# lmb-freiburg/flownet2

Hardware: AMD Instinct MI355X
Metric: image-pairs/sec FlowNetC forward at 448x320 (higher is better)
Workload: dtype f32

## Files before the change

### flownet2_amd/_lib.py

```python
from __future__ import annotations

import ctypes as C
import os

_HERE = os.path.dirname(os.path.abspath(__file__))
SO_PATH = os.path.join(_HERE, "libflownet2_hip.so")

EXPORTS = [
    "fn2_version", "fn2_last_error_string",
    "fn2_correlation_out_shape", "fn2_correlation_workspace_bytes", "fn2_correlation_forward", "fn2_correlation_forward_fused", "fn2_correlation_backward",
    "fn2_correlation1d_out_shape", "fn2_correlation1d_forward", "fn2_correlation1d_backward",
    "fn2_flow_warp_forward", "fn2_flow_warp_forward_slices", "fn2_flow_warp_backward_workspace_bytes", "fn2_flow_warp_backward",
    "fn2_resample_forward", "fn2_resample_forward_slices",
    "fn2_l1loss_workspace_bytes", "fn2_l1loss_forward", "fn2_l1loss_backward",
    "fn2_l1loss_multi_workspace_bytes", "fn2_l1loss_multi_sync_bytes", "fn2_l1loss_forward_multi", "fn2_l1loss_backward_multi",
    "fn2_channel_norm_forward", "fn2_channel_norm_forward_slices", "fn2_channel_norm_backward",
    "fn2_downsample_forward",
    "fn2_downsample_forward_multi",
    "fn2_predict_flow_conv_workspace_bytes", "fn2_predict_flow_conv_forward", "fn2_upsample_flow_deconv_forward", "fn2_upsample_flow_deconv_forward_into",
    "fn2_predict_flow_conv_backward_supported", "fn2_predict_flow_conv_backward_workspace_bytes", "fn2_predict_flow_conv_backward", "fn2_upsample_flow_deconv_backward_workspace_bytes", "fn2_upsample_flow_deconv_backward",
    "fn2_bias_leaky_relu_forward", "fn2_scale_shift_forward", "fn2_bias_leaky_relu_backward_workspace_bytes", "fn2_bias_leaky_relu_backward", "fn2_bias_leaky_relu_backward_slices", "fn2_bias_leaky_relu_backward_slices2",
    "fn2_conv_k7s2_relu_supported", "fn2_conv_k7s2_relu_forward",
    "fn2_conv_k7s2_wgrad_supported", "fn2_conv_k7s2_wgrad_ksplit", "fn2_conv_k7s2_wgrad_workspace_bytes", "fn2_conv_k7s2_wgrad",
    "fn2_conv_mfma_supported", "fn2_conv_mfma_packed_floats", "fn2_conv_mfma_pack_weights", "fn2_conv_mfma_pack_weights_view", "fn2_conv_mfma_forward",
    "fn2_conv_mfma_num_variants", "fn2_debug_set_conv_variant",
    "fn2_caffemodel_index", "fn2_caffemodel_read_blob", "fn2_hdf5_index", "fn2_hdf5_read_float",
    "fn2_conv_wino_supported", "fn2_conv_wino_packed_floats", "fn2_conv_wino_pack_weights", "fn2_conv_wino_forward",
    "fn2_conv_wino_num_variants", "fn2_debug_set_wino_variant",
    "fn2_conv_plane_supported", "fn2_conv_plane_ksplit", "fn2_conv_plane_workspace_bytes", "fn2_conv_plane_forward",
    "fn2_conv_plane_k_supported", "fn2_conv_plane_k_ksplit", "fn2_conv_plane_k_workspace_bytes", "fn2_conv_plane_k_forward",
    "fn2_conv_plane_num_variants", "fn2_debug_set_plane_variant", "fn2_debug_set_plane_ksplit", "fn2_set_batch_invariant", "fn2_get_batch_invariant",
    "fn2_deconv_plane_supported", "fn2_deconv_plane_ksplit", "fn2_deconv_plane_workspace_bytes", "fn2_deconv_plane_packed_floats",
    "fn2_deconv_plane_pack_weights", "fn2_deconv_plane_pack_weights_k", "fn2_deconv_plane_forward",
    "fn2_tconv_supported", "fn2_tconv_forward", "fn2_tconv_num_variants", "fn2_debug_set_tconv_variant",
    "fn2_debug_set_wgrad_buffers", "fn2_debug_set_wgrad_chunk", "fn2_conv_wgrad_supported", "fn2_conv_wgrad_ksplit", "fn2_conv_wgrad_workspace_bytes", "fn2_conv_wgrad",
    "fn2_conv_route", "fn2_conv_packed_weight_floats", "fn2_conv_pack_weights", "fn2_conv_workspace_bytes", "fn2_conv_forward",
    "fn2_deconv_route", "fn2_deconv_packed_weight_floats", "fn2_deconv_pack_weights", "fn2_deconv_workspace_bytes", "fn2_deconv_forward",
    "fn2_conv_backward_data_route", "fn2_conv_backward_data_packed_weight_floats", "fn2_conv_backward_data_pack_workspace_bytes",
    "fn2_conv_backward_data_pack_weights", "fn2_conv_backward_data_workspace_bytes", "fn2_conv_backward_data_workspace_bytes_with_room", "fn2_conv_backward_data_computed_channels", "fn2_conv_backward_data",
    "fn2_conv_backward_data_masked_supported", "fn2_conv_backward_data_masked", "fn2_conv_backward_weights_bias_fused", "fn2_conv_backward_weights_bias",
    "fn2_conv_backward_weights_supported", "fn2_conv_backward_weights_workspace_bytes", "fn2_conv_backward_weights", "fn2_conv_backward_bias",
    "fn2_im2col_forward", "fn2_col2im_bias_relu_forward", "fn2_col2im_bias_relu_forward_into",
    "fn2_datum_parse", "fn2_datum_float_data", "fn2_datum_serialize",
    "fn2_custom_data_sample_bytes", "fn2_custom_data_encode_sample", "fn2_custom_data_stage_records", "fn2_custom_data_decode_forward",
    "fn2_augmentation_matrix", "fn2_flow_augmentation_forward",
    "fn2_data_augmentation_workspace_bytes", "fn2_data_augmentation_forward",
]


class Fn2Error(RuntimeError):

    def __init__(self, status: int, message: str):
        super().__init__(f"[fn2 status {status}] {message}")
        self.status = status


class CaffemodelEntry(C.Structure):
    _fields_ = [("name_off", C.c_size_t), ("name_len", C.c_size_t), ("type_off", C.c_size_t), ("type_len", C.c_size_t),
                ("v1_type", C.c_longlong), ("v1", C.c_int), ("blob_index", C.c_int), ("num_axes", C.c_int), ("dim", C.c_longlong * 8),
                ("count", C.c_size_t), ("is_double", C.c_int), ("blob_off", C.c_size_t), ("blob_len", C.c_size_t)]


class Hdf5Entry(C.Structure):
    _fields_ = [("path", C.c_char * 256), ("num_axes", C.c_int), ("dim", C.c_longlong * 8), ("count", C.c_size_t), ("type_class", C.c_int),
                ("type_size", C.c_int), ("type_signed", C.c_int), ("big_endian", C.c_int), ("layout", C.c_int), ("num_filters", C.c_int),
                ("header_off", C.c_size_t)]


class ConvDesc(C.Structure):
    _fields_ = [("N", C.c_int), ("Cin", C.c_int), ("Hin", C.c_int), ("Win", C.c_int), ("Cout", C.c_int), ("kernel", C.c_int), ("stride", C.c_int), ("pad", C.c_int)]


class CorrParams(C.Structure):
    _fields_ = [("pad", C.c_int), ("kernel_size", C.c_int), ("max_displacement", C.c_int),
                ("stride1", C.c_int), ("stride2", C.c_int), ("corr_type", C.c_int), ("do_abs", C.c_int),
                ("single_direction", C.c_int)]


class DatumView(C.Structure):
    _fields_ = [("channels", C.c_int), ("height", C.c_int), ("width", C.c_int), ("label", C.c_int), ("encoded", C.c_int),
                ("data", C.c_void_p), ("data_bytes", C.c_size_t), ("float_data_count", C.c_size_t)]


class DataAugParams(C.Structure):
    _fields_ = [("crop_width", C.c_int), ("crop_height", C.c_int), ("max_multiplier", C.c_float), ("has_chromatic_eigvec", C.c_int),
                ("chromatic_eigvec", C.c_float * 9), ("mean_mode", C.c_int), ("noise_seed", C.c_ulonglong), ("noise_stream", C.c_ulonglong)]


class L1LossParams(C.Structure):
    _fields_ = [("l2_per_location", C.c_int), ("l2_prescale_by_channels", C.c_int),
                ("normalize_by_num_entries", C.c_int), ("epsilon", C.c_float), ("plateau", C.c_float)]


class L1LossScale(C.Structure):
    _fields_ = [("bottom0", C.c_void_p), ("bottom1", C.c_void_p), ("bottom0_diff", C.c_void_p), ("bottom1_diff", C.c_void_p),
                ("N", C.c_int), ("C", C.c_int), ("H", C.c_int), ("W", C.c_int), ("loss_weight", C.c_float)]


_lib = None


def lib():
    global _lib
    if _lib is not None:
        return _lib
    if not os.path.exists(SO_PATH):
        raise RuntimeError(
            f"{SO_PATH} not found: the HIP extension is not built. Run `python -m flownet2_amd.build` "
            "(or __graft_entry__.build()). flownet2_amd has no CPU / PyTorch fallback.")
    L = C.CDLL(SO_PATH)
    vp, fp, i, sz = C.c_void_p, C.c_void_p, C.c_int, C.c_size_t
    L.fn2_version.restype = C.c_char_p
    L.fn2_last_error_string.restype = C.c_char_p
    L.fn2_correlation_out_shape.argtypes = [C.POINTER(CorrParams), i, i, i, C.POINTER(i), C.POINTER(i), C.POINTER(i)]
    L.fn2_correlation_workspace_bytes.argtypes = [C.POINTER(CorrParams), i, i, i, i]
    L.fn2_correlation_workspace_bytes.restype = sz
    L.fn2_correlation_forward.argtypes = [C.POINTER(CorrParams), fp, fp, fp, i, i, i, i, vp, sz, vp]
    L.fn2_correlation_forward_fused.argtypes = [C.POINTER(CorrParams), fp, fp, fp, i, i, i, i, i, i, i, C.c_float, vp, sz, vp]
    L.fn2_correlation_backward.argtypes = [C.POINTER(CorrParams), fp, fp, fp, fp, fp, i, i, i, i, vp, sz, vp]
    L.fn2_correlation1d_out_shape.argtypes = [C.POINTER(CorrParams), i, i, i, C.POINTER(i), C.POINTER(i), C.POINTER(i)]
    L.fn2_correlation1d_forward.argtypes = [C.POINTER(CorrParams), fp, fp, fp, i, i, i, i, vp]
    L.fn2_correlation1d_backward.argtypes = [C.POINTER(CorrParams), fp, fp, fp, fp, fp, i, i, i, i, vp]
    L.fn2_flow_warp_forward.argtypes = [fp, fp, fp, i, i, i, i, i, vp]
    L.fn2_flow_warp_forward_slices.argtypes = [fp, i, i, fp, i, i, fp, i, i, i, i, i, i, i, vp]
    L.fn2_flow_warp_backward_workspace_bytes.argtypes = [i, i, i, i]
    L.fn2_flow_warp_backward_workspace_bytes.restype = sz
    L.fn2_flow_warp_backward.argtypes = [fp, fp, fp, fp, fp, i, i, i, i, i, i, vp, sz, vp]
    L.fn2_resample_forward.argtypes = [fp, fp, i, i, i, i, i, i, i, i, vp]
    L.fn2_resample_forward_slices.argtypes = [fp, C.c_float, fp, i, i, fp, i, i, C.c_float, i, i, i, i, i, i, i, i, vp]
    L.fn2_l1loss_workspace_bytes.argtypes = [i, i, i, i]
    L.fn2_l1loss_workspace_bytes.restype = sz
    L.fn2_l1loss_forward.argtypes = [C.POINTER(L1LossParams), fp, fp, fp, i, i, i, i, vp, sz, vp]
    L.fn2_l1loss_backward.argtypes = [C.POINTER(L1LossParams), fp, fp, C.c_float, fp, fp, i, i, i, i, vp, sz, vp]
    L.fn2_l1loss_multi_workspace_bytes.argtypes = [i]
    L.fn2_l1loss_multi_workspace_bytes.restype = sz
    L.fn2_l1loss_multi_sync_bytes.argtypes = []
    L.fn2_l1loss_multi_sync_bytes.restype = sz
    L.fn2_l1loss_forward_multi.argtypes = [C.POINTER(L1LossParams), i, C.POINTER(L1LossScale), fp, fp, vp, sz, vp, vp]
    L.fn2_l1loss_backward_multi.argtypes = [C.POINTER(L1LossParams), i, C.POINTER(L1LossScale), fp, vp, sz, vp]
    L.fn2_channel_norm_forward.argtypes = [fp, fp, i, i, i, i, vp]
    L.fn2_channel_norm_forward_slices.argtypes = [fp, i, i, fp, i, i, fp, i, i, i, i, i, i, vp]
    L.fn2_channel_norm_backward.argtypes = [fp, fp, fp, fp, i, i, i, i, vp]
    L.fn2_downsample_forward.argtypes = [fp, fp, i, i, i, i, i, i, vp]
    L.fn2_downsample_forward_multi.argtypes = [fp, C.POINTER(fp), C.POINTER(i), C.POINTER(i), i, i, i, i, i, vp]
    L.fn2_predict_flow_conv_workspace_bytes.argtypes = [i, i, i, i]
    L.fn2_predict_flow_conv_workspace_bytes.restype = sz
    L.fn2_predict_flow_conv_forward.argtypes = [fp, fp, fp, fp, i, i, i, i, vp, sz, vp]
    L.fn2_predict_flow_conv_backward_supported.argtypes = [i, i, i, i]
    L.fn2_predict_flow_conv_backward_workspace_bytes.argtypes = [i, i, i, i]
    L.fn2_predict_flow_conv_backward_workspace_bytes.restype = sz
    L.fn2_predict_flow_conv_backward.argtypes = [fp, i, i, fp, fp, fp, fp, fp, i, i, i, i, i, vp, sz, vp]
    L.fn2_upsample_flow_deconv_backward_workspace_bytes.argtypes = [i, i, i]
    L.fn2_upsample_flow_deconv_backward_workspace_bytes.restype = sz
    L.fn2_upsample_flow_deconv_backward.argtypes = [fp, fp, fp, fp, fp, fp, i, i, i, i, vp, sz, vp]
    L.fn2_upsample_flow_deconv_forward.argtypes = [fp, fp, fp, fp, i, i, i, vp]
    L.fn2_upsample_flow_deconv_forward_into.argtypes = [fp, fp, fp, fp, i, i, i, i, i, vp]
    L.fn2_bias_leaky_relu_forward.argtypes = [fp, fp, i, i, i, i, C.c_float, vp]
    L.fn2_scale_shift_forward.argtypes = [fp, fp, fp, i, i, i, i, i, i, C.c_float, vp]
    L.fn2_bias_leaky_relu_backward_workspace_bytes.argtypes = [i, i, i, i]
    L.fn2_bias_leaky_relu_backward_workspace_bytes.restype = sz
    L.fn2_bias_leaky_relu_backward.argtypes = [fp, fp, fp, fp, i, i, i, i, C.c_float, vp, sz, vp]
    L.fn2_bias_leaky_relu_backward_slices.argtypes = [fp, fp, i, i, fp, fp, i, i, i, i, C.c_float, vp, sz, vp]
    L.fn2_bias_leaky_relu_backward_slices2.argtypes = [fp, i, i, fp, i, i, fp, fp, i, i, i, i, C.c_float, vp, sz, vp]
    L.fn2_conv_k7s2_relu_supported.argtypes = [i, i, i, i]
    L.fn2_im2col_forward.argtypes = [fp, fp, i, i, i, i, i, i, i, vp]
    L.fn2_col2im_bias_relu_forward.argtypes = [fp, fp, fp, i, i, i, i, i, i, i, i, C.c_float, vp]
    L.fn2_col2im_bias_relu_forward_into.argtypes = [fp, fp, fp, i, i, i, i, i, i, i, i, C.c_float, i, i, vp]
    L.fn2_conv_k7s2_relu_forward.argtypes = [fp, fp, fp, fp, i, i, i, i, i, C.c_float, vp]
    L.fn2_conv_mfma_supported.argtypes = [i] * 7
    L.fn2_conv_mfma_packed_floats.argtypes = [i, i, i]
    L.fn2_conv_mfma_packed_floats.restype = sz
    L.fn2_conv_mfma_pack_weights.argtypes = [fp, fp, i, i, i, vp]
    L.fn2_conv_mfma_pack_weights_view.argtypes = [fp, fp, i, i, i, i, i, C.c_longlong, C.c_longlong, i, vp]
    L.fn2_conv_mfma_forward.argtypes = [fp, fp, fp, fp] + [i] * 13 + [C.c_float, vp]
    L.fn2_debug_set_conv_variant.argtypes = [i]
    L.fn2_conv_wino_supported.argtypes = [i] * 5
    L.fn2_conv_wino_packed_floats.argtypes = [i, i]
    L.fn2_conv_wino_packed_floats.restype = sz
    L.fn2_conv_wino_pack_weights.argtypes = [fp, fp, i, i, vp]
    L.fn2_conv_wino_forward.argtypes = [fp, fp, fp, fp] + [i] * 11 + [C.c_float, vp]
    L.fn2_debug_set_wino_variant.argtypes = [i]
    L.fn2_conv_plane_supported.argtypes = [i] * 7
    L.fn2_conv_plane_ksplit.argtypes = [i] * 7
    L.fn2_conv_plane_workspace_bytes.argtypes = [i] * 7
    L.fn2_conv_plane_workspace_bytes.restype = sz
    L.fn2_conv_plane_forward.argtypes = [fp, fp, fp, fp] + [i] * 12 + [C.c_float, vp, sz, vp]
    L.fn2_conv_k7s2_wgrad_supported.argtypes = [i] * 5
    L.fn2_conv_k7s2_wgrad_ksplit.argtypes = [i] * 5
    L.fn2_conv_k7s2_wgrad_workspace_bytes.argtypes = [i] * 5
    L.fn2_conv_k7s2_wgrad_workspace_bytes.restype = sz
    L.fn2_conv_k7s2_wgrad.argtypes = [fp, fp, fp] + [i] * 6 + [vp, sz, vp]
    L.fn2_conv_plane_k_supported.argtypes = [i] * 8
    L.fn2_conv_plane_k_ksplit.argtypes = [i] * 8
    L.fn2_conv_plane_k_workspace_bytes.argtypes = [i] * 8
    L.fn2_conv_plane_k_workspace_bytes.restype = sz
    L.fn2_conv_plane_k_forward.argtypes = [fp, fp, fp, fp] + [i] * 13 + [C.c_float, vp, sz, vp]
    L.fn2_debug_set_plane_variant.argtypes = [i]
    L.fn2_debug_set_plane_ksplit.argtypes = [i]
    L.fn2_set_batch_invariant.argtypes = [i]
    L.fn2_get_batch_invariant.argtypes = []
    L.fn2_tconv_supported.argtypes = [i] * 8
    L.fn2_tconv_forward.argtypes = [fp, fp, fp, fp] + [i] * 14 + [C.c_float, vp]
    L.fn2_debug_set_tconv_variant.argtypes = [i]
    L.fn2_debug_set_wgrad_buffers.argtypes = [i]
    L.fn2_debug_set_wgrad_chunk.argtypes = [i]
    L.fn2_conv_wgrad_supported.argtypes = [i] * 10
    L.fn2_conv_wgrad_ksplit.argtypes = [i] * 10
    L.fn2_conv_wgrad_workspace_bytes.argtypes = [i] * 10
    L.fn2_conv_wgrad_workspace_bytes.restype = sz
    L.fn2_conv_wgrad.argtypes = [fp, fp, fp] + [i] * 15 + [vp, sz, vp]
    L.fn2_deconv_plane_supported.argtypes = [i] * 5
    L.fn2_deconv_plane_ksplit.argtypes = [i] * 5
    L.fn2_deconv_plane_workspace_bytes.argtypes = [i] * 5
    L.fn2_deconv_plane_workspace_bytes.restype = sz
    L.fn2_deconv_plane_packed_floats.argtypes = [i, i]
    L.fn2_deconv_plane_packed_floats.restype = sz
    L.fn2_deconv_plane_pack_weights.argtypes = [fp, fp, i, i, vp]
    L.fn2_deconv_plane_pack_weights_k.argtypes = [fp, fp, i, i, i, vp]
    L.fn2_deconv_plane_forward.argtypes = [fp, fp, fp, fp] + [i] * 10 + [C.c_float, vp, sz, vp]
    L.fn2_caffemodel_index.argtypes = [vp, sz, C.POINTER(CaffemodelEntry), i, C.POINTER(C.c_int)]
    L.fn2_caffemodel_read_blob.argtypes = [vp, sz, C.POINTER(CaffemodelEntry), fp, sz]
    L.fn2_hdf5_index.argtypes = [vp, sz, C.POINTER(Hdf5Entry), i, C.POINTER(C.c_int)]
    L.fn2_hdf5_read_float.argtypes = [vp, sz, C.POINTER(Hdf5Entry), fp, sz]
    ip = C.POINTER(C.c_int)
    L.fn2_datum_parse.argtypes = [vp, sz, C.POINTER(DatumView)]
    L.fn2_datum_float_data.argtypes = [vp, sz, fp, sz]
    L.fn2_datum_serialize.argtypes = [i, i, i, vp, sz, i, vp, sz]
    L.fn2_datum_serialize.restype = C.c_longlong
    L.fn2_custom_data_sample_bytes.argtypes = [i, i, i, ip, i, ip, i]
    L.fn2_custom_data_sample_bytes.restype = sz
    L.fn2_custom_data_encode_sample.argtypes = [vp, vp, vp, vp, i, i, vp, sz]
    L.fn2_custom_data_stage_records.argtypes = [C.POINTER(C.c_void_p), C.POINTER(sz), i, vp, sz, ip, ip, ip, C.POINTER(sz), ip]
    L.fn2_custom_data_decode_forward.argtypes = [vp, sz, i, i, i, i, ip, i, ip, i, i, fp, C.c_float, C.POINTER(C.c_void_p), vp]
    L.fn2_augmentation_matrix.argtypes = [fp, i, i, i, i, i, fp]
    L.fn2_flow_augmentation_forward.argtypes = [fp, fp, fp, fp, i, i, i, i, i, vp]
    L.fn2_data_augmentation_workspace_bytes.argtypes = [i]
    L.fn2_data_augmentation_workspace_bytes.restype = sz
    L.fn2_data_augmentation_forward.argtypes = [C.POINTER(DataAugParams), fp, fp, fp, fp, i, i, i, i, vp, sz, vp]
    dp = C.POINTER(ConvDesc)
    for pre in ("fn2_conv", "fn2_deconv"):
        getattr(L, pre + "_route").argtypes = [dp, i]
        getattr(L, pre + "_packed_weight_floats").argtypes = [dp, i]
        getattr(L, pre + "_packed_weight_floats").restype = sz
        getattr(L, pre + "_pack_weights").argtypes = [dp, i, fp, fp, vp]
        getattr(L, pre + "_workspace_bytes").argtypes = [dp, i]
        getattr(L, pre + "_workspace_bytes").restype = sz
        getattr(L, pre + "_forward").argtypes = [dp, i, fp, i, i, fp, fp, fp, i, i, i, C.c_float, vp, sz, vp]
    L.fn2_conv_backward_data_route.argtypes = [dp, i]
    L.fn2_conv_backward_data_packed_weight_floats.argtypes = [dp, i, i]
    L.fn2_conv_backward_data_packed_weight_floats.restype = sz
    L.fn2_conv_backward_data_pack_workspace_bytes.argtypes = [dp, i, i]
    L.fn2_conv_backward_data_pack_workspace_bytes.restype = sz
    L.fn2_conv_backward_data_pack_weights.argtypes = [dp, i, i, fp, fp, vp, sz, vp]
    L.fn2_conv_backward_data_workspace_bytes.argtypes = [dp, i, i]
    L.fn2_conv_backward_data_workspace_bytes.restype = sz
    L.fn2_conv_backward_data_computed_channels.argtypes = [dp, i, i]
    L.fn2_conv_backward_data.argtypes = [dp, i, i, fp, i, i, fp, fp, i, i, i, vp, sz, vp]
    L.fn2_conv_backward_weights_supported.argtypes = [dp, i]
    L.fn2_conv_backward_weights_workspace_bytes.argtypes = [dp, i]
    L.fn2_conv_backward_weights_workspace_bytes.restype = sz
    L.fn2_conv_backward_weights.argtypes = [dp, i, fp, i, i, fp, i, i, fp, i, vp, sz, vp]
    L.fn2_conv_backward_data_workspace_bytes_with_room.argtypes = [dp, i, i, i]
    L.fn2_conv_backward_data_workspace_bytes_with_room.restype = sz
    L.fn2_conv_backward_data_masked_supported.argtypes = [dp, i, i]
    L.fn2_conv_backward_data_masked.argtypes = [dp, i, i, fp, i, i, fp, fp, i, i, fp, i, i, C.c_float, vp]
    L.fn2_conv_backward_weights_bias_fused.argtypes = [dp, i]
    L.fn2_conv_backward_weights_bias.argtypes = [dp, i, fp, fp, fp, fp, i, vp, sz, vp]
    L.fn2_conv_backward_bias.argtypes = [fp, i, i, fp, i, i, i, i, i, vp, sz, vp]
    if hasattr(L, "fn2_debug_set_correlation_impl"):
        L.fn2_debug_set_correlation_impl.argtypes = [i]
    if hasattr(L, "fn2_debug_correlation_units_plan"):
        L.fn2_debug_correlation_units_plan.argtypes = [i, i, i, i, C.POINTER(C.c_uint), i]
    if hasattr(L, "fn2_debug_set_resample_generic"):
        L.fn2_debug_set_resample_generic.argtypes = [i]
    for name in EXPORTS:
        if not hasattr(L, name):
            raise RuntimeError(f"{SO_PATH} does not export {name}")
        fn = getattr(L, name)
        if fn.restype is C.c_int:
            pass
    _lib = L
    return L


def check(status: int):
    if status != 0:
        raise Fn2Error(status, lib().fn2_last_error_string().decode())


def version() -> str:
    return lib().fn2_version().decode()
```

### flownet2_amd/build.py

```python
from __future__ import annotations

import glob
import os
import shutil
import subprocess
import sys

HERE = os.path.dirname(os.path.abspath(__file__))
CSRC = os.path.join(HERE, "csrc")
SO = os.path.join(HERE, "libflownet2_hip.so")
ARCH = "gfx950"


def hipcc() -> str:
    for c in (os.environ.get("HIPCC"), "/opt/rocm/bin/hipcc", shutil.which("hipcc")):
        if c and os.path.exists(c):
            return c
    raise RuntimeError("hipcc not found (need ROCm >= 7.0 for gfx950)")


def sources():
    return sorted(glob.glob(os.path.join(CSRC, "*.hip")) + glob.glob(os.path.join(CSRC, "*.cpp")))


def is_stale() -> bool:
    if not os.path.exists(SO):
        return True
    t = os.path.getmtime(SO)
    deps = sources() + glob.glob(os.path.join(CSRC, "*.hpp")) + [os.path.join(HERE, "..", "include", "flownet2_hip.h")]
    return any(os.path.getmtime(d) > t for d in deps)


def build(force: bool = False, verbose: bool = False) -> str:
    if not force and not is_stale():
        return SO
    objs = []
    objdir = os.path.join(HERE, "build")
    os.makedirs(objdir, exist_ok=True)
    flags = ["--offload-arch=" + ARCH, "-O3", "-std=c++17", "-fPIC", "-fvisibility=hidden", "-munsafe-fp-atomics",
             "-Wall", "-Wno-unused-function"]
    if os.environ.get("FN2_ABLATION"):
        flags.append("-DFN2_ABLATION=1")
    per_file = {"conv_wino.hip": ["-fno-slp-vectorize"]}
    procs = []
    for src in sources():
        obj = os.path.join(objdir, os.path.basename(src) + ".o")
        objs.append(obj)
        hdrs = glob.glob(os.path.join(CSRC, "*.hpp")) + [os.path.join(HERE, "..", "include", "flownet2_hip.h")]
        if not force and os.path.exists(obj) and all(os.path.getmtime(obj) >= os.path.getmtime(d) for d in [src] + hdrs):
            continue
        cmd = [hipcc()] + flags + per_file.get(os.path.basename(src), []) + ["-x", "hip", "-c", src, "-o", obj]
        if verbose:
            print(" ".join(cmd), file=sys.stderr)
        procs.append((src, subprocess.Popen(cmd, stdout=subprocess.PIPE, stderr=subprocess.STDOUT)))
    for src, p in procs:
        out, _ = p.communicate()
        if p.returncode != 0:
            raise RuntimeError(f"hipcc failed on {src}:\n{out.decode()}")
        if verbose and out:
            print(out.decode(), file=sys.stderr)
    cmd = [hipcc(), "--offload-arch=" + ARCH, "-shared", "-fPIC", "-o", SO] + objs + ["-lz"]
    subprocess.check_call(cmd)
    return SO


if __name__ == "__main__":
    print(build(force="--force" in sys.argv, verbose=True))
```

### flownet2_amd/csrc/conv_stem.hip

```cpp
#include "fn2_common.hpp"
#include "mfma_tile.hpp"

#include <type_traits>

namespace fn2 {
using mfma::f32x4;
using mfma::kOOB;
using mfma::kRsrcWord3;
using mfma::lds_ptr_t;

struct StemArgs {
  int N, Hin, Win, Hout, Wout, Cout;
  int Ctot, c0;
  int ntx;
  int nyb;
  float slope;
};

template <int CIN, int RB, int XT, int PASS>
__global__ void __launch_bounds__(256, 2)
conv_k7s2_relu(const float* __restrict__ in, const float* __restrict__ weight, const float* __restrict__ bias,
               float* __restrict__ out, StemArgs a) {
  constexpr int ROWS = 2 * RB + 5;
  constexpr int RS = 32 * XT + 8;
  constexpr int CS = ROWS * RS;
  constexpr int SLOTS = CIN * ROWS * (RS / 4);
  constexpr int NRUN = (SLOTS + 63) / 64;
  extern __shared__ __attribute__((aligned(16))) float smem[];

  const int tid = threadIdx.x, lane = tid & 63;
  const int wave = __builtin_amdgcn_readfirstlane(tid >> 6);
  int b = blockIdx.x;
  const int bx = b % a.ntx; b /= a.ntx;
  const int by = b % a.nyb; b /= a.nyb;
  const int cog = b % (a.Cout / 64), n = b / (a.Cout / 64);
  const int x0 = bx * 16 * XT, y0 = by * RB;
  const int co0 = cog * 64 + wave * 16;

  const size_t plane = (size_t)a.Hin * a.Win;
  const __amdgpu_buffer_rsrc_t rs = __builtin_amdgcn_make_buffer_rsrc(
      const_cast<float*>(in + ((size_t)n * a.Ctot + a.c0) * plane), 0, (unsigned)(4u * CIN * plane), kRsrcWord3);
  const unsigned lds_base = (unsigned)(uintptr_t)(lds_ptr_t)smem;
#pragma unroll
  for (int i = 0; i < (NRUN + 3) / 4; ++i) {
    const int run = i * 4 + wave;
    if (run < NRUN) {
      const int s = run * 64 + lane;
      unsigned voff = kOOB;
      if (s < SLOTS) {
        const int c = s / (ROWS * (RS / 4)), rem = s % (ROWS * (RS / 4));
        const int row = rem / (RS / 4), gq = rem % (RS / 4);
        const int yi = 2 * y0 - 3 + row, xi = 2 * x0 - 4 + 4 * gq;
        if (yi >= 0 && yi < a.Hin && xi >= 0 && xi < a.Win) voff = 4u * (unsigned)(c * plane + (size_t)yi * a.Win + xi);
      }
      __builtin_amdgcn_raw_ptr_buffer_load_lds(rs, (lds_ptr_t)(uintptr_t)(lds_base + run * 1024u), 16, voff, 0, 0, 0);
    }
  }

  const int kk = lane >> 4, nn = lane & 15;
  float w[CIN][7][2];
  {
    const float* wp = weight + ((size_t)(co0 + nn) * a.Ctot + a.c0) * 49;
#pragma unroll
    for (int c = 0; c < CIN; ++c)
#pragma unroll
      for (int ky = 0; ky < 7; ++ky) {
        w[c][ky][0] = wp[(c * 7 + ky) * 7 + kk];
        w[c][ky][1] = kk < 3 ? wp[(c * 7 + ky) * 7 + 4 + kk] : 0.f;
      }
  }
  const float bv = bias ? bias[co0 + nn] : 0.f;
  asm volatile("s_waitcnt vmcnt(0)" ::: "memory");
  __syncthreads();

  const int abase = 2 * nn + kk + 1;
  const int xq = 4 * (lane >> 4);
  auto tiles = [&](auto ntag, int rb, int y, int t) {
    constexpr int NTL = decltype(ntag)::value;
    f32x4 acc[NTL];
#pragma unroll
    for (int u = 0; u < NTL; ++u) acc[u] = f32x4{0.f, 0.f, 0.f, 0.f};
    const float* r0 = smem + (2 * rb) * RS + 32 * t + abase;
#pragma unroll
    for (int c = 0; c < CIN; ++c)
#pragma unroll
      for (int ky = 0; ky < 7; ++ky)
#pragma unroll
        for (int h = 0; h < 2; ++h)
#pragma unroll
          for (int u = 0; u < NTL; ++u) {
            float av = r0[c * CS + ky * RS + 4 * h + 32 * u];
            if (h == 1) av = kk == 3 ? 0.f : av;
            acc[u] = __builtin_amdgcn_mfma_f32_16x16x4f32(av, w[c][ky][h], acc[u], 0, 0, 0);
          }
    float* orow = out + (((size_t)n * a.Cout + co0 + nn) * a.Hout + y) * a.Wout;
#pragma unroll
    for (int u = 0; u < NTL; ++u) {
      const int x = x0 + 16 * (t + u) + xq;
      if (x < a.Wout) {
        f32x4 v = acc[u];
        if constexpr (PASS == 2) v += *reinterpret_cast<const f32x4*>(orow + x);
        if constexpr (PASS != 1) {
#pragma unroll
          for (int j = 0; j < 4; ++j) { const float s = v[j] + bv; v[j] = s > 0.f ? s : s * a.slope; }
        }
        *reinterpret_cast<f32x4*>(orow + x) = v;
      }
    }
  };
  for (int rb = 0; rb < RB; ++rb) {
    const int y = y0 + rb;
    if (y >= a.Hout) break;
    int t = 0;
#pragma unroll 1
    for (; t + 1 < XT; t += 2) {
      if (x0 + 16 * t >= a.Wout) break;
      tiles(std::integral_constant<int, 2>{}, rb, y, t);
    }
    if ((XT & 1) && x0 + 16 * t < a.Wout) tiles(std::integral_constant<int, 1>{}, rb, y, t);
  }
}

template <int CIN, int PASS>
static int launch_stem(const float* in, const float* weight, const float* bias, float* out, int N, int Ctot, int c0, int Hin, int Win,
                       int Cout, float slope, hipStream_t st) {
  constexpr int RB = 2, XT = 7;
  StemArgs a;
  a.N = N; a.Hin = Hin; a.Win = Win; a.Cout = Cout; a.slope = slope; a.Ctot = Ctot; a.c0 = c0;
  a.Hout = (Hin + 6 - 7) / 2 + 1; a.Wout = (Win + 6 - 7) / 2 + 1;
  a.ntx = (a.Wout + 16 * XT - 1) / (16 * XT);
  a.nyb = (a.Hout + RB - 1) / RB;
  const long long grid = (long long)N * (Cout / 64) * a.nyb * a.ntx;
  if (grid > 0x7fffffffll) return fail(FN2_ERR_UNSUPPORTED, "conv_k7s2_relu: grid too large");
  constexpr size_t lds = sizeof(float) * CIN * (2 * RB + 5) * (32 * XT + 8) + 1024;
  static bool attr_set = false;
  if (!attr_set) {
    (void)hipFuncSetAttribute(reinterpret_cast<const void*>(&conv_k7s2_relu<CIN, RB, XT, PASS>), hipFuncAttributeMaxDynamicSharedMemorySize, (int)lds);
    attr_set = true;
  }
  hipLaunchKernelGGL((conv_k7s2_relu<CIN, RB, XT, PASS>), dim3((unsigned)grid), dim3(256), lds, st, in, weight, bias, out, a);
  return check_launch("conv_k7s2_relu_forward");
}

}

using namespace fn2;

FN2_API int fn2_conv_k7s2_relu_supported(int Cin, int Hin, int Win, int Cout) {
  return (Cin == 3 || Cin == 6 || Cin == 12) && Cout % 64 == 0 && Cout > 0 && Hin >= 1 && Win >= 8 && Win % 8 == 0 &&
         (long long)Cin * Hin * Win < (1ll << 28);
}

FN2_API int fn2_conv_k7s2_relu_forward(const float* in, const float* weight, const float* bias, float* out,
                                       int N, int Cin, int Hin, int Win, int Cout, float negative_slope, void* stream) {
  if (N < 0 || Cin <= 0 || Hin <= 0 || Win <= 0 || Cout <= 0) return fail(FN2_ERR_INVALID_ARG, "conv_k7s2_relu: bad shape");
  if (N == 0) return FN2_OK;
  if (!in || !weight || !out) return fail(FN2_ERR_INVALID_ARG, "conv_k7s2_relu: null blob");
  if (!fn2_conv_k7s2_relu_supported(Cin, Hin, Win, Cout))
    return fail(FN2_ERR_UNSUPPORTED, "conv_k7s2_relu: needs Cin in {3,6,12}, Cout %% 64 == 0, width %% 8 == 0 (got Cin %d, Cout %d, W %d)", Cin, Cout, Win);
  if (((reinterpret_cast<uintptr_t>(in) | reinterpret_cast<uintptr_t>(out)) & 15) != 0)
    return fail(FN2_ERR_UNSUPPORTED, "conv_k7s2_relu: blobs must be 16-byte aligned");
  hipStream_t st = reinterpret_cast<hipStream_t>(stream);
  if (Cin == 3) return launch_stem<3, 0>(in, weight, bias, out, N, 3, 0, Hin, Win, Cout, negative_slope, st);
  if (Cin == 6) return launch_stem<6, 0>(in, weight, bias, out, N, 6, 0, Hin, Win, Cout, negative_slope, st);
  const int rc = launch_stem<6, 1>(in, weight, bias, out, N, 12, 0, Hin, Win, Cout, negative_slope, st);
  if (rc) return rc;
  return launch_stem<6, 2>(in, weight, bias, out, N, 12, 6, Hin, Win, Cout, negative_slope, st);
}
```

### flownet2_amd/csrc/flow_head.hip

```cpp
#include "fn2_common.hpp"

namespace fn2 {

constexpr int kHeadPix = 64;

template <int G>
__global__ void __launch_bounds__(kHeadPix* G) conv3x3_c2_taps(const float* __restrict__ in, const float* __restrict__ w,
                                                                float* __restrict__ P, int N, int C, int H, int W, int nsplit) {
  __shared__ float red[G][18][kHeadPix];
  const int lane_pix = threadIdx.x % kHeadPix;
  const int grp = __builtin_amdgcn_readfirstlane(threadIdx.x / kHeadPix);
  const size_t plane = (size_t)H * W;
  const long long total = (long long)N * H * W;
  const long long p = (long long)blockIdx.x * kHeadPix + lane_pix;
  const bool live = p < total;
  const int n = live ? (int)(p / (long long)plane) : 0;
  const unsigned pix = live ? (unsigned)(p - (long long)n * plane) : 0u;
  const float* src = in + (size_t)n * C * plane + pix;
  float a[18];
#pragma unroll
  for (int k = 0; k < 18; ++k) a[k] = 0.f;
  const int ngroups = G * nsplit;
  const int c_per = (C + ngroups - 1) / ngroups;
  const int c_lo = min(C, ((int)blockIdx.y * G + grp) * c_per), c_hi = min(C, c_lo + c_per);
  for (int c = c_lo; c < c_hi; c += 8) {
    float v[8];
#pragma unroll
    for (int cc = 0; cc < 8; ++cc) v[cc] = (c + cc < c_hi) ? src[(size_t)(c + cc) * plane] : 0.f;
    __builtin_amdgcn_sched_barrier(0);
#pragma unroll
    for (int cc = 0; cc < 8; ++cc) {
      if (c + cc < c_hi) {
        const float* w0 = w + (size_t)(c + cc) * 9;
        const float* w1 = w + ((size_t)C + c + cc) * 9;
#pragma unroll
        for (int t = 0; t < 9; ++t) {
          a[t] = fmaf(w0[t], v[cc], a[t]);
          a[9 + t] = fmaf(w1[t], v[cc], a[9 + t]);
        }
      }
    }
  }
#pragma unroll
  for (int k = 0; k < 18; ++k) red[grp][k][lane_pix] = a[k];
  __syncthreads();
  if (live) {
    float* dst = P + ((size_t)blockIdx.y * N + n) * 18 * plane + pix;
    for (int k = grp; k < 18; k += G) {
      float sacc = 0.f;
#pragma unroll
      for (int g = 0; g < G; ++g) sacc += red[g][k][lane_pix];
      dst[(size_t)k * plane] = sacc;
    }
  }
}

template <int NSPLIT>
__global__ void __launch_bounds__(256) conv3x3_c2_gather(const float* __restrict__ P, const float* __restrict__ bias,
                                                          float* __restrict__ out, int N, int H, int W) {
  const unsigned plane = (unsigned)H * W;
  const unsigned pix = blockIdx.x * 256u + threadIdx.x;
  if (pix >= plane) return;
  const int y = pix / W, x = pix - y * W;
  const unsigned no = blockIdx.y;
  const unsigned n = no >> 1, o = no & 1;
  float v[NSPLIT][9];
#pragma unroll
  for (int sp = 0; sp < NSPLIT; ++sp) {
    const float* Pn = P + (((size_t)sp * N + n) * 18 + o * 9) * plane;
#pragma unroll
    for (int dy = 0; dy < 3; ++dy)
#pragma unroll
      for (int dx = 0; dx < 3; ++dx) {
        const int yy = y + dy - 1, xx = x + dx - 1;
        const bool ok = yy >= 0 && yy < H && xx >= 0 && xx < W;
        v[sp][dy * 3 + dx] = ok ? Pn[(size_t)(dy * 3 + dx) * plane + (unsigned)yy * W + xx] : 0.f;
      }
  }
  float sacc = bias ? bias[o] : 0.f;
#pragma unroll
  for (int sp = 0; sp < NSPLIT; ++sp)
#pragma unroll
    for (int t = 0; t < 9; ++t) sacc += v[sp][t];
  out[(size_t)no * plane + pix] = sacc;
}

__global__ void __launch_bounds__(256) deconv4x4s2_c2(const float* __restrict__ in, const float* __restrict__ w,
                                                       const float* __restrict__ bias, float* __restrict__ out,
                                                       int N, int H, int W, int out_ctot, int out_c0) {
  const int Ho = 2 * H, Wo = 2 * W;
  const long long total = (long long)N * Ho * Wo;
  for (long long idx = blockIdx.x * (long long)blockDim.x + threadIdx.x; idx < total; idx += (long long)gridDim.x * blockDim.x) {
    const int X = (int)(idx % Wo), Y = (int)((idx / Wo) % Ho), n = (int)(idx / ((long long)Wo * Ho));
    float a0 = bias ? bias[0] : 0.f, a1 = bias ? bias[1] : 0.f;
#pragma unroll
    for (int ty = 0; ty < 2; ++ty) {
      const int ky = ((Y + 1) & 1) + 2 * ty;
      const int iy = (Y + 1 - ky) / 2;
      if (Y + 1 - ky < 0 || iy >= H) continue;
#pragma unroll
      for (int tx = 0; tx < 2; ++tx) {
        const int kx = ((X + 1) & 1) + 2 * tx;
        const int ix = (X + 1 - kx) / 2;
        if (X + 1 - kx < 0 || ix >= W) continue;
#pragma unroll
        for (int c = 0; c < 2; ++c) {
          const float v = in[(((size_t)n * 2 + c) * H + iy) * W + ix];
          a0 = fmaf(w[((c * 2 + 0) * 4 + ky) * 4 + kx], v, a0);
          a1 = fmaf(w[((c * 2 + 1) * 4 + ky) * 4 + kx], v, a1);
        }
      }
    }
    out[(((size_t)n * out_ctot + out_c0 + 0) * Ho + Y) * Wo + X] = a0;
    out[(((size_t)n * out_ctot + out_c0 + 1) * Ho + Y) * Wo + X] = a1;
  }
}

}

using namespace fn2;

constexpr int kHeadG = 16;

static int head_splits(int N, int C, int H, int W) {
  const long long blocks = ((long long)order_batch(N) * H * W + kHeadPix - 1) / kHeadPix;
  int nsplit = 1;
  while (nsplit < 8 && blocks * kHeadG * nsplit < 4096 && C >= 8 * kHeadG * nsplit * 2) nsplit *= 2;
  return nsplit;
}

FN2_API size_t fn2_predict_flow_conv_workspace_bytes(int N, int C, int H, int W) {
  if (N < 1 || C < 1 || H < 1 || W < 1) return 0;
  return sizeof(float) * (size_t)head_splits(N, C, H, W) * N * 18 * H * W;
}

FN2_API int fn2_predict_flow_conv_forward(const float* in, const float* weight, const float* bias, float* out,
                                          int N, int C, int H, int W, void* workspace, size_t workspace_bytes, void* stream) {
  if (N < 0 || C < 1 || H < 1 || W < 1) return fail(FN2_ERR_INVALID_ARG, "predict_flow_conv: bad shape [%d,%d,%d,%d]", N, C, H, W);
  if (N == 0) return FN2_OK;
  if (!in || !weight || !out) return fail(FN2_ERR_INVALID_ARG, "predict_flow_conv: NULL blob pointer");
  if ((long long)H * W >= (1ll << 31) || 2ll * N > 65535) return fail(FN2_ERR_UNSUPPORTED, "predict_flow_conv: blob too large");
  const size_t need = fn2_predict_flow_conv_workspace_bytes(N, C, H, W);
  if (!workspace || workspace_bytes < need) return fail(FN2_ERR_WORKSPACE, "predict_flow_conv: workspace too small (%zu < %zu)", workspace_bytes, need);
  const long long total = (long long)N * H * W;
  const unsigned blocks = (unsigned)((total + kHeadPix - 1) / kHeadPix);
  const int nsplit = head_splits(N, C, H, W);
  hipStream_t st = as_stream(stream);
  float* P = reinterpret_cast<float*>(workspace);
  hipLaunchKernelGGL(conv3x3_c2_taps<kHeadG>, dim3(blocks, nsplit), dim3(kHeadPix * kHeadG), 0, st, in, weight, P, N, C, H, W, nsplit);
  const dim3 g2(((unsigned)H * W + 255) / 256, 2 * N);
  switch (nsplit) {
    case 1: hipLaunchKernelGGL(conv3x3_c2_gather<1>, g2, dim3(256), 0, st, P, bias, out, N, H, W); break;
    case 2: hipLaunchKernelGGL(conv3x3_c2_gather<2>, g2, dim3(256), 0, st, P, bias, out, N, H, W); break;
    case 4: hipLaunchKernelGGL(conv3x3_c2_gather<4>, g2, dim3(256), 0, st, P, bias, out, N, H, W); break;
    default: hipLaunchKernelGGL(conv3x3_c2_gather<8>, g2, dim3(256), 0, st, P, bias, out, N, H, W); break;
  }
  return check_launch("predict_flow_conv_forward");
}

FN2_API int fn2_upsample_flow_deconv_forward(const float* in, const float* weight, const float* bias, float* out,
                                             int N, int H, int W, void* stream) {
  if (N < 0 || H < 1 || W < 1) return fail(FN2_ERR_INVALID_ARG, "upsample_flow_deconv: bad shape");
  if (N == 0) return FN2_OK;
  if (!in || !weight || !out) return fail(FN2_ERR_INVALID_ARG, "upsample_flow_deconv: NULL blob pointer");
  const long long total = (long long)N * 4 * H * W;
  hipLaunchKernelGGL(deconv4x4s2_c2, dim3(blocks_for(total, 256, 4096)), dim3(256), 0, as_stream(stream), in, weight, bias, out, N, H, W, 2, 0);
  return check_launch("upsample_flow_deconv_forward");
}

FN2_API int fn2_upsample_flow_deconv_forward_into(const float* in, const float* weight, const float* bias, float* top,
                                                  int N, int H, int W, int top_channels, int top_c0, void* stream) {
  if (N < 0 || H < 1 || W < 1) return fail(FN2_ERR_INVALID_ARG, "upsample_flow_deconv: bad shape");
  if (top_c0 < 0 || top_c0 + 2 > top_channels) return fail(FN2_ERR_INVALID_ARG, "upsample_flow_deconv: channel slice outside the blob");
  if (N == 0) return FN2_OK;
  if (!in || !weight || !top) return fail(FN2_ERR_INVALID_ARG, "upsample_flow_deconv: NULL blob pointer");
  const long long total = (long long)N * 4 * H * W;
  hipLaunchKernelGGL(deconv4x4s2_c2, dim3(blocks_for(total, 256, 4096)), dim3(256), 0, as_stream(stream), in, weight, bias, top, N, H, W, top_channels, top_c0);
  return check_launch("upsample_flow_deconv_forward_into");
}
```

### flownet2_amd/functional.py

```python
from __future__ import annotations

import os

import torch

from . import ops


_BATCH_INVARIANT = [False]


def set_batch_invariant(on: bool = True):
    _BATCH_INVARIANT[0] = bool(on)
    ops.set_batch_invariant(bool(on))


def batch_invariant() -> bool:
    return _BATCH_INVARIANT[0]


LIBRARY_FALLBACKS = [0]


def _note_fallback(what, x, w):
    LIBRARY_FALLBACKS[0] += 1
    if os.environ.get("FN2_STRICT") == "1":
        raise RuntimeError("flownet2_amd: no own kernel for %s bottom %s weight %s (FN2_STRICT=1)" % (what, tuple(x.shape), tuple(w.shape)))
    if os.environ.get("FN2_TRACE_FALLBACK") == "1":
        print("library fallback: %s bottom %s weight %s" % (what, tuple(x.shape), tuple(w.shape)), flush=True)


def lib_conv2d(x, w, b, stride, pad):
    if x.is_cuda:
        _note_fallback("Convolution{stride %d, pad %d}" % (stride, pad), x, w)
    if not _BATCH_INVARIANT[0] or not x.is_cuda:
        return torch.nn.functional.conv2d(x, w, b, stride=stride, padding=pad)
    return torch.cat([torch.nn.functional.conv2d(x[n:n + 1], w, b, stride=stride, padding=pad) for n in range(x.shape[0])], 0)


def lib_conv_transpose2d(x, w, b, stride, pad):
    if x.is_cuda:
        _note_fallback("Deconvolution{stride %d, pad %d}" % (stride, pad), x, w)
    if not _BATCH_INVARIANT[0] or not x.is_cuda:
        return torch.nn.functional.conv_transpose2d(x, w, b, stride=stride, padding=pad)
    return torch.cat([torch.nn.functional.conv_transpose2d(x[n:n + 1], w, b, stride=stride, padding=pad) for n in range(x.shape[0])], 0)


def scale_shift(x, scale, shift=None, out=None, out_c0=0):
    with torch.no_grad():
        return ops.scale_shift_forward(x.detach().contiguous(), scale, shift, out=out, out_c0=out_c0)


class _Correlation(torch.autograd.Function):
    @staticmethod
    def forward(ctx, b0, b1, params):
        ctx.params = params
        ctx.save_for_backward(b0, b1)
        return ops.correlation_forward(params, b0, b1)

    @staticmethod
    def backward(ctx, g):
        b0, b1 = ctx.saved_tensors
        d0, d1 = ops.correlation_backward(ctx.params, b0, b1, g.contiguous(),
                                          need0=ctx.needs_input_grad[0], need1=ctx.needs_input_grad[1])
        return d0, d1, None


def correlation(b0, b1, pad=0, kernel_size=1, max_displacement=0, stride_1=1, stride_2=1, correlation_type=ops.MULTIPLY):
    p = ops.corr_params(pad, kernel_size, max_displacement, stride_1, stride_2, correlation_type)
    return _Correlation.apply(b0.contiguous(), b1.contiguous(), p)


class _CorrelationReluInto(torch.autograd.Function):

    @staticmethod
    def forward(ctx, b0, b1, params, blob, c0, slope):
        ops.correlation_forward(params, b0, b1, out=blob, out_c0=c0, relu=True, negative_slope=slope)
        tc = ops.correlation_out_shape(params, b0.shape[1], b0.shape[2], b0.shape[3])[0]
        ctx.cfg = (params, c0, tc, slope)
        ctx.save_for_backward(b0, b1, blob)
        return blob[:, c0:c0 + tc]

    @staticmethod
    def backward(ctx, g):
        b0, b1, blob = ctx.saved_tensors
        params, c0, tc, slope = ctx.cfg
        gb, g0 = _channel_slice(g)
        d, _ = ops.bias_leaky_relu_backward((blob, c0, tc), (gb, g0, tc), slope, False)
        d0, d1 = ops.correlation_backward(params, b0, b1, d, need0=ctx.needs_input_grad[0], need1=ctx.needs_input_grad[1])
        return d0, d1, None, None, None, None


def correlation_relu_into(b0, b1, out, out_c0, negative_slope, pad=0, kernel_size=1, max_displacement=0, stride_1=1, stride_2=1, training=False):
    p = ops.corr_params(pad, kernel_size, max_displacement, stride_1, stride_2, ops.MULTIPLY)
    if torch.is_grad_enabled() and (b0.requires_grad or b1.requires_grad):
        if not training:
            return None
        return _CorrelationReluInto.apply(b0.contiguous(), b1.contiguous(), p, out, out_c0, negative_slope)
    return ops.correlation_forward(p, b0.contiguous(), b1.contiguous(), out=out, out_c0=out_c0, relu=True, negative_slope=negative_slope)


class _FlowWarp(torch.autograd.Function):
    @staticmethod
    def forward(ctx, image, flow, fill_value):
        ctx.save_for_backward(image, flow)
        return ops.flow_warp_forward(image, flow, fill_value)

    @staticmethod
    def backward(ctx, g):
        image, flow = ctx.saved_tensors
        di, df = ops.flow_warp_backward(image, flow, g.contiguous(), ctx.needs_input_grad[0], ctx.needs_input_grad[1])
        return (di if ctx.needs_input_grad[0] else None), (df if ctx.needs_input_grad[1] else None), None


def flow_warp(image, flow, fill_value=ops.FILL_ZERO):
    return _FlowWarp.apply(image.contiguous(), flow.contiguous(), fill_value)


def resample(x, height, width, type=ops.LINEAR, antialias=True):
    with torch.no_grad():
        return ops.resample_forward(x.detach().contiguous(), height, width, type, antialias)


def resample_slices(x, height, width, type=ops.LINEAR, antialias=True, in_scale=1.0, out=None, out2=None, out2_scale=1.0):
    with torch.no_grad():
        return ops.resample_forward_slices(x.detach().contiguous(), height, width, type, antialias, in_scale, out, out2, out2_scale)


def flow_warp_slices(image, flow, out=None, fill_value=ops.FILL_ZERO):
    with torch.no_grad():
        return ops.flow_warp_forward_slices(image, flow, out, fill_value)


def channel_norm_slices(x, minus=None, out=None):
    with torch.no_grad():
        return ops.channel_norm_forward_slices(x, minus, out)


def downsample(x, top_height, top_width):
    with torch.no_grad():
        return ops.downsample_forward(x.detach().contiguous(), top_height, top_width)


def downsample_ahead(x, sizes):
    with torch.no_grad():
        x = x.detach().contiguous()
        many = (lambda: ops.downsample_forward_multi(x, sizes)) if ops.downsample_multi_supported(x.shape, sizes) and x.shape[0] > 0 else \
            (lambda: [ops.downsample_forward(x, h, w) for h, w in sizes])
        if not x.is_cuda:
            return [ops.downsample_forward(x, h, w) for h, w in sizes], None
        main = torch.cuda.current_stream(x.device)
        side = _WGRAD_SIDE["streams"].get(x.device)
        if side is None:
            side = _WGRAD_SIDE["streams"][x.device] = torch.cuda.Stream(device=x.device)
        side.wait_stream(main)
        with torch.cuda.stream(side):
            outs = many()
            ev = torch.cuda.Event()
            ev.record(side)
        x.record_stream(side)
        for t in outs:
            t.record_stream(main)
        return outs, ev


def wait_ahead(event):
    if event is not None:
        torch.cuda.current_stream().wait_event(event)


class _ChannelNorm(torch.autograd.Function):
    @staticmethod
    def forward(ctx, x):
        top = ops.channel_norm_forward(x)
        ctx.save_for_backward(x, top)
        return top

    @staticmethod
    def backward(ctx, g):
        x, top = ctx.saved_tensors
        return ops.channel_norm_backward(x, top, g.contiguous())


def channel_norm(x):
    return _ChannelNorm.apply(x.contiguous())


class _L1Loss(torch.autograd.Function):
    @staticmethod
    def forward(ctx, b0, b1, params):
        loss, ws = ops.l1loss_forward(params, b0, b1)
        ctx.params, ctx.ws = params, ws
        ctx.save_for_backward(b0, b1)
        return loss

    @staticmethod
    def backward(ctx, g):
        b0, b1 = ctx.saved_tensors
        d0, d1 = ops.l1loss_backward(ctx.params, b0, b1, float(g), ctx.ws)
        return (d0 if ctx.needs_input_grad[0] else None), (d1 if (b1 is not None and ctx.needs_input_grad[1]) else None), None


def l1_loss(b0, b1=None, l2_per_location=False, l2_prescale_by_channels=False, normalize_by_num_entries=False,
            epsilon=1e-2, plateau=0.0):
    p = ops.l1_params(l2_per_location, l2_prescale_by_channels, normalize_by_num_entries, epsilon, plateau)
    return _L1Loss.apply(b0.contiguous(), b1.contiguous() if b1 is not None else None, p)


class _L1LossMulti(torch.autograd.Function):

    @staticmethod
    def forward(ctx, params, weights, n, *blobs):
        b0, b1 = list(blobs[:n]), list(blobs[n:])
        total, losses, ws = ops.l1loss_forward_multi(params, b0, b1, weights)
        ctx.params, ctx.weights, ctx.n, ctx.ws = params, weights, n, ws
        ctx.save_for_backward(*blobs)
        ctx.mark_non_differentiable(losses)
        return total, losses

    @staticmethod
    def backward(ctx, g, _g_losses):
        n = ctx.n
        blobs = ctx.saved_tensors
        b0, b1 = list(blobs[:n]), list(blobs[n:])
        need1 = any(ctx.needs_input_grad[3 + n:])
        d0, d1 = ops.l1loss_backward_multi(ctx.params, b0, b1, ctx.weights, g.contiguous(), ctx.ws, need1=need1)
        grads = [d if ctx.needs_input_grad[3 + k] else None for k, d in enumerate(d0)]
        grads += [d if ctx.needs_input_grad[3 + n + k] else None for k, d in enumerate(d1)]
        return (None, None, None) + tuple(grads)


def l1_loss_multi(preds, targets, weights, l2_per_location=False, l2_prescale_by_channels=False, normalize_by_num_entries=False,
                  epsilon=1e-2, plateau=0.0):
    p = ops.l1_params(l2_per_location, l2_prescale_by_channels, normalize_by_num_entries, epsilon, plateau)
    blobs = [t.contiguous() for t in preds] + [t.contiguous() for t in targets]
    return _L1LossMulti.apply(p, tuple(float(w) for w in weights), len(preds), *blobs)


class _PredictFlow(torch.autograd.Function):

    @staticmethod
    def forward(ctx, x, weight, bias):
        ctx.save_for_backward(x, weight)
        ctx.has_bias = bias is not None
        return ops.predict_flow_conv_forward(x.contiguous(), weight.contiguous(), bias)

    @staticmethod
    def backward(ctx, g):
        x, w = ctx.saved_tensors
        blob, c0 = _channel_slice(x)
        g = g.contiguous()
        need_x, need_w, need_b = ctx.needs_input_grad[0], ctx.needs_input_grad[1], ctx.has_bias and ctx.needs_input_grad[2]
        side = _wgrad_side_stream(g, x, w) if (need_w or need_b) and need_x else None
        if side is None:
            return ops.predict_flow_conv_backward((blob, c0, x.shape[1]), w, g, need_x, need_w, need_b)
        dx, _, _ = ops.predict_flow_conv_backward((blob, c0, x.shape[1]), w, g, True, False, False)
        main = torch.cuda.current_stream(g.device)
        side.wait_stream(main)
        with torch.cuda.stream(side):
            _, dw, db = ops.predict_flow_conv_backward((blob, c0, x.shape[1]), w, g, False, need_w, need_b)
        for t in (g, blob):
            t.record_stream(side)
        for t in (dw, db):
            if t is not None:
                t.record_stream(main)
        if dw is not None:
            _SIDE_PENDING.append((w, dw.data_ptr()))
        return dx, dw, db


class _UpsampleFlow(torch.autograd.Function):

    @staticmethod
    def forward(ctx, x, weight, bias, into=None):
        ctx.save_for_backward(x, weight)
        ctx.has_bias = bias is not None
        if into is None:
            return ops.upsample_flow_deconv_forward(x.contiguous(), weight.contiguous(), bias)
        ops.upsample_flow_deconv_forward(x.contiguous(), weight.contiguous(), bias, out=into[0], out_c0=into[1])
        return into[0][:, into[1]:into[1] + 2]

    @staticmethod
    def backward(ctx, g):
        x, w = ctx.saved_tensors
        dx, dw, db = ops.upsample_flow_deconv_backward(x.contiguous(), w, g.contiguous(), ctx.needs_input_grad[0], ctx.needs_input_grad[1],
                                                       ctx.has_bias and ctx.needs_input_grad[2])
        return dx, dw, db, None


def predict_flow_conv(x, weight, bias=None):
    run = lambda xx, ww, bb: ops.predict_flow_conv_forward(xx.contiguous(), ww.contiguous(), bb)
    if _needs_grad(x, weight, bias):
        if ops.predict_flow_conv_backward_supported(x.shape[0], x.shape[1], x.shape[2], x.shape[3]):
            return _PredictFlow.apply(x, weight, bias)
        return _OwnForwardConv.apply(x, weight, bias, run, 1, 1, 0.0, False, False)
    return run(x, weight, bias)


def upsample_flow_deconv(x, weight, bias=None, out=None, out_c0=0):
    if out is not None and not _needs_grad(x, weight, bias):
        return ops.upsample_flow_deconv_forward(x.contiguous(), weight.contiguous(), bias, out=out, out_c0=out_c0)
    run = lambda xx, ww, bb: ops.upsample_flow_deconv_forward(xx.contiguous(), ww.contiguous(), bb)
    if _needs_grad(x, weight, bias):
        return _UpsampleFlow.apply(x, weight, bias, None if out is None else (out, out_c0))
    return run(x, weight, bias)


class _BiasLeakyReLU(torch.autograd.Function):

    @staticmethod
    def forward(ctx, y, bias, negative_slope):
        ctx.mark_dirty(y)
        ops.bias_leaky_relu_(y, bias, negative_slope)
        ctx.slope = negative_slope
        ctx.has_bias = bias is not None
        ctx.save_for_backward(y)
        return y

    @staticmethod
    def backward(ctx, g):
        (y,) = ctx.saved_tensors
        d, db = ops.bias_leaky_relu_backward(y, g.contiguous(), ctx.slope, ctx.has_bias and ctx.needs_input_grad[1])
        return d, db, None


def conv_bias_leaky_relu(y, bias, negative_slope=0.1):
    if not y.is_contiguous():
        if bias is not None:
            y = y + bias.view(1, -1, 1, 1)
        return torch.nn.functional.leaky_relu(y, negative_slope)
    if torch.is_grad_enabled() and (y.requires_grad or (bias is not None and bias.requires_grad)):
        return _BiasLeakyReLU.apply(y, bias, negative_slope)
    return ops.bias_leaky_relu_(y, bias, negative_slope)


def invalidate_weight_caches():
    _bump_weight_generation()
    _PACKED_T.clear()


_WEIGHT_GENERATION = [0]


def weight_generation() -> int:
    return _WEIGHT_GENERATION[0]


def _bump_weight_generation(*_a, **_k):
    _WEIGHT_GENERATION[0] += 1


try:
    from torch.optim.optimizer import register_optimizer_step_post_hook as _reg_step_hook
    _reg_step_hook(_bump_weight_generation)
    _HAVE_STEP_HOOK = True
except Exception:
    _HAVE_STEP_HOOK = False


def _cached(cache, key, w, make):
    import weakref
    if w.requires_grad and (not _HAVE_STEP_HOOK or (w.is_cuda and torch.cuda.is_current_stream_capturing())):
        cache.pop(key, None)
        return make()
    gen = _WEIGHT_GENERATION[0] if w.requires_grad else -1
    hit = cache.get(key)
    if hit is None or hit[0]() is not w or hit[1] != w._version or hit[3] != gen:
        hit = (weakref.ref(w, lambda _r, k=key: cache.pop(k, None)), w._version, make(), gen)
        cache[key] = hit
    return hit[2]


_ROUTE_FORCE = [False]


def set_route_force(on: bool = True):
    _ROUTE_FORCE[0] = bool(on)


def _channel_slice(x):
    if x.is_contiguous():
        return x, 0
    b = x._base
    if (b is not None and b.dim() == 4 and b.is_contiguous() and x.dim() == 4 and x.stride() == b.stride() and x.shape[0] == b.shape[0]
            and x.shape[2:] == b.shape[2:]):
        plane = b.shape[2] * b.shape[3]
        off = x.storage_offset() - b.storage_offset()
        if off % plane == 0 and 0 <= off // plane and off // plane + x.shape[1] <= b.shape[1]:
            return b, off // plane
    return x.contiguous(), 0


class _OwnForwardConv(torch.autograd.Function):

    @staticmethod
    def forward(ctx, x, weight, bias, runner, stride, pad, negative_slope, act, transposed, into=None, relu_chain=None):
        if into is None:
            y = runner(x, weight, bias)
        else:
            runner(x, weight, bias, into[0], into[1])
            co = weight.shape[1] if transposed else weight.shape[0]
            y = into[0][:, into[1]:into[1] + co]
        ctx.cfg = (stride, pad, negative_slope, act, bias is not None, transposed)
        ctx.into = into
        ctx.relu_chain, ctx.chain_cell = (int(relu_chain[0]), relu_chain[1]) if relu_chain else (0, None)
        if ctx.relu_chain & 1:
            ctx.chain_cell["armed"] = True
        elif ctx.relu_chain & 2 and not ctx.chain_cell.get("armed"):
            raise RuntimeError("relu_chain: the layer in front of this one is not a chain producer (it would undo its ReLU twice)")
        ctx.save_for_backward(x, weight, (into[0] if into is not None else y) if act else None)
        return y

    @staticmethod
    def backward(ctx, g):
        x, w, y = ctx.saved_tensors
        stride, pad, slope, act, has_bias, transposed = ctx.cfg
        if act and ctx.into is not None:
            y = (y, ctx.into[1], w.shape[1] if transposed else w.shape[0])
        premasked = False
        if ctx.relu_chain & 1:
            if not ctx.chain_cell.get("masked"):
                raise RuntimeError("relu_chain: the consumer of this layer did not fold the ReLU derivative into its data gradient")
            ctx.chain_cell["masked"] = False
            premasked = True
        gx, gw, db = conv_backward(x, w, y if act else None, g, stride, pad, slope, transposed, bool(ctx.needs_input_grad[0]),
                                   bool(ctx.needs_input_grad[1]), has_bias and ctx.needs_input_grad[2], premasked=premasked,
                                   mask_bottom=(ctx.chain_cell["slope"] if (ctx.relu_chain & 2) else None))
        if ctx.relu_chain & 2:
            ctx.chain_cell["masked"] = True
        return (gx, gw, db) + (None,) * (len(ctx.needs_input_grad) - 3)


_GRAD_SLOT = [None]


def set_grad_slots(fn=None):
    _GRAD_SLOT[0] = fn


def _grad_slot(w):
    fn = _GRAD_SLOT[0]
    if fn is None or w.grad is not None:
        return None
    return fn(w)


_WGRAD_SIDE = {"pixels": 0, "streams": {}}
_SIDE_TASK = [-1]
_SIDE_PENDING = []


def set_wgrad_side_stream(max_pixels: int = 0):
    _WGRAD_SIDE["pixels"] = int(max_pixels)


def side_stream_for_collective(device):
    if not _WGRAD_SIDE["pixels"]:
        return None
    st = _WGRAD_SIDE["streams"].get(device)
    if st is None:
        return None
    st.wait_stream(torch.cuda.current_stream(device))
    return st


def _wgrad_side_stream(d, x, w):
    if not _WGRAD_SIDE["pixels"] or not d.is_cuda or w.grad is not None or max(d.shape[2] * d.shape[3], x.shape[2] * x.shape[3]) > _WGRAD_SIDE["pixels"]:
        return None
    task = torch._C._current_graph_task_id()
    if task < 0:
        return None
    if task != _SIDE_TASK[0]:
        if _SIDE_PENDING:
            _SIDE_PENDING.clear()
            for dev, st in _WGRAD_SIDE["streams"].items():
                torch.cuda.current_stream(dev).wait_stream(st)
        torch.autograd.Variable._execution_engine.queue_callback(join_side_streams)
        _SIDE_TASK[0] = task
    st = _WGRAD_SIDE["streams"].get(d.device)
    if st is None:
        st = _WGRAD_SIDE["streams"][d.device] = torch.cuda.Stream(device=d.device)
    return st


def join_side_streams():
    _SIDE_TASK[0] = -1
    if not _SIDE_PENDING:
        return
    for dev, st in _WGRAD_SIDE["streams"].items():
        torch.cuda.current_stream(dev).wait_stream(st)
    pending = list(_SIDE_PENDING)
    _SIDE_PENDING.clear()
    if _GRAD_SLOT[0] is not None:
        return
    for w, ptr in pending:
        if ptr and w.grad is not None and w.grad.data_ptr() != ptr:
            raise RuntimeError("functional.set_wgrad_side_stream: autograd did not move a weight gradient computed on the second stream into "
                               ".grad as it was (shared weight? retained graph?): the result may have been read early.  Switch it off "
                               "(set_wgrad_side_stream(0)) for this graph.")


def relu_chain_supported(x_shape, w, stride, pad) -> bool:
    desc = _layer_desc(w, stride, pad, False, x_shape=x_shape)
    if desc is None or not w.is_cuda:
        return False
    route = ops.conv_backward_data_route(desc, False)
    return route != 0 and ops.conv_backward_data_masked_supported(desc, False, route)


def conv_backward(x, w, y, g, stride, pad, slope, transposed, need_x, need_w, need_b, premasked=False, mask_bottom=None):
    if y is not None and premasked:
        d = g.contiguous()
        db = None
        if need_w and need_b and not transposed and d.is_cuda:
            desc = _layer_desc(w, stride, pad, False, x_shape=x.shape)
            if desc is not None and ops.conv_backward_weights_bias_fused(desc, False) and x.is_contiguous():
                gw, db = ops.conv_backward_weights_bias(x, d, desc, False, out=_grad_slot(w))
                gx = _own_bwd_data(d, w, stride, pad, transposed, x.shape) if need_x else None
                if not need_x or gx is not None:
                    return gx, gw, db
        if need_b:
            db = ops.conv_backward_bias(d, d.shape[1])
    elif y is not None:
        gb, g0 = _channel_slice(g)
        if not isinstance(y, tuple):
            yb, y0 = _channel_slice(y)
            y = (yb, y0, y.shape[1])
        d, db = ops.bias_leaky_relu_backward(y, (gb, g0, g.shape[1]), slope, need_b)
    else:
        g = g.contiguous()
        d, db = g, (g.sum((0, 2, 3)) if need_b else None)
    gx = None
    if need_x and mask_bottom is not None:
        gx = _own_bwd_data_masked(d, w, stride, pad, x, mask_bottom)
    if need_x and gx is None:
        if mask_bottom is not None:
            raise RuntimeError("relu_chain: the data gradient of this layer has no masked form (relu_chain_supported was not asked?)")
        gx = _own_bwd_data(d, w, stride, pad, transposed, x.shape)
    gw = None
    if need_w:
        side = _wgrad_side_stream(d, x, w)
        if side is None:
            gw = _own_bwd_weight(d, x, w, stride, pad, transposed)
        else:
            main = torch.cuda.current_stream(d.device)
            side.wait_stream(main)
            with torch.cuda.stream(side):
                gw = _own_bwd_weight(d, x, w, stride, pad, transposed)
            if gw is None:
                main.wait_stream(side)
            else:
                for t in (d, x):
                    t.record_stream(side)
                gw.record_stream(main)
                _SIDE_PENDING.append((w, gw.data_ptr()))
    lib_x, lib_w = need_x and gx is None, need_w and gw is None
    if (lib_x or lib_w) and os.environ.get("FN2_TRACE_BWD") == "1":
        print("bwd on the library: x %s w %s stride %d pad %d transposed %s -> %s%s" % (tuple(x.shape), tuple(w.shape), stride, pad, transposed,
                                                                                      "data " if lib_x else "", "weight" if lib_w else ""), flush=True)
    if lib_x or lib_w:
        if x.is_cuda:
            _note_fallback("%s backward{stride %d, pad %d}%s%s" % ("Deconvolution" if transposed else "Convolution", stride, pad,
                                                                   " data" if lib_x else "", " weight" if lib_w else ""), x, w)
        cd, was = torch.backends.cudnn, torch.backends.cudnn.deterministic
        cd.deterministic = True
        try:
            gxl, gwl, _ = torch.ops.aten.convolution_backward(d, x, w, None, [stride, stride], [pad, pad], [1, 1], transposed, [0, 0], 1,
                                                              [lib_x, lib_w, False])
        finally:
            cd.deterministic = was
        gx, gw = (gxl if lib_x else gx), (gwl if lib_w else gw)
    return gx, gw, db


def _layer_desc(w, stride, pad, transposed, x_shape=None, d_shape=None):
    k = int(w.shape[2])
    if w.shape[3] != k:
        return None
    Cin, Cout = (int(w.shape[0]), int(w.shape[1])) if transposed else (int(w.shape[1]), int(w.shape[0]))
    if x_shape is not None:
        N, H, W = int(x_shape[0]), int(x_shape[2]), int(x_shape[3])
    elif transposed and d_shape[2] % 2 == 0 and d_shape[3] % 2 == 0:
        N, H, W = int(d_shape[0]), int(d_shape[2]) // 2, int(d_shape[3]) // 2
    elif not transposed and stride == 1:
        N, H, W = int(d_shape[0]), int(d_shape[2]) - 1 + k - 2 * pad, int(d_shape[3]) - 1 + k - 2 * pad
    else:
        return None
    if H < 1 or W < 1:
        return None
    return ops.conv_desc(N, Cin, H, W, Cout, k, stride, pad)


def _own_bwd_weight(d, x, w, stride, pad, transposed):
    if not d.is_cuda:
        return None
    desc = _layer_desc(w, stride, pad, transposed, x_shape=x.shape)
    if desc is None or not ops.conv_backward_weights_supported(desc, transposed):
        return None
    if (not transposed and desc.kernel == 7) and not (d.is_contiguous() and x.is_contiguous()):
        d, x = d.contiguous(), x.contiguous()
    xb, x0 = _channel_slice(x)
    db, d0 = _channel_slice(d)
    return ops.conv_backward_weights(xb, db, desc, transposed, out=_grad_slot(w), bottom_c0=x0, top_c0=d0)


_PACKED_T = {}


def _cached_pack(cache, w, tag, make):
    return _cached(cache, (id(w), tag), w, make)


def _own_bwd_data(d, w, stride, pad, transposed, x_shape=None):
    if not d.is_cuda:
        return None
    desc = _layer_desc(w, stride, pad, transposed, x_shape=x_shape, d_shape=d.shape)
    if desc is None:
        return None
    route = ops.conv_backward_data_route(desc, transposed)
    if route == 0:
        return None
    key = (desc.N, desc.Hin, desc.Win)
    packed = _cached_pack(_PACKED_T, w, ("dgrad", route, bool(transposed), stride, pad) + key,
                          lambda: ops.conv_backward_data_pack_weights(w.detach().contiguous(), desc, transposed, route))
    db, d0 = _channel_slice(d)
    return ops.conv_backward_data(db, packed, desc, transposed, route, top_c0=d0)


def _own_bwd_data_masked(d, w, stride, pad, x, slope):
    desc = _layer_desc(w, stride, pad, False, x_shape=x.shape)
    if desc is None or not d.is_cuda:
        return None
    route = ops.conv_backward_data_route(desc, False)
    if route == 0 or not ops.conv_backward_data_masked_supported(desc, False, route):
        return None
    key = (desc.N, desc.Hin, desc.Win)
    packed = _cached_pack(_PACKED_T, w, ("dgrad", route, False, stride, pad) + key,
                          lambda: ops.conv_backward_data_pack_weights(w.detach().contiguous(), desc, False, route))
    db, d0 = _channel_slice(d)
    xb, x0 = _channel_slice(x)
    return ops.conv_backward_data_masked(db, packed, desc, False, route, xb, slope, top_c0=d0, data_c0=x0)


def _needs_grad(*ts):
    return torch.is_grad_enabled() and any(t is not None and t.requires_grad for t in ts)


def conv_forward_route(desc, act=True, whole_blobs=True) -> int:
    route = ops.conv_forward_route(desc, force=_ROUTE_FORCE[0])
    stem = route == ops.CONV_ROUTE_STEM
    if route == ops.CONV_ROUTE_HEAD:
        return ops.CONV_ROUTE_NONE
    if stem and not (act and whole_blobs):
        return ops.CONV_ROUTE_NONE
    if desc.kernel not in (1, 3, 5, 7) or (desc.kernel == 7 and not stem and desc.Cin % 4 != 0):
        return ops.CONV_ROUTE_NONE
    return route


def deconv_forward_route(desc, act=True) -> int:
    if not act or desc.Cin < 64:
        return ops.DECONV_ROUTE_NONE
    route = ops.deconv_forward_route(desc)
    return ops.DECONV_ROUTE_NONE if route == ops.DECONV_ROUTE_HEAD else route


def conv_route_name(x_shape, w, stride, pad, act=True, whole_blobs=True):
    desc = _layer_desc(w, stride, pad, False, x_shape=x_shape)
    return ops.CONV_FWD_ROUTES[conv_forward_route(desc, act, whole_blobs)] if desc is not None else None


def conv_mfma_relu(x, weight, bias, stride, pad, negative_slope=0.1, act=True, out=None, out_c0=0, relu_chain=None):
    desc = _layer_desc(weight, stride, pad, False, x_shape=x.shape) if x.is_cuda else None
    route = conv_forward_route(desc, act, out is None) if desc is not None else ops.CONV_ROUTE_NONE
    if route == ops.CONV_ROUTE_NONE:
        return None
    if relu_chain is not None and int(relu_chain[0]) & 1 and route != ops.CONV_ROUTE_STEM:
        raise RuntimeError("relu_chain: only the stem layer is a chain producer")

    def run(xx, ww, bb, o=None, o0=0):
        if route == ops.CONV_ROUTE_STEM:
            blob, c0, packed = xx.contiguous(), 0, ww.detach().contiguous()
        else:
            blob, c0 = _channel_slice(xx)
            packed = _cached_pack(_PACKED_T, ww, ("fwd", route, False), lambda: ops.conv_pack_weights(ww.detach(), desc, route))
        return ops.conv_forward(blob, packed, bb, desc, route, False, act, negative_slope, out=o, out_c0=o0, in_c0=c0)

    if _needs_grad(x, weight, bias):
        return _OwnForwardConv.apply(x, weight, bias, run, stride, pad, negative_slope, act, False, None if out is None else (out, out_c0), relu_chain)
    return run(x, weight, bias, out, out_c0)


def deconv_relu(x, weight, bias, negative_slope=0.1, act=True, out=None, out_c0=0):
    desc = _layer_desc(weight, 2, 1, True, x_shape=x.shape) if x.is_cuda else None
    route = deconv_forward_route(desc, act) if desc is not None else ops.DECONV_ROUTE_NONE
    if route == ops.DECONV_ROUTE_NONE:
        return None

    def run(xx, ww, bb, o=None, o0=0):
        blob, c0 = _channel_slice(xx)
        packed = _cached_pack(_PACKED_T, ww, ("fwd", route, True), lambda: ops.conv_pack_weights(ww.detach(), desc, route, True))
        return ops.conv_forward(blob, packed, bb, desc, route, True, True, negative_slope, out=o, out_c0=o0, in_c0=c0)

    if _needs_grad(x, weight, bias):
        return _OwnForwardConv.apply(x, weight, bias, run, 2, 1, negative_slope, True, True, None if out is None else (out, out_c0))
    return run(x, weight, bias, out, out_c0)
```

### flownet2_amd/nets.py

```python
from __future__ import annotations

import math
import weakref
from typing import Dict, Optional


import torch
import torch.nn.functional as F

NEG_SLOPE = 0.1
FLOW_SCALE = 20.0
SD_FLOW_SCALE = 0.05
LOSS_WEIGHTS = {6: 0.32, 5: 0.08, 4: 0.02, 3: 0.01, 2: 0.005}

_ENC_TAIL = [("conv4", 256, 512, 3, 2, 1), ("conv4_1", 512, 512, 3, 1, 1), ("conv5", 512, 512, 3, 2, 1),
             ("conv5_1", 512, 512, 3, 1, 1), ("conv6", 512, 1024, 3, 2, 1), ("conv6_1", 1024, 1024, 3, 1, 1)]
_DEC = [("Convolution1", "conv", 1024, 2), ("deconv5", "deconv", 1024, 512), ("upsample_flow6to5", "deconv", 2, 2),
        ("Convolution2", "conv", 1026, 2), ("deconv4", "deconv", 1026, 256), ("upsample_flow5to4", "deconv", 2, 2),
        ("Convolution3", "conv", 770, 2), ("deconv3", "deconv", 770, 128), ("upsample_flow4to3", "deconv", 2, 2),
        ("Convolution4", "conv", 386, 2), ("deconv2", "deconv", 386, 64), ("upsample_flow3to2", "deconv", 2, 2),
        ("Convolution5", "conv", 194, 2)]


def layer_table(kind: str = "C", in_channels: int = 6):
    t = []
    if kind == "C":
        t += [("conv1", "conv", 3, 64, 7, 2, 3), ("conv2", "conv", 64, 128, 5, 2, 2), ("conv3", "conv", 128, 256, 5, 2, 2),
              ("conv_redir", "conv", 256, 32, 1, 1, 0), ("conv3_1", "conv", 473, 256, 3, 1, 1)]
    else:
        t += [("conv1", "conv", in_channels, 64, 7, 2, 3), ("conv2", "conv", 64, 128, 5, 2, 2), ("conv3", "conv", 128, 256, 5, 2, 2),
              ("conv3_1", "conv", 256, 256, 3, 1, 1)]
    t += [(n, "conv", ci, co, k, s, p) for (n, ci, co, k, s, p) in _ENC_TAIL]
    for (n, k, ci, co) in _DEC:
        t.append((n, k, ci, co, 3, 1, 1) if k == "conv" else (n, k, ci, co, 4, 2, 1))
    return t


def init_params(kind: str = "C", seed: int = 0, device="cpu", in_channels: int = 6) -> Dict[str, torch.Tensor]:
    g = torch.Generator().manual_seed(seed)
    params = {}
    for (name, k, ci, co, ks, s, p) in layer_table(kind, in_channels):
        shape = (co, ci, ks, ks) if k == "conv" else (ci, co, ks, ks)
        fan_in = ci * ks * ks if k == "conv" else ci * ks * ks / (s * s)
        std = math.sqrt(2.0 / ((1 + NEG_SLOPE ** 2) * fan_in))
        if name.startswith("Convolution"):
            std *= 0.5
        if name.startswith("upsample_flow"):
            std = 0.25
        params[name + ".w"] = (torch.randn(shape, generator=g) * std).to(device)
        params[name + ".b"] = torch.zeros(co).to(device)
    return params


def num_params(params) -> int:
    return sum(int(v.numel()) for v in params.values())


def _conv(x, P, name, stride, pad, act=True, backend=None, relu_chain=None):
    w = P[name + ".w"]
    if relu_chain is not None:
        y = conv_forward(x, w, P[name + ".b"], stride, pad, act, backend, relu_chain=relu_chain)
    else:
        y = _conv_routed(x, P, name, stride, pad, act, backend)
    if _TRACE_CONV:
        print("conv route %-16s in %-22s k%d s%d act=%d -> %s" % (name, tuple(x.shape), w.shape[2], stride, act, _LAST_ROUTE[0]))
    return y


_TRACE_CONV = __import__("os").environ.get("FN2_TRACE_CONV") == "1"
_LAST_ROUTE = [""]


def _conv_routed(x, P, name, stride, pad, act, backend):
    return conv_forward(x, P[name + ".w"], P[name + ".b"], stride, pad, act, backend)


def conv_forward(x, w, b, stride, pad, act, backend, slope=None, relu_chain=None):
    slope = NEG_SLOPE if slope is None else slope
    y = None
    if backend is not None and hasattr(backend, "conv_mfma_relu"):
        y = backend.conv_mfma_relu(x, w, b, stride, pad, slope, act, relu_chain=relu_chain)
    if y is not None:
        _LAST_ROUTE[0] = "fn2 %s" % backend.conv_route_name(x.shape, w, stride, pad, act) if _TRACE_CONV and hasattr(backend, "conv_route_name") else "own kernel"
        return y
    if relu_chain is not None:
        raise RuntimeError("relu_chain: no own kernel takes this layer (its consumer was told the stem kernel would)")
    _LAST_ROUTE[0] = "library conv2d"
    conv2d = getattr(backend, "lib_conv2d", None) or (lambda xx, ww, bb, s, p: F.conv2d(xx, ww, bb, stride=s, padding=p))
    if act and backend is not None and hasattr(backend, "conv_bias_leaky_relu"):
        return backend.conv_bias_leaky_relu(conv2d(x, w, None, stride, pad), b, slope)
    y = conv2d(x, w, b, stride, pad)
    return F.leaky_relu(y, slope) if act else y


_CONSTS: Dict[tuple, torch.Tensor] = {}


def _const(device, values):
    key = (str(device), tuple(float(v) for v in values))
    if key not in _CONSTS:
        _CONSTS[key] = torch.tensor(key[1], device=device, dtype=torch.float32)
    return _CONSTS[key]


def _deconv(x, P, name, act=True, backend=None):
    return deconv_forward(x, P[name + ".w"], P[name + ".b"], act, backend)


def deconv_forward(x, w, b, act=True, backend=None, slope=None):
    slope = NEG_SLOPE if slope is None else slope
    if backend is not None and hasattr(backend, "deconv_relu"):
        y = backend.deconv_relu(x, w, b, slope, act)
        if y is not None:
            return y
    deconv2d = getattr(backend, "lib_conv_transpose2d", None) or (lambda xx, ww, bb, s, p: F.conv_transpose2d(xx, ww, bb, stride=s, padding=p))
    if act and backend is not None and hasattr(backend, "conv_bias_leaky_relu"):
        return backend.conv_bias_leaky_relu(deconv2d(x, w, None, 2, 1), b, slope)
    y = deconv2d(x, w, b, 2, 1)
    return F.leaky_relu(y, slope) if act else y


def _conv_into_concat(x, P, name, stride, pad, extra_channels, backend, relu_chain=None):
    w = P[name + ".w"]
    training = torch.is_grad_enabled() and (x.requires_grad or _any_requires_grad(P))
    if (backend is not None and hasattr(backend, "conv_mfma_relu") and x.is_cuda and w.shape[2] in (3, 5)
            and (not training or (CONCAT_IN_PLACE_TRAINING[0] and hasattr(backend, "conv_backward")))):
        k = w.shape[2]
        ho, wo = (x.shape[2] + 2 * pad - k) // stride + 1, (x.shape[3] + 2 * pad - k) // stride + 1
        blob = torch.empty((x.shape[0], w.shape[0] + extra_channels, ho, wo), device=x.device, dtype=x.dtype)
        y = backend.conv_mfma_relu(x, w, P[name + ".b"], stride, pad, NEG_SLOPE, True, out=blob, out_c0=0, relu_chain=relu_chain)
        if y is not None:
            return blob, (y if (training and y.requires_grad) else blob[:, :w.shape[0]])
    if relu_chain is not None:
        raise RuntimeError("relu_chain: conv '%s' left the own-kernel route after its producer was told it would fold the ReLU derivative" % name)
    return None, _conv(x, P, name, stride, pad, backend=backend)


def _conv_into(x, P, name, stride, pad, blob, c0, backend):
    return backend.conv_mfma_relu(x, P[name + ".w"], P[name + ".b"], stride, pad, NEG_SLOPE, True, out=blob, out_c0=c0)


def _any_requires_grad(P) -> bool:
    vals = P.P.values() if isinstance(P, _Prefixed) else P.values()
    return any(v.requires_grad for v in vals)


def _stage_deconv(P, x, dname, blob, cs, cd, backend, allow_copy=True):
    d = backend.deconv_relu(x, P[dname + ".w"], P[dname + ".b"], NEG_SLOPE, True, out=blob, out_c0=cs) if hasattr(backend, "deconv_relu") else None
    if d is None and allow_copy:
        blob[:, cs:cs + cd].copy_(_deconv(x, P, dname, backend=backend))
    return d


def _refine_stage(P, skip, x, dname, flow, uname, backend):
    def up(t, name, out=None, out_c0=0):
        if backend is not None and hasattr(backend, "upsample_flow_deconv"):
            if out is not None:
                return backend.upsample_flow_deconv(t, P[name + ".w"], P[name + ".b"], out=out, out_c0=out_c0)
            return backend.upsample_flow_deconv(t, P[name + ".w"], P[name + ".b"])
        return _deconv(t, P, name, act=False)

    blob, s = skip if isinstance(skip, tuple) else (None, skip)
    if blob is None:
        return torch.cat([s, _deconv(x, P, dname, backend=backend), up(flow, uname)], 1)
    cs, cd = s.shape[1], P[dname + ".w"].shape[1]
    assert blob.shape[1] == cs + cd + 2
    stage_params = [P[n] for n in (dname + ".w", dname + ".b", uname + ".w", uname + ".b")]
    if torch.is_grad_enabled() and (s.requires_grad or x.requires_grad or flow.requires_grad or any(p.requires_grad for p in stage_params)):
        d = _stage_deconv(P, x, dname, blob, cs, cd, backend, allow_copy=False)
        u = up(flow, uname, out=blob, out_c0=cs + cd) if (d is not None and hasattr(backend, "upsample_flow_deconv")) else None
        if d is None or u is None:
            return torch.cat([s, _deconv(x, P, dname, backend=backend), up(flow, uname)], 1)
        part = lambda t, c0, c: t if t.requires_grad else blob[:, c0:c0 + c]
        return _ConcatInPlace.apply(blob, s, part(d, cs, cd), part(u, cs + cd, 2))
    _stage_deconv(P, x, dname, blob, cs, cd, backend)
    if hasattr(backend, "upsample_flow_deconv"):
        up(flow, uname, out=blob, out_c0=cs + cd)
    else:
        blob[:, cs + cd:].copy_(up(flow, uname))
    return blob


def _decoder(P, conv6_1, conv5_1, conv4_1, conv3_1, conv2, backend=None):
    def pf(x, name):
        if backend is not None and hasattr(backend, "predict_flow_conv"):
            return backend.predict_flow_conv(x, P[name + ".w"], P[name + ".b"])
        return _conv(x, P, name, 1, 1, act=False, backend=backend)

    def stage(skip, x, dname, flow, uname):
        return _refine_stage(P, skip, x, dname, flow, uname, backend)


    flow6 = pf(conv6_1, "Convolution1")
    c5 = stage(conv5_1, conv6_1, "deconv5", flow6, "upsample_flow6to5")
    flow5 = pf(c5, "Convolution2")
    c4 = stage(conv4_1, c5, "deconv4", flow5, "upsample_flow5to4")
    flow4 = pf(c4, "Convolution3")
    c3 = stage(conv3_1, c4, "deconv3", flow4, "upsample_flow4to3")
    flow3 = pf(c3, "Convolution4")
    c2 = stage(conv2, c3, "deconv2", flow3, "upsample_flow3to2")
    flow2 = pf(c2, "Convolution5")
    return {2: flow2, 3: flow3, 4: flow4, 5: flow5, 6: flow6}


def _skip_conv(x, P, name, stride, pad, dname, backend, relu_chain=None):
    return _conv_into_concat(x, P, name, stride, pad, P[dname + ".w"].shape[1] + 2, backend, relu_chain=relu_chain)


RELU_CHAIN = [True]


def _stem_chain(P, x, backend):
    if not (RELU_CHAIN[0] and CONCAT_IN_PLACE_TRAINING[0] and torch.is_grad_enabled() and x.is_cuda and hasattr(backend, "relu_chain_supported")
            and hasattr(backend, "conv_route_name")):
        return None, None
    w1, w2 = P["conv1.w"], P["conv2.w"]
    if not (w1.requires_grad and w2.requires_grad and P["conv1.b"].requires_grad) or x.requires_grad:
        return None, None
    if backend.conv_route_name(x.shape, w1, 2, 3) != "stem":
        return None, None
    c1_shape = (x.shape[0], w1.shape[0], (x.shape[2] - 1) // 2 + 1, (x.shape[3] - 1) // 2 + 1)
    if not backend.relu_chain_supported(c1_shape, w2, 2, 2):
        return None, None
    cell = {"masked": False, "slope": NEG_SLOPE}
    return (1, cell), (2, cell)


CONCAT_IN_PLACE_TRAINING = [True]


class _ConcatInPlace(torch.autograd.Function):

    @staticmethod
    def forward(ctx, blob, *parts):
        ctx.cuts = [p.shape[1] for p in parts]
        assert sum(ctx.cuts) == blob.shape[1] and all(p.data_ptr() >= blob.data_ptr() for p in parts)
        return blob.view_as(blob)

    @staticmethod
    def backward(ctx, g):
        out, c0 = [None], 0
        for c in ctx.cuts:
            out.append(g[:, c0:c0 + c])
            c0 += c
        return tuple(out)


TOWER_SPLIT_OPS = [True]


class _SplitTowers(torch.autograd.Function):

    @staticmethod
    def forward(ctx, x):
        n = x.shape[0] // 2
        return x[:n], x[n:]

    @staticmethod
    def backward(ctx, ga, gb):
        return torch.cat([ga, gb], 0)


class _StackedAndFirstTower(torch.autograd.Function):

    @staticmethod
    def forward(ctx, x):
        return x.view_as(x), x[:x.shape[0] // 2]

    @staticmethod
    def backward(ctx, g_all, g_first):
        if g_all._base is not None or not g_all.is_contiguous():
            g_all = g_all.clone(memory_format=torch.contiguous_format)
        g_all[:g_first.shape[0]].add_(g_first)
        return g_all


def flownet_c_core(P, img0, img1, backend, towers=None):
    x = towers if towers is not None else torch.cat([img0, img1], 0)
    n = x.shape[0] // 2
    chain1, chain2 = _stem_chain(P, x, backend)
    c1 = _conv(x, P, "conv1", 2, 3, backend=backend, relu_chain=chain1)
    blob2, c2 = _skip_conv(c1, P, "conv2", 2, 2, "deconv2", backend, relu_chain=chain2)
    training = TOWER_SPLIT_OPS[0] and torch.is_grad_enabled() and c2.requires_grad
    c2_first = None
    if training:
        c2, c2_first = _StackedAndFirstTower.apply(c2)
    c3 = _conv(c2, P, "conv3", 2, 2, backend=backend)
    c3a, c3b = _SplitTowers.apply(c3) if (training and c3.requires_grad) else (c3[:n], c3[n:])
    cat = redir = None
    cr = P["conv_redir.w"].shape[0]
    if hasattr(backend, "correlation_relu_into") and c3a.is_cuda:
        cat = torch.empty((n, cr + 441, c3a.shape[2], c3a.shape[3]), device=c3a.device, dtype=c3a.dtype)
        in_graph = (CONCAT_IN_PLACE_TRAINING[0] and torch.is_grad_enabled() and (c3a.requires_grad or c3b.requires_grad)
                    and hasattr(backend, "conv_backward"))
        if in_graph:
            redir = _conv_into(c3a, P, "conv_redir", 1, 0, cat, 0, backend)
            corr = backend.correlation_relu_into(c3a, c3b, cat, cr, NEG_SLOPE, pad=20, kernel_size=1, max_displacement=20, stride_1=1, stride_2=2,
                                                 training=True)
            if redir is not None and redir.requires_grad:
                cat = _ConcatInPlace.apply(cat, redir, corr)
            else:
                cat = torch.cat([_conv(c3a, P, "conv_redir", 1, 0, backend=backend), corr], 1)
        elif backend.correlation_relu_into(c3a, c3b, cat, cr, NEG_SLOPE, pad=20, kernel_size=1, max_displacement=20,
                                           stride_1=1, stride_2=2) is None:
            cat = None
        else:
            into = None
            if hasattr(backend, "conv_mfma_relu") and not (torch.is_grad_enabled() and _any_requires_grad(P)):
                into = backend.conv_mfma_relu(c3a, P["conv_redir.w"], P["conv_redir.b"], 1, 0, NEG_SLOPE, True, out=cat, out_c0=0)
            if into is None:
                cat[:, :cr].copy_(_conv(c3a, P, "conv_redir", 1, 0, backend=backend))
    if cat is None:
        redir = _conv(c3a, P, "conv_redir", 1, 0, backend=backend)
        corr = backend.correlation(c3a, c3b, pad=20, kernel_size=1, max_displacement=20, stride_1=1, stride_2=2)
        cat = torch.cat([redir, F.leaky_relu(corr, NEG_SLOPE)], 1)
    blob3, c31 = _skip_conv(cat, P, "conv3_1", 1, 1, "deconv3", backend)
    c4 = _conv(c31, P, "conv4", 2, 1, backend=backend)
    blob4, c41 = _skip_conv(c4, P, "conv4_1", 1, 1, "deconv4", backend)
    c5 = _conv(c41, P, "conv5", 2, 1, backend=backend)
    blob5, c51 = _skip_conv(c5, P, "conv5_1", 1, 1, "deconv5", backend)
    c6 = _conv(c51, P, "conv6", 2, 1, backend=backend)
    c61 = _conv(c6, P, "conv6_1", 1, 1, backend=backend)
    c2s = c2_first if c2_first is not None else c2[:n]
    skip2 = (blob2[:n], c2s) if blob2 is not None else c2s
    return _decoder(P, c61, (blob5, c51), (blob4, c41), (blob3, c31), skip2, backend)


def flownet_s_core(P, x, backend=None):
    c1 = _conv(x, P, "conv1", 2, 3, backend=backend)
    blob2, c2 = _skip_conv(c1, P, "conv2", 2, 2, "deconv2", backend)
    c3 = _conv(c2, P, "conv3", 2, 2, backend=backend)
    blob3, c31 = _skip_conv(c3, P, "conv3_1", 1, 1, "deconv3", backend)
    c4 = _conv(c31, P, "conv4", 2, 1, backend=backend)
    blob4, c41 = _skip_conv(c4, P, "conv4_1", 1, 1, "deconv4", backend)
    c5 = _conv(c41, P, "conv5", 2, 1, backend=backend)
    blob5, c51 = _skip_conv(c5, P, "conv5_1", 1, 1, "deconv5", backend)
    c6 = _conv(c51, P, "conv6", 2, 1, backend=backend)
    c61 = _conv(c6, P, "conv6_1", 1, 1, backend=backend)
    return _decoder(P, c61, (blob5, c51), (blob4, c41), (blob3, c31), (blob2, c2), backend)


def adapted_size(h: int, w: int, divisor: int = 64):
    return int(math.ceil(h / divisor) * divisor), int(math.ceil(w / divisor) * divisor)


def deploy_forward(kind: str, P, img0, img1, backend, mean: Optional[torch.Tensor] = None):
    N, _, H, W = img0.shape
    ah, aw = adapted_size(H, W)
    neg_default = mean is None
    if mean is None:
        mean = _const(img0.device, (0.411, 0.433, 0.45))
    if (ah, aw) == (H, W) and img0.is_cuda and not torch.is_grad_enabled() and hasattr(backend, "scale_shift"):
        neg_mean = _const(img0.device, (-0.411, -0.433, -0.45)) if neg_default else (-mean).contiguous()
        if kind == "C":
            x = torch.empty((2 * N, 3, H, W), device=img0.device, dtype=torch.float32)
            backend.scale_shift(img0, 1.0 / 255.0, neg_mean, out=x[:N])
            backend.scale_shift(img1, 1.0 / 255.0, neg_mean, out=x[N:])
            flows = flownet_c_core(P, None, None, backend, towers=x)
        else:
            x = torch.empty((N, 6, H, W), device=img0.device, dtype=torch.float32)
            backend.scale_shift(img0, 1.0 / 255.0, neg_mean, out=x, out_c0=0)
            backend.scale_shift(img1, 1.0 / 255.0, neg_mean, out=x, out_c0=3)
            flows = flownet_s_core(P, x, backend)
    else:
        pre = []
        for im in (img0, img1):
            x = im * (1.0 / 255.0)
            if (ah, aw) != (H, W):
                x = backend.resample(x, ah, aw)
            pre.append(x - mean.view(1, 3, 1, 1))
        if kind == "C":
            flows = flownet_c_core(P, pre[0], pre[1], backend)
        else:
            flows = flownet_s_core(P, torch.cat(pre, 1), backend)
    if img0.is_cuda and not torch.is_grad_enabled() and hasattr(backend, "resample_slices"):
        flow = backend.resample_slices(flows[2], H, W, in_scale=FLOW_SCALE)
        if (ah, aw) == (H, W):
            return flow
    else:
        flow = flows[2] * FLOW_SCALE
        flow = backend.resample(flow, H, W)
    scale = _const(flow.device, (W / float(aw), H / float(ah)))
    return flow * scale.view(1, 2, 1, 1)


def loss_targets_ahead(gt_flow, backend, divisors=None):
    if not (hasattr(backend, "downsample_ahead") and gt_flow.is_cuda):
        return None
    H, W = gt_flow.shape[2], gt_flow.shape[3]
    divisors = divisors or {s: 2 ** s for s in LOSS_WEIGHTS}
    gt = gt_flow * (1.0 / FLOW_SCALE)
    sizes = [(H // divisors[s], W // divisors[s]) for s in LOSS_WEIGHTS]
    tgts, ev = backend.downsample_ahead(gt, sizes)
    return {"targets": dict(zip(LOSS_WEIGHTS, tgts)), "event": ev, "sizes": dict(zip(LOSS_WEIGHTS, sizes))}


FINAL_FLOW_GT_SCALE = {"SD": 1.0 / SD_FLOW_SCALE, "fusion": 1.0}


def final_flow_loss(flow, gt_flow, backend, scale):
    tgt = backend.downsample(gt_flow * scale, flow.shape[2], flow.shape[3])
    return backend.l1_loss(flow, tgt, l2_per_location=True, normalize_by_num_entries=True)


def multiscale_loss(flows, gt_flow, backend, targets=None):
    if hasattr(backend, "l1_loss_multi") and gt_flow.is_cuda:
        scales = list(LOSS_WEIGHTS.items())
        preds = [flows[s] for s, _ in scales]
        if targets is not None and all(tuple(targets["sizes"][s]) == tuple(flows[s].shape[2:]) for s, _ in scales):
            backend.wait_ahead(targets["event"])
            tgts = [targets["targets"][s] for s, _ in scales]
        else:
            gt = gt_flow * (1.0 / FLOW_SCALE)
            tgts = [backend.downsample(gt, p.shape[2], p.shape[3]) for p in preds]
        return backend.l1_loss_multi(preds, tgts, [w for _, w in scales], l2_per_location=True, normalize_by_num_entries=True)[0]
    gt = gt_flow * (1.0 / FLOW_SCALE)
    total = 0.0
    for s, w in LOSS_WEIGHTS.items():
        pred = flows[s]
        tgt = backend.downsample(gt, pred.shape[2], pred.shape[3])
        total = total + w * backend.l1_loss(pred, tgt, l2_per_location=True, normalize_by_num_entries=True)
    return total


def conv_flops(kind: str, h: int, w: int, in_channels: int = 6) -> float:
    fl = 0.0
    size = {}
    hh, ww = h, w
    res = {"conv1": 2, "conv2": 4, "conv3": 8, "conv_redir": 8, "conv3_1": 8, "conv4": 16, "conv4_1": 16, "conv5": 32, "conv5_1": 32,
           "conv6": 64, "conv6_1": 64, "Convolution1": 64, "deconv5": 32, "upsample_flow6to5": 32, "Convolution2": 32,
           "deconv4": 16, "upsample_flow5to4": 16, "Convolution3": 16, "deconv3": 8, "upsample_flow4to3": 8, "Convolution4": 8,
           "deconv2": 4, "upsample_flow3to2": 4, "Convolution5": 4}
    for (name, k, ci, co, ks, s, p) in layer_table(kind, in_channels):
        oh, ow = hh // res[name], ww // res[name]
        macs = oh * ow * co * ci * ks * ks if k == "conv" else (oh // 2) * (ow // 2) * ci * co * ks * ks
        mult = 2 if (kind == "C" and name in ("conv1", "conv2", "conv3")) else 1
        fl += 2.0 * macs * mult
    return fl


_SD_TABLE = [("conv0", "conv", 6, 64, 3, 1, 1), ("conv1", "conv", 64, 64, 3, 2, 1), ("conv1_1", "conv", 64, 128, 3, 1, 1),
             ("conv2", "conv", 128, 128, 3, 2, 1), ("conv2_1", "conv", 128, 128, 3, 1, 1), ("conv3", "conv", 128, 256, 3, 2, 1),
             ("conv3_1", "conv", 256, 256, 3, 1, 1), ("conv4", "conv", 256, 512, 3, 2, 1), ("conv4_1", "conv", 512, 512, 3, 1, 1),
             ("conv5", "conv", 512, 512, 3, 2, 1), ("conv5_1", "conv", 512, 512, 3, 1, 1), ("conv6", "conv", 512, 1024, 3, 2, 1),
             ("conv6_1", "conv", 1024, 1024, 3, 1, 1),
             ("Convolution1", "conv", 1024, 2, 3, 1, 1), ("deconv5", "deconv", 1024, 512, 4, 2, 1), ("upsample_flow6to5", "deconv", 2, 2, 4, 2, 1),
             ("interconv5", "conv", 1026, 512, 3, 1, 1), ("Convolution2", "conv", 512, 2, 3, 1, 1),
             ("deconv4", "deconv", 1026, 256, 4, 2, 1), ("upsample_flow5to4", "deconv", 2, 2, 4, 2, 1),
             ("interconv4", "conv", 770, 256, 3, 1, 1), ("Convolution3", "conv", 256, 2, 3, 1, 1),
             ("deconv3", "deconv", 770, 128, 4, 2, 1), ("upsample_flow4to3", "deconv", 2, 2, 4, 2, 1),
             ("interconv3", "conv", 386, 128, 3, 1, 1), ("Convolution4", "conv", 128, 2, 3, 1, 1),
             ("deconv2", "deconv", 386, 64, 4, 2, 1), ("upsample_flow3to2", "deconv", 2, 2, 4, 2, 1),
             ("interconv2", "conv", 194, 64, 3, 1, 1), ("Convolution5", "conv", 64, 2, 3, 1, 1)]
_FUSE_TABLE = [("conv0", "conv", 11, 64, 3, 1, 1), ("conv1", "conv", 64, 64, 3, 2, 1), ("conv1_1", "conv", 64, 128, 3, 1, 1),
               ("conv2", "conv", 128, 128, 3, 2, 1), ("conv2_1", "conv", 128, 128, 3, 1, 1),
               ("Convolution5", "conv", 128, 2, 3, 1, 1), ("deconv1", "deconv", 128, 32, 4, 2, 1), ("upsample_flow2to1", "deconv", 2, 2, 4, 2, 1),
               ("interconv1", "conv", 162, 32, 3, 1, 1), ("Convolution6", "conv", 32, 2, 3, 1, 1),
               ("deconv0", "deconv", 162, 16, 4, 2, 1), ("upsample_flow1to0", "deconv", 2, 2, 4, 2, 1),
               ("interconv0", "conv", 82, 16, 3, 1, 1), ("Convolution7", "conv", 16, 2, 3, 1, 1)]


_SD_RES = {"conv0": 1, "conv1": 2, "conv1_1": 2, "conv2": 4, "conv2_1": 4, "conv3": 8, "conv3_1": 8, "conv4": 16, "conv4_1": 16, "conv5": 32,
           "conv5_1": 32, "conv6": 64, "conv6_1": 64, "Convolution1": 64, "deconv5": 32, "upsample_flow6to5": 32, "interconv5": 32,
           "Convolution2": 32, "deconv4": 16, "upsample_flow5to4": 16, "interconv4": 16, "Convolution3": 16, "deconv3": 8,
           "upsample_flow4to3": 8, "interconv3": 8, "Convolution4": 8, "deconv2": 4, "upsample_flow3to2": 4, "interconv2": 4, "Convolution5": 4}
_FUSE_RES = {"conv0": 1, "conv1": 2, "conv1_1": 2, "conv2": 4, "conv2_1": 4, "Convolution5": 4, "deconv1": 2, "upsample_flow2to1": 2,
             "interconv1": 2, "Convolution6": 2, "deconv0": 1, "upsample_flow1to0": 1, "interconv0": 1, "Convolution7": 1}


def _table_flops(table, res, h, w):
    fl = 0.0
    for (name, k, ci, co, ks, s, p) in table:
        oh, ow = h // res[name], w // res[name]
        fl += 2.0 * (oh * ow * co * ci * ks * ks if k == "conv" else (oh // 2) * (ow // 2) * ci * co * ks * ks)
    return fl


def flownet2_conv_flops(h: int, w: int) -> float:
    return conv_flops("C", h, w) + 2 * conv_flops("S", h, w, 12) + _table_flops(_SD_TABLE, _SD_RES, h, w) + _table_flops(_FUSE_TABLE, _FUSE_RES, h, w)


def _init_table(table, prefix, g, params, device):
    for (name, k, ci, co, ks, s, p) in table:
        shape = (co, ci, ks, ks) if k == "conv" else (ci, co, ks, ks)
        fan_in = ci * ks * ks if k == "conv" else ci * ks * ks / (s * s)
        std = math.sqrt(2.0 / ((1 + NEG_SLOPE ** 2) * fan_in))
        if name.startswith("Convolution"):
            std *= 0.5
        if name.startswith("upsample_flow"):
            std = 0.25
        params[prefix + name + ".w"] = (torch.randn(shape, generator=g) * std).to(device)
        params[prefix + name + ".b"] = torch.zeros(co).to(device)


def init_params_flownet2(seed: int = 0, device="cpu") -> Dict[str, torch.Tensor]:
    g = torch.Generator().manual_seed(seed)
    P: Dict[str, torch.Tensor] = {}
    _init_table(layer_table("C"), "", g, P, device)
    _init_table(layer_table("S", 12), "net2_", g, P, device)
    _init_table(layer_table("S", 12), "net3_", g, P, device)
    _init_table(_SD_TABLE, "netsd_", g, P, device)
    _init_table(_FUSE_TABLE, "fuse_", g, P, device)
    return P


class _Prefixed(dict):

    def __init__(self, P, prefix):
        super().__init__()
        self.P, self.prefix = P, prefix

    def __getitem__(self, k):
        return self.P[self.prefix + k]


def _pf(P, x, name, backend):
    if backend is not None and hasattr(backend, "predict_flow_conv"):
        return backend.predict_flow_conv(x, P[name + ".w"], P[name + ".b"])
    return _conv(x, P, name, 1, 1, act=False, backend=backend)


def flownet_sd_core(P, x, backend):
    c0 = _conv(x, P, "conv0", 1, 1, backend=backend)
    c1 = _conv(_conv(c0, P, "conv1", 2, 1, backend=backend), P, "conv1_1", 1, 1, backend=backend)
    blob2, c2 = _conv_into_concat(_conv(c1, P, "conv2", 2, 1, backend=backend), P, "conv2_1", 1, 1, 64 + 2, backend)
    blob3, c3 = _conv_into_concat(_conv(c2, P, "conv3", 2, 1, backend=backend), P, "conv3_1", 1, 1, 128 + 2, backend)
    blob4, c4 = _skip_conv(_conv(c3, P, "conv4", 2, 1, backend=backend), P, "conv4_1", 1, 1, "deconv4", backend)
    blob5, c5 = _skip_conv(_conv(c4, P, "conv5", 2, 1, backend=backend), P, "conv5_1", 1, 1, "deconv5", backend)
    c6 = _conv(_conv(c5, P, "conv6", 2, 1, backend=backend), P, "conv6_1", 1, 1, backend=backend)
    flow6 = _pf(P, c6, "Convolution1", backend)
    cat5 = _refine_stage(P, (blob5, c5), c6, "deconv5", flow6, "upsample_flow6to5", backend)
    flow5 = _pf(P, _conv(cat5, P, "interconv5", 1, 1, act=False, backend=backend), "Convolution2", backend)
    cat4 = _refine_stage(P, (blob4, c4), cat5, "deconv4", flow5, "upsample_flow5to4", backend)
    flow4 = _pf(P, _conv(cat4, P, "interconv4", 1, 1, act=False, backend=backend), "Convolution3", backend)
    cat3 = _refine_stage(P, (blob3, c3), cat4, "deconv3", flow4, "upsample_flow4to3", backend)
    flow3 = _pf(P, _conv(cat3, P, "interconv3", 1, 1, act=False, backend=backend), "Convolution4", backend)
    cat2 = _refine_stage(P, (blob2, c2), cat3, "deconv2", flow3, "upsample_flow3to2", backend)
    return _pf(P, _conv(cat2, P, "interconv2", 1, 1, act=False, backend=backend), "Convolution5", backend)


def fusion_core(P, x, backend):
    blob0, c0 = _conv_into_concat(x, P, "conv0", 1, 1, 16 + 2, backend)
    blob1, c1 = _conv_into_concat(_conv(c0, P, "conv1", 2, 1, backend=backend), P, "conv1_1", 1, 1, 32 + 2, backend)
    c2 = _conv(_conv(c1, P, "conv2", 2, 1, backend=backend), P, "conv2_1", 1, 1, backend=backend)
    flow2 = _pf(P, c2, "Convolution5", backend)
    cat1 = _refine_stage(P, (blob1, c1), c2, "deconv1", flow2, "upsample_flow2to1", backend)
    flow1 = _pf(P, _conv(cat1, P, "interconv1", 1, 1, act=False, backend=backend), "Convolution6", backend)
    cat0 = _refine_stage(P, (blob0, c0), cat1, "deconv0", flow1, "upsample_flow1to0", backend)
    return _pf(P, _conv(cat0, P, "interconv0", 1, 1, act=False, backend=backend), "Convolution7", backend)


def flownet2_deploy_forward(P, img0, img1, backend, mean: Optional[torch.Tensor] = None):
    N, _, H, W = img0.shape
    ah, aw = adapted_size(H, W)
    neg_mean = _const(img0.device, (-0.411, -0.433, -0.45)) if mean is None else (-mean).contiguous()
    if mean is None:
        mean = _const(img0.device, (0.411, 0.433, 0.45))
    if img0.is_cuda and not torch.is_grad_enabled() and hasattr(backend, "resample_slices"):
        return _flownet2_pick_streams(P, img0, img1, backend, neg_mean)
    if (ah, aw) == (H, W) and img0.is_cuda and not torch.is_grad_enabled() and hasattr(backend, "scale_shift"):
        a = backend.scale_shift(img0, 1.0 / 255.0, neg_mean)
        b = backend.scale_shift(img1, 1.0 / 255.0, neg_mean)
    else:
        a = backend.resample(img0 * (1.0 / 255.0), ah, aw) - mean.view(1, 3, 1, 1)
        b = backend.resample(img1 * (1.0 / 255.0), ah, aw) - mean.view(1, 3, 1, 1)

    def refine_input(flow_q):
        flow = backend.resample(flow_q * FLOW_SCALE, ah, aw)
        warped = backend.flow_warp(b, flow)
        err = backend.channel_norm(a - warped)
        return flow, warped, err

    flow1_q = flownet_c_core(P, a, b, backend)[2]
    f1, w1, e1 = refine_input(flow1_q)
    flow2_q = flownet_s_core(_Prefixed(P, "net2_"), torch.cat([a, b, w1, f1 * (1.0 / FLOW_SCALE), e1], 1), backend)[2]
    f2, w2, e2 = refine_input(flow2_q)
    flow3_q = flownet_s_core(_Prefixed(P, "net3_"), torch.cat([a, b, w2, f2 * (1.0 / FLOW_SCALE), e2], 1), backend)[2]
    flow_css = backend.resample(flow3_q * FLOW_SCALE, ah, aw, type=1)
    flow_sd = backend.resample(flownet_sd_core(_Prefixed(P, "netsd_"), torch.cat([a, b], 1), backend) * SD_FLOW_SCALE, ah, aw, type=1)
    err_css = backend.channel_norm(a - backend.flow_warp(b, flow_css))
    err_sd = backend.channel_norm(a - backend.flow_warp(b, flow_sd))
    fuse_in = torch.cat([a, flow_sd, flow_css, backend.channel_norm(flow_sd), backend.channel_norm(flow_css), err_sd, err_css], 1)
    flow = fusion_core(_Prefixed(P, "fuse_"), fuse_in, backend)
    flow = backend.resample(flow, H, W)
    scale = _const(flow.device, (W / float(aw), H / float(ah)))
    return flow * scale.view(1, 2, 1, 1)


_SD_STREAM = {"mode": "auto", "streams": {}, "picked": {}}


def set_sd_side_stream(mode="auto"):
    _SD_STREAM["mode"] = {True: "on", False: "off"}.get(mode, mode)
    _SD_STREAM["picked"] = {}


def _flownet2_pick_streams(P, img0, img1, backend, neg_mean):
    import time
    mode = _SD_STREAM["mode"]
    run = lambda side: _flownet2_deploy_forward_slices(P, img0, img1, backend, neg_mean, side)
    if mode != "auto":
        return run(mode == "on")
    key = (img0.device, tuple(img0.shape))
    st = _SD_STREAM["picked"].get(key)
    if isinstance(st, bool):
        return run(st)
    if torch.cuda.is_current_stream_capturing():
        return run(True)
    if st is None:
        st = _SD_STREAM["picked"][key] = {"n": 0, True: [], False: []}
    n = st["n"]
    st["n"] += 1
    if n == 0:
        return run(True)
    side = n % 2 == 1
    torch.cuda.synchronize(img0.device)
    t0 = time.perf_counter()
    out = run(side)
    torch.cuda.synchronize(img0.device)
    st[side].append(time.perf_counter() - t0)
    if n >= 4:
        _SD_STREAM["picked"][key] = min(st[True]) <= 1.01 * min(st[False])
        _SD_STREAM.setdefault("timings_ms", {})[key] = {"second_stream": round(min(st[True]) * 1e3, 4), "one_stream": round(min(st[False]) * 1e3, 4)}
    return out


def sd_side_stream_timings():
    return dict(_SD_STREAM.get("timings_ms", {}))


def sd_side_stream_picks():
    return {k: v for k, v in _SD_STREAM["picked"].items() if isinstance(v, bool)}


def _sd_side_stream(dev, on):
    if not on:
        return None
    st = _SD_STREAM["streams"].get(dev)
    if st is None:
        st = _SD_STREAM["streams"][dev] = torch.cuda.Stream(device=dev)
    return st


def _flownet2_deploy_forward_slices(P, img0, img1, backend, neg_mean, sd_beside=True):
    N, _, H, W = img0.shape
    ah, aw = adapted_size(H, W)
    dev = img0.device
    new = lambda c: torch.empty((N, c, ah, aw), device=dev, dtype=torch.float32)
    towers = torch.empty((2 * N, 3, ah, aw), device=dev, dtype=torch.float32)
    blob = new(12)
    pair = new(6)
    fuse = new(11)
    for k, img in enumerate((img0, img1)):
        if (ah, aw) == (H, W):
            src, s = img, 1.0 / 255.0
        else:
            src, s = backend.resample_slices(img, ah, aw, in_scale=1.0 / 255.0), 1.0
        backend.scale_shift(src, s, neg_mean, out=towers[k * N:(k + 1) * N])
        backend.scale_shift(src, s, neg_mean, out=blob, out_c0=3 * k)
        backend.scale_shift(src, s, neg_mean, out=pair, out_c0=3 * k)
        if k == 0:
            backend.scale_shift(src, s, neg_mean, out=fuse, out_c0=0)
    A, B, WARPED = (blob, 0, 3), (blob, 3, 3), (blob, 6, 3)

    def refine_input(flow_q):
        flow = backend.resample_slices(flow_q, ah, aw, in_scale=FLOW_SCALE, out2=(blob, 9, 2), out2_scale=1.0 / FLOW_SCALE)
        backend.flow_warp_slices(B, flow, out=WARPED)
        backend.channel_norm_slices(A, minus=WARPED, out=(blob, 11, 1))

    side = _sd_side_stream(dev, sd_beside)
    sd_q = None
    if side is not None:
        main = torch.cuda.current_stream(dev)
        side.wait_stream(main)
        with torch.cuda.stream(side):
            sd_q = flownet_sd_core(_Prefixed(P, "netsd_"), pair, backend)
    flow1_q = flownet_c_core(P, None, None, backend, towers=towers)[2]
    refine_input(flow1_q)
    flow2_q = flownet_s_core(_Prefixed(P, "net2_"), blob, backend)[2]
    refine_input(flow2_q)
    flow3_q = flownet_s_core(_Prefixed(P, "net3_"), blob, backend)[2]
    if side is not None:
        main.wait_stream(side)
        sd_q.record_stream(main)
    else:
        sd_q = flownet_sd_core(_Prefixed(P, "netsd_"), pair, backend)
    backend.resample_slices(sd_q, ah, aw, type=1, in_scale=SD_FLOW_SCALE, out=(fuse, 3, 2))
    backend.resample_slices(flow3_q, ah, aw, type=1, in_scale=FLOW_SCALE, out=(fuse, 5, 2))
    backend.channel_norm_slices((fuse, 3, 2), out=(fuse, 7, 1))
    backend.channel_norm_slices((fuse, 5, 2), out=(fuse, 8, 1))
    backend.flow_warp_slices(B, (fuse, 3, 2), out=WARPED)
    backend.channel_norm_slices(A, minus=WARPED, out=(fuse, 9, 1))
    backend.flow_warp_slices(B, (fuse, 5, 2), out=WARPED)
    backend.channel_norm_slices(A, minus=WARPED, out=(fuse, 10, 1))
    flow = fusion_core(_Prefixed(P, "fuse_"), fuse, backend)
    if (ah, aw) == (H, W):
        return flow
    flow = backend.resample(flow, H, W)
    scale = _const(flow.device, (W / float(aw), H / float(ah)))
    return flow * scale.view(1, 2, 1, 1)
```

### flownet2_amd/ops.py

```python
from __future__ import annotations

import ctypes as C

import torch

from . import _lib
from ._lib import CorrParams, L1LossParams, check

MULTIPLY, SUBTRACT = 0, 1
FILL_ZERO, FILL_NAN = 1, 2
NEAREST, LINEAR, CUBIC, AREA = 1, 2, 3, 4


def _stream():
    return C.c_void_p(torch.cuda.current_stream().cuda_stream)


def _chk(t: torch.Tensor, name: str, ndim: int = 4):
    if not isinstance(t, torch.Tensor) or not t.is_cuda:
        raise ValueError(f"{name}: expected a CUDA (HIP) tensor; flownet2_amd has no CPU path")
    if t.dtype != torch.float32:
        raise ValueError(f"{name}: expected float32 (Dtype=float), got {t.dtype}")
    if ndim is not None and t.dim() != ndim:
        raise ValueError(f"{name}: expected {ndim} axes (NCHW), got shape {tuple(t.shape)}")
    return t.contiguous()


def _ptr(t):
    return C.c_void_p(t.data_ptr()) if t is not None else C.c_void_p(0)


def corr_params(pad=0, kernel_size=1, max_displacement=0, stride_1=1, stride_2=1, correlation_type=MULTIPLY, do_abs=False,
                single_direction=0):
    return CorrParams(int(pad), int(kernel_size), int(max_displacement), int(stride_1), int(stride_2),
                      int(correlation_type), int(bool(do_abs)), int(single_direction))


def correlation_out_shape(p: CorrParams, Cc: int, H: int, W: int):
    tc, th, tw = C.c_int(), C.c_int(), C.c_int()
    check(_lib.lib().fn2_correlation_out_shape(C.byref(p), Cc, H, W, C.byref(tc), C.byref(th), C.byref(tw)))
    return tc.value, th.value, tw.value


def correlation_forward(p: CorrParams, bottom0: torch.Tensor, bottom1: torch.Tensor, out: torch.Tensor | None = None,
                        out_c0: int = 0, relu: bool = False, negative_slope: float = 0.0):
    b0, b1 = _chk(bottom0, "bottom[0]"), _chk(bottom1, "bottom[1]")
    if b0.shape != b1.shape:
        raise ValueError("Both bottom blobs must have same shape")
    N, Cc, H, W = b0.shape
    tc, th, tw = correlation_out_shape(p, Cc, H, W)
    top = out if out is not None else torch.empty((N, tc, th, tw), device=b0.device, dtype=torch.float32)
    assert top.is_contiguous() and top.shape[0] == N and tuple(top.shape[2:]) == (th, tw) and out_c0 + tc <= top.shape[1]
    if not relu and out_c0 == 0 and top.shape[1] == tc:
        check(_lib.lib().fn2_correlation_forward(C.byref(p), _ptr(b0), _ptr(b1), _ptr(top), N, Cc, H, W, None, 0, _stream()))
    else:
        check(_lib.lib().fn2_correlation_forward_fused(C.byref(p), _ptr(b0), _ptr(b1), _ptr(top), N, Cc, H, W, int(top.shape[1]), int(out_c0),
                                                       int(bool(relu)), C.c_float(float(negative_slope)), None, 0, _stream()))
    return top


def correlation_backward(p: CorrParams, bottom0, bottom1, top_diff, need0=True, need1=True):
    b0, b1, td = _chk(bottom0, "bottom[0]"), _chk(bottom1, "bottom[1]"), _chk(top_diff, "top.diff")
    N, Cc, H, W = b0.shape
    d0 = torch.empty_like(b0) if need0 else None
    d1 = torch.empty_like(b1) if need1 else None
    check(_lib.lib().fn2_correlation_backward(C.byref(p), _ptr(b0), _ptr(b1), _ptr(td), _ptr(d0), _ptr(d1),
                                              N, Cc, H, W, None, 0, _stream()))
    return d0, d1


def correlation1d_out_shape(p: CorrParams, Cc: int, H: int, W: int):
    tc, th, tw = C.c_int(), C.c_int(), C.c_int()
    check(_lib.lib().fn2_correlation1d_out_shape(C.byref(p), Cc, H, W, C.byref(tc), C.byref(th), C.byref(tw)))
    return tc.value, th.value, tw.value


def correlation1d_forward(p: CorrParams, bottom0: torch.Tensor, bottom1: torch.Tensor):
    b0, b1 = _chk(bottom0, "bottom[0]"), _chk(bottom1, "bottom[1]")
    if b0.shape != b1.shape:
        raise ValueError("Both bottom blobs must have same shape")
    N, Cc, H, W = b0.shape
    tc, th, tw = correlation1d_out_shape(p, Cc, H, W)
    top = torch.empty((N, tc, th, tw), device=b0.device, dtype=torch.float32)
    check(_lib.lib().fn2_correlation1d_forward(C.byref(p), _ptr(b0), _ptr(b1), _ptr(top), N, Cc, H, W, _stream()))
    return top


def correlation1d_backward(p: CorrParams, bottom0, bottom1, top_diff, need0=True, need1=True):
    b0, b1, td = _chk(bottom0, "bottom[0]"), _chk(bottom1, "bottom[1]"), _chk(top_diff, "top.diff")
    N, Cc, H, W = b0.shape
    d0 = torch.empty_like(b0) if need0 else None
    d1 = torch.empty_like(b1) if need1 else None
    check(_lib.lib().fn2_correlation1d_backward(C.byref(p), _ptr(b0), _ptr(b1), _ptr(td), _ptr(d0), _ptr(d1), N, Cc, H, W, _stream()))
    return d0, d1


def set_correlation_impl(impl):
    check(_lib.lib().fn2_debug_set_correlation_impl(int(impl)))


def set_resample_generic(on):
    check(_lib.lib().fn2_debug_set_resample_generic(int(bool(on))))


def flow_warp_forward(image, flow, fill_value=FILL_ZERO):
    im, fl = _chk(image, "bottom[0] (image)"), _chk(flow, "bottom[1] (flow)")
    N, Cc, H, W = im.shape
    if fl.shape[0] != N:
        raise ValueError("Num of the inputs should be the same")
    if fl.shape[1] != 2:
        raise ValueError("Flow should have 2 channels: x-flow and y-flow")
    if fl.shape[3] != W or fl.shape[2] != H:
        raise ValueError("Width/Height of the inputs should be the same")
    out = torch.empty_like(im)
    check(_lib.lib().fn2_flow_warp_forward(_ptr(im), _ptr(fl), _ptr(out), N, Cc, H, W, int(fill_value), _stream()))
    return out


def _as_slice(arg, what):
    if isinstance(arg, tuple):
        blob, c0, Cc = arg
        if isinstance(blob, torch.Tensor) and not blob.is_contiguous():
            raise ValueError(what + ": a sliced blob must be contiguous")
        blob = _chk(blob, what)
        if c0 < 0 or Cc < 1 or c0 + Cc > blob.shape[1]:
            raise ValueError("%s: channel slice [%d, %d) outside a blob of %d channels" % (what, c0, c0 + Cc, blob.shape[1]))
        return blob, int(blob.shape[1]), int(c0), int(Cc)
    t = _chk(arg, what)
    return t, int(t.shape[1]), 0, int(t.shape[1])


def flow_warp_forward_slices(image, flow, out=None, fill_value=FILL_ZERO):
    im, ictot, ic0, Cc = _as_slice(image, "bottom[0] (image)")
    fl, fctot, fc0, Cf = _as_slice(flow, "bottom[1] (flow)")
    N, _, H, W = im.shape
    if fl.shape[0] != N or Cf != 2 or tuple(fl.shape[2:]) != (H, W):
        raise ValueError("flow_warp: flow must be [N,2,H,W] of the image's size")
    if out is None:
        out = torch.empty((N, Cc, H, W), device=im.device, dtype=torch.float32)
    top, octot, oc0, Co = _as_slice(out, "top[0]")
    if Co != Cc or top.shape[0] != N or tuple(top.shape[2:]) != (H, W):
        raise ValueError("flow_warp: top slice does not match the image")
    check(_lib.lib().fn2_flow_warp_forward_slices(_ptr(im), ictot, ic0, _ptr(fl), fctot, fc0, _ptr(top), octot, oc0, N, Cc, H, W, int(fill_value), _stream()))
    return top


def flow_warp_backward(image, flow, warped_diff, propagate_image=True, propagate_flow=True):
    im, fl, wd = _chk(image, "image"), _chk(flow, "flow"), _chk(warped_diff, "top.diff")
    N, Cc, H, W = im.shape
    di, df = torch.empty_like(im), torch.empty_like(fl)
    nbytes = _lib.lib().fn2_flow_warp_backward_workspace_bytes(N, Cc, H, W)
    ws = torch.empty(nbytes, dtype=torch.uint8, device=im.device)
    check(_lib.lib().fn2_flow_warp_backward(_ptr(im), _ptr(fl), _ptr(wd), _ptr(di), _ptr(df), N, Cc, H, W,
                                            int(propagate_image), int(propagate_flow), _ptr(ws), nbytes, _stream()))
    return di, df


def resample_forward(x, height, width, type=LINEAR, antialias=True):
    x = _chk(x, "bottom[0]")
    N, Cc, H, W = x.shape
    if height < 1 or width < 1:
        raise ValueError("ResampleLayer must have top_height > 0 and top_width > 0")
    out = torch.empty((N, Cc, int(height), int(width)), device=x.device, dtype=torch.float32)
    check(_lib.lib().fn2_resample_forward(_ptr(x), _ptr(out), N, Cc, H, W, int(height), int(width), int(type), int(bool(antialias)), _stream()))
    return out


def resample_forward_slices(x, height, width, type=LINEAR, antialias=True, in_scale=1.0, out=None, out2=None, out2_scale=1.0):
    x = _chk(x, "bottom[0]")
    N, Cc, H, W = x.shape
    if height < 1 or width < 1:
        raise ValueError("ResampleLayer must have top_height > 0 and top_width > 0")
    if out is None:
        out = torch.empty((N, Cc, int(height), int(width)), device=x.device, dtype=torch.float32)
    top, octot, oc0, Co = _as_slice(out, "top[0]")
    if Co != Cc or top.shape[0] != N or tuple(top.shape[2:]) != (int(height), int(width)):
        raise ValueError("resample: top slice does not match")
    t2, o2ctot, o2c0 = None, 0, 0
    if out2 is not None:
        t2, o2ctot, o2c0, C2 = _as_slice(out2, "top[1]")
        if C2 != Cc or t2.shape[0] != N or tuple(t2.shape[2:]) != (int(height), int(width)):
            raise ValueError("resample: second top slice does not match")
    check(_lib.lib().fn2_resample_forward_slices(_ptr(x), C.c_float(float(in_scale)), _ptr(top), octot, oc0, _ptr(t2), o2ctot, o2c0,
                                                 C.c_float(float(out2_scale)), N, Cc, H, W, int(height), int(width), int(type),
                                                 int(bool(antialias)), _stream()))
    return top


def l1_params(l2_per_location=False, l2_prescale_by_channels=False, normalize_by_num_entries=False, epsilon=1e-2, plateau=0.0):
    return L1LossParams(int(bool(l2_per_location)), int(bool(l2_prescale_by_channels)), int(bool(normalize_by_num_entries)),
                        float(epsilon), float(plateau))


def l1loss_workspace(x: torch.Tensor) -> torch.Tensor:
    N, Cc, H, W = x.shape
    nbytes = _lib.lib().fn2_l1loss_workspace_bytes(N, Cc, H, W)
    return torch.empty(nbytes, dtype=torch.uint8, device=x.device)


def l1loss_forward(p: L1LossParams, bottom0, bottom1=None, workspace=None):
    b0 = _chk(bottom0, "bottom[0]")
    b1 = _chk(bottom1, "bottom[1]") if bottom1 is not None else None
    if b1 is not None and b1.shape != b0.shape:
        raise ValueError("L1Loss: bottom blobs must have the same shape")
    N, Cc, H, W = b0.shape
    ws = workspace if workspace is not None else l1loss_workspace(b0)
    loss = torch.empty((), device=b0.device, dtype=torch.float32)
    check(_lib.lib().fn2_l1loss_forward(C.byref(p), _ptr(b0), _ptr(b1), _ptr(loss), N, Cc, H, W, _ptr(ws), ws.numel(), _stream()))
    return loss, ws


def l1loss_backward(p: L1LossParams, bottom0, bottom1, top_diff: float, workspace):
    b0 = _chk(bottom0, "bottom[0]")
    b1 = _chk(bottom1, "bottom[1]") if bottom1 is not None else None
    N, Cc, H, W = b0.shape
    d0 = torch.empty_like(b0)
    d1 = torch.empty_like(b0) if b1 is not None else None
    check(_lib.lib().fn2_l1loss_backward(C.byref(p), _ptr(b0), _ptr(b1), C.c_float(float(top_diff)), _ptr(d0), _ptr(d1),
                                         N, Cc, H, W, _ptr(workspace), workspace.numel(), _stream()))
    return d0, d1


_L1_SYNC = {}


def _l1_scales(bottoms0, bottoms1, weights, diffs0=None, diffs1=None):
    n = len(bottoms0)
    arr = (_lib.L1LossScale * n)()
    for k in range(n):
        b0 = _chk(bottoms0[k], "bottom[0]")
        b1 = _chk(bottoms1[k], "bottom[1]") if bottoms1 is not None and bottoms1[k] is not None else None
        if b1 is not None and b1.shape != b0.shape:
            raise ValueError("L1Loss: bottom blobs must have the same shape")
        N, Cc, H, W = b0.shape
        arr[k].bottom0, arr[k].bottom1 = b0.data_ptr(), (b1.data_ptr() if b1 is not None else None)
        arr[k].bottom0_diff = diffs0[k].data_ptr() if diffs0 is not None else None
        arr[k].bottom1_diff = diffs1[k].data_ptr() if diffs1 is not None and diffs1[k] is not None else None
        arr[k].N, arr[k].C, arr[k].H, arr[k].W = N, Cc, H, W
        arr[k].loss_weight = float(weights[k])
    return arr


def l1loss_forward_multi(p: L1LossParams, bottoms0, bottoms1, weights):
    n = len(bottoms0)
    dev = bottoms0[0].device
    ws = torch.empty(int(_lib.lib().fn2_l1loss_multi_workspace_bytes(n)), dtype=torch.uint8, device=dev)
    key = (dev.index, int(torch.cuda.current_stream().cuda_stream))
    sync = _L1_SYNC.get(key)
    if sync is None:
        sync = _L1_SYNC[key] = torch.zeros(int(_lib.lib().fn2_l1loss_multi_sync_bytes()), dtype=torch.uint8, device=dev)
    losses = torch.empty((n,), device=dev, dtype=torch.float32)
    total = torch.empty((), device=dev, dtype=torch.float32)
    arr = _l1_scales(bottoms0, bottoms1, weights)
    check(_lib.lib().fn2_l1loss_forward_multi(C.byref(p), n, arr, _ptr(losses), _ptr(total), _ptr(ws), ws.numel(), _ptr(sync), _stream()))
    return total, losses, ws


def l1loss_backward_multi(p: L1LossParams, bottoms0, bottoms1, weights, total_diff, workspace, need1=False):
    n = len(bottoms0)
    d0 = [torch.empty_like(b) for b in bottoms0]
    d1 = [torch.empty_like(b) if (need1 and bottoms1 is not None and bottoms1[k] is not None) else None for k, b in enumerate(bottoms0)]
    arr = _l1_scales(bottoms0, bottoms1, weights, d0, d1)
    td = _chk(total_diff.reshape(1), "total_diff", ndim=1) if total_diff is not None else None
    check(_lib.lib().fn2_l1loss_backward_multi(C.byref(p), n, arr, _ptr(td), _ptr(workspace), workspace.numel(), _stream()))
    return d0, d1


def channel_norm_forward(x):
    x = _chk(x, "bottom[0]")
    N, Cc, H, W = x.shape
    out = torch.empty((N, 1, H, W), device=x.device, dtype=torch.float32)
    check(_lib.lib().fn2_channel_norm_forward(_ptr(x), _ptr(out), N, Cc, H, W, _stream()))
    return out


def channel_norm_forward_slices(x, minus=None, out=None):
    b, bctot, bc0, Cc = _as_slice(x, "bottom[0]")
    N, _, H, W = b.shape
    m, mctot, mc0 = None, 0, 0
    if minus is not None:
        m, mctot, mc0, Cm = _as_slice(minus, "bottom[1]")
        if Cm != Cc or tuple(m.shape[2:]) != (H, W) or m.shape[0] != N:
            raise ValueError("channel_norm: the subtrahend does not match the bottom")
    if out is None:
        out = torch.empty((N, 1, H, W), device=b.device, dtype=torch.float32)
    top, tctot, tc0, Ct = _as_slice(out, "top[0]")
    if Ct != 1 or top.shape[0] != N or tuple(top.shape[2:]) != (H, W):
        raise ValueError("channel_norm: top slice must be one channel of the bottom's size")
    check(_lib.lib().fn2_channel_norm_forward_slices(_ptr(b), bctot, bc0, _ptr(m), mctot, mc0, _ptr(top), tctot, tc0, N, Cc, H, W, _stream()))
    return top


def channel_norm_backward(x, top, top_diff):
    x, top, td = _chk(x, "bottom[0]"), _chk(top, "top"), _chk(top_diff, "top.diff")
    N, Cc, H, W = x.shape
    d = torch.empty_like(x)
    check(_lib.lib().fn2_channel_norm_backward(_ptr(x), _ptr(top), _ptr(td), _ptr(d), N, Cc, H, W, _stream()))
    return d


def downsample_forward(x, top_height, top_width):
    x = _chk(x, "bottom[0]")
    N, Cc, H, W = x.shape
    if top_height < 1 or top_width < 1:
        raise ValueError("DownsampleLayer must have top_height > 0 and top_width > 0")
    out = torch.empty((N, Cc, int(top_height), int(top_width)), device=x.device, dtype=torch.float32)
    check(_lib.lib().fn2_downsample_forward(_ptr(x), _ptr(out), N, Cc, H, W, int(top_height), int(top_width), _stream()))
    return out


def downsample_forward_multi(x, sizes):
    x = _chk(x, "bottom[0]")
    N, Cc, H, W = x.shape
    sizes = [(int(h), int(w)) for h, w in sizes]
    outs = [torch.empty((N, Cc, h, w), device=x.device, dtype=torch.float32) for h, w in sizes]
    n = len(sizes)
    ptrs = (C.c_void_p * n)(*[_ptr(o) for o in outs])
    hs, ws = (C.c_int * n)(*[h for h, _ in sizes]), (C.c_int * n)(*[w for _, w in sizes])
    check(_lib.lib().fn2_downsample_forward_multi(_ptr(x), ptrs, hs, ws, n, N, Cc, H, W, _stream()))
    return outs


def downsample_multi_supported(x_shape, sizes) -> bool:
    H, W = int(x_shape[2]), int(x_shape[3])
    return 1 <= len(sizes) <= 8 and all(int(h) >= 2 and int(w) >= 2 and (int(h), int(w)) != (H, W) for h, w in sizes)


def predict_flow_conv_forward(x, weight, bias=None):
    x, w = _chk(x, "bottom[0]"), _chk(weight, "weight")
    N, Cc, H, W = x.shape
    if tuple(w.shape) != (2, Cc, 3, 3):
        raise ValueError(f"predict_flow weight must be [2,{Cc},3,3], got {tuple(w.shape)}")
    b = _chk(bias, "bias", ndim=1) if bias is not None else None
    out = torch.empty((N, 2, H, W), device=x.device, dtype=torch.float32)
    nbytes = _lib.lib().fn2_predict_flow_conv_workspace_bytes(N, Cc, H, W)
    ws = torch.empty(nbytes, dtype=torch.uint8, device=x.device) if nbytes else None
    check(_lib.lib().fn2_predict_flow_conv_forward(_ptr(x), _ptr(w), _ptr(b), _ptr(out), N, Cc, H, W, _ptr(ws), nbytes, _stream()))
    return out


def upsample_flow_deconv_forward(x, weight, bias=None, out=None, out_c0=0):
    x, w = _chk(x, "bottom[0]"), _chk(weight, "weight")
    N, Cc, H, W = x.shape
    if Cc != 2 or tuple(w.shape) != (2, 2, 4, 4):
        raise ValueError("upsample_flow expects a 2-channel flow and a [2,2,4,4] weight")
    b = _chk(bias, "bias", ndim=1) if bias is not None else None
    if out is not None:
        _chk(out, "top[0]")
        if out.shape[0] != N or tuple(out.shape[2:]) != (2 * H, 2 * W):
            raise ValueError(f"upsample_flow: top blob {tuple(out.shape)} does not match [{N},*,{2 * H},{2 * W}]")
        check(_lib.lib().fn2_upsample_flow_deconv_forward_into(_ptr(x), _ptr(w), _ptr(b), _ptr(out), N, H, W, out.shape[1], int(out_c0), _stream()))
        return out[:, out_c0:out_c0 + 2]
    out = torch.empty((N, 2, 2 * H, 2 * W), device=x.device, dtype=torch.float32)
    check(_lib.lib().fn2_upsample_flow_deconv_forward(_ptr(x), _ptr(w), _ptr(b), _ptr(out), N, H, W, _stream()))
    return out


def bias_leaky_relu_(x, bias=None, negative_slope=0.1):
    if not (isinstance(x, torch.Tensor) and x.is_cuda and x.dtype == torch.float32 and x.dim() == 4 and x.is_contiguous()):
        raise ValueError("bias_leaky_relu_: expected a contiguous float32 CUDA (HIP) NCHW tensor")
    N, Cc, H, W = x.shape
    b = _chk(bias, "bias", ndim=1) if bias is not None else None
    if b is not None and b.numel() != Cc:
        raise ValueError(f"bias must have {Cc} entries, got {b.numel()}")
    check(_lib.lib().fn2_bias_leaky_relu_forward(_ptr(x), _ptr(b), N, Cc, H, W, C.c_float(float(negative_slope)), _stream()))
    return x


def scale_shift_forward(x, scale, shift=None, out=None, out_c0=0):
    x = _chk(x, "bottom[0]")
    N, Cc, H, W = x.shape
    if out is None:
        out = torch.empty_like(x)
    else:
        _chk(out, "top[0]")
        if out.shape[0] != N or tuple(out.shape[2:]) != (H, W):
            raise ValueError("scale_shift: top blob does not match the bottom")
    s = _chk(shift, "shift", ndim=1) if shift is not None else None
    check(_lib.lib().fn2_scale_shift_forward(_ptr(x), _ptr(out), _ptr(s), N, Cc, H, W, out.shape[1], out_c0, C.c_float(float(scale)), _stream()))
    return out


def predict_flow_conv_backward_supported(N, C, H, W) -> bool:
    return bool(_lib.lib().fn2_predict_flow_conv_backward_supported(int(N), int(C), int(H), int(W)))


def predict_flow_conv_backward(x, weight, top_diff, need_x=True, need_w=True, need_b=True):
    xb, xctot, xc0, Cc = _as_slice(x, "bottom[0]")
    w, g = _chk(weight, "weight"), _chk(top_diff, "top.diff")
    N, _, H, W = xb.shape
    if tuple(w.shape) != (2, Cc, 3, 3) or tuple(g.shape) != (N, 2, H, W):
        raise ValueError("predict_flow_conv_backward: weight must be [2,C,3,3] and top_diff [N,2,H,W]")
    dx = torch.empty((N, Cc, H, W), device=g.device, dtype=torch.float32) if need_x else None
    dw = torch.empty_like(w) if need_w else None
    db = torch.empty(2, device=g.device, dtype=torch.float32) if need_b else None
    nbytes = _lib.lib().fn2_predict_flow_conv_backward_workspace_bytes(N, Cc, H, W) if (need_w or need_b) else 0
    ws = torch.empty(max(nbytes, 4), dtype=torch.uint8, device=g.device)
    check(_lib.lib().fn2_predict_flow_conv_backward(_ptr(xb), xctot, xc0, _ptr(w), _ptr(g), _ptr(dx), _ptr(dw), _ptr(db), N, Cc, H, W, 0,
                                                    _ptr(ws), nbytes, _stream()))
    return dx, dw, db


def upsample_flow_deconv_backward(x, weight, top_diff, need_x=True, need_w=True, need_b=True):
    x, w, g = _chk(x, "bottom[0]"), _chk(weight, "weight"), _chk(top_diff, "top.diff")
    N, Cc, H, W = x.shape
    if Cc != 2 or tuple(w.shape) != (2, 2, 4, 4) or tuple(g.shape) != (N, 2, 2 * H, 2 * W):
        raise ValueError("upsample_flow_deconv_backward: bottom [N,2,H,W], weight [2,2,4,4], top_diff [N,2,2H,2W]")
    dx = torch.empty_like(x) if need_x else None
    dw = torch.empty_like(w) if need_w else None
    db = torch.empty(2, device=g.device, dtype=torch.float32) if need_b else None
    nbytes = _lib.lib().fn2_upsample_flow_deconv_backward_workspace_bytes(N, H, W) if (need_w or need_b) else 0
    ws = torch.empty(max(nbytes, 4), dtype=torch.uint8, device=g.device)
    check(_lib.lib().fn2_upsample_flow_deconv_backward(_ptr(x), _ptr(w), _ptr(g), _ptr(dx), _ptr(dw), _ptr(db), N, H, W, 0, _ptr(ws), nbytes, _stream()))
    return dx, dw, db


def conv_k7s2_relu_supported(Cin, Hin, Win, Cout) -> bool:
    return bool(_lib.lib().fn2_conv_k7s2_relu_supported(int(Cin), int(Hin), int(Win), int(Cout)))


def conv_k7s2_wgrad_supported(N, Cin, Hin, Win, Cout) -> bool:
    return bool(_lib.lib().fn2_conv_k7s2_wgrad_supported(int(N), int(Cin), int(Hin), int(Win), int(Cout)))


def conv_k7s2_wgrad_ksplit(N, Cin, Hin, Win, Cout) -> int:
    return int(_lib.lib().fn2_conv_k7s2_wgrad_ksplit(int(N), int(Cin), int(Hin), int(Win), int(Cout)))


def conv_k7s2_wgrad(top_diff, bottom):
    d, x = _chk(top_diff, "top.diff"), _chk(bottom, "bottom[0]")
    N, Cin, H, W = x.shape
    Cout = d.shape[1]
    if tuple(d.shape) != (N, Cout, (H - 1) // 2 + 1, (W - 1) // 2 + 1):
        raise ValueError(f"conv_k7s2_wgrad: top_diff {tuple(d.shape)} does not belong to a bottom of {tuple(x.shape)}")
    dw = torch.empty((Cout, Cin, 7, 7), device=x.device, dtype=torch.float32)
    need = int(_lib.lib().fn2_conv_k7s2_wgrad_workspace_bytes(N, Cin, H, W, Cout))
    ws = _plane_workspace(x.device, need) if need else None
    check(_lib.lib().fn2_conv_k7s2_wgrad(_ptr(d), _ptr(x), _ptr(dw), N, Cin, H, W, Cout, 0, _ptr(ws), need, _stream()))
    return dw


def conv_k7s2_relu_forward(x, weight, bias=None, negative_slope=0.1):
    x, w = _chk(x, "bottom[0]"), _chk(weight, "weight")
    N, Cin, H, W = x.shape
    Cout = w.shape[0]
    if tuple(w.shape) != (Cout, Cin, 7, 7):
        raise ValueError(f"stem weight must be [Cout,{Cin},7,7], got {tuple(w.shape)}")
    b = _chk(bias, "bias", ndim=1) if bias is not None else None
    out = torch.empty((N, Cout, (H - 1) // 2 + 1, (W - 1) // 2 + 1), device=x.device, dtype=torch.float32)
    check(_lib.lib().fn2_conv_k7s2_relu_forward(_ptr(x), _ptr(w), _ptr(b), _ptr(out), N, Cin, H, W, Cout,
                                                C.c_float(float(negative_slope)), _stream()))
    return out


CONV_ROUTE_NONE, CONV_ROUTE_DIRECT, CONV_ROUTE_WINOGRAD, CONV_ROUTE_PLANE, CONV_ROUTE_STEM, CONV_ROUTE_HEAD = range(6)
DECONV_ROUTE_NONE, DECONV_ROUTE_GEMM, DECONV_ROUTE_PLANE, DECONV_ROUTE_HEAD = range(4)
CONV_FWD_ROUTES = {0: None, 1: "direct", 2: "wino", 3: "plane", 4: "stem", 5: "head"}
DECONV_FWD_ROUTES = {0: None, 1: "gemm", 2: "plane", 3: "head"}
CONV_ROUTES = {0: None, 1: "direct", 2: "wino", 3: "plane", 4: None, 5: None}
DECONV_ROUTES = {0: None, 1: "gemm", 2: "plane", 3: None}


def conv_route(N, Cin, Hin, Win, Cout, kernel, stride, pad, force=False):
    return CONV_ROUTES[conv_forward_route(conv_desc(N, Cin, Hin, Win, Cout, kernel, stride, pad), force)]


def deconv_route(N, Cin, Hin, Win, Cout, kernel=4, stride=2, pad=1):
    return DECONV_ROUTES[deconv_forward_route(conv_desc(N, Cin, Hin, Win, Cout, kernel, stride, pad))]


BWD_ROUTES = {0: None, 1: "wino", 2: "tconv", 3: "plane", 4: "direct", 5: "deconv_plane"}


def conv_desc(N, Cin, Hin, Win, Cout, kernel, stride, pad):
    return _lib.ConvDesc(int(N), int(Cin), int(Hin), int(Win), int(Cout), int(kernel), int(stride), int(pad))


def conv_forward_route(desc, force=False) -> int:
    return int(_lib.lib().fn2_conv_route(C.byref(desc), 1 if force else 0))


def deconv_forward_route(desc) -> int:
    return int(_lib.lib().fn2_deconv_route(C.byref(desc), 0))


def conv_pack_weights(weight, desc, route, transposed=False):
    w = _chk(weight, "weight")
    L = _lib.lib()
    floats, pack = (L.fn2_deconv_packed_weight_floats, L.fn2_deconv_pack_weights) if transposed else (L.fn2_conv_packed_weight_floats, L.fn2_conv_pack_weights)
    n = int(floats(C.byref(desc), int(route)))
    k = desc.kernel
    if n == 0 or tuple(w.shape) != ((desc.Cin, desc.Cout, k, k) if transposed else (desc.Cout, desc.Cin, k, k)):
        raise ValueError("conv_pack_weights: route %d has no operand for a weight of shape %s" % (route, tuple(w.shape)))
    packed = torch.empty(n, device=w.device, dtype=torch.float32)
    check(pack(C.byref(desc), int(route), _ptr(w), _ptr(packed), _stream()))
    return packed


def conv_forward(x, packed, bias, desc, route, transposed=False, relu=True, negative_slope=0.1, out=None, out_c0=0, in_c0=0):
    x = _chk(x, "bottom[0]")
    N, Ctot, H, W = x.shape
    k, s, p = desc.kernel, desc.stride, desc.pad
    if (N, H, W) != (desc.N, desc.Hin, desc.Win) or in_c0 < 0 or in_c0 + desc.Cin > Ctot:
        raise ValueError(f"conv_forward: bottom blob {tuple(x.shape)} does not hold the layer's [{desc.N},{desc.Cin},{desc.Hin},{desc.Win}] at channel {in_c0}")
    Ho, Wo = (2 * H, 2 * W) if transposed else ((H + 2 * p - k) // s + 1, (W + 2 * p - k) // s + 1)
    if out is None:
        out = torch.empty((N, desc.Cout, Ho, Wo), device=x.device, dtype=torch.float32)
    else:
        _chk(out, "top[0]")
        if not out.is_contiguous() or out.shape[0] != N or tuple(out.shape[2:]) != (Ho, Wo) or out_c0 < 0 or out_c0 + desc.Cout > out.shape[1]:
            raise ValueError(f"conv_forward: top blob {tuple(out.shape)} does not match [{N},>={out_c0 + desc.Cout},{Ho},{Wo}]")
    b = _chk(bias, "bias", ndim=1) if bias is not None else None
    pw = _chk(packed, "packed weight", ndim=None)
    L = _lib.lib()
    if pw.numel() != int((L.fn2_deconv_packed_weight_floats if transposed else L.fn2_conv_packed_weight_floats)(C.byref(desc), int(route))):
        raise ValueError("conv_forward: the operand has %d floats, not what route %d reads for this layer" % (pw.numel(), route))
    need = int((L.fn2_deconv_workspace_bytes if transposed else L.fn2_conv_workspace_bytes)(C.byref(desc), int(route)))
    if transposed and route == DECONV_ROUTE_GEMM:
        ws = torch.empty((need + 3) // 4, device=x.device, dtype=torch.float32)
    else:
        ws = _plane_workspace(x.device, need) if need else None
    check((L.fn2_deconv_forward if transposed else L.fn2_conv_forward)(
        C.byref(desc), int(route), _ptr(x), Ctot, int(in_c0), _ptr(pw), _ptr(b), _ptr(out), out.shape[1], int(out_c0),
        int(bool(relu)), C.c_float(float(negative_slope)), _ptr(ws), need, _stream()))
    return out


def conv_backward_data_route(desc, transposed=False) -> int:
    return int(_lib.lib().fn2_conv_backward_data_route(C.byref(desc), int(bool(transposed))))


def conv_backward_data_pack_weights(weight, desc, transposed, route):
    w = _chk(weight, "weight")
    L, tr = _lib.lib(), int(bool(transposed))
    n = int(L.fn2_conv_backward_data_packed_weight_floats(C.byref(desc), tr, int(route)))
    if n == 0:
        raise ValueError("conv_backward_data_pack_weights: route %d is not this layer's" % route)
    packed = torch.empty(n, device=w.device, dtype=torch.float32)
    need = int(L.fn2_conv_backward_data_pack_workspace_bytes(C.byref(desc), tr, int(route)))
    ws = torch.empty(need // 4, device=w.device, dtype=torch.float32) if need else None
    check(L.fn2_conv_backward_data_pack_weights(C.byref(desc), tr, int(route), _ptr(w), _ptr(packed), _ptr(ws), need, _stream()))
    return packed


def conv_backward_data(top_diff, packed_weight, desc, transposed, route, top_c0=0):
    d = _chk(top_diff, "top_diff")
    L, tr = _lib.lib(), int(bool(transposed))
    Cp = int(L.fn2_conv_backward_data_computed_channels(C.byref(desc), tr, int(route)))
    if Cp == 0:
        raise ValueError("conv_backward_data: route %d is not this layer's" % route)
    out = torch.empty((desc.N, Cp, desc.Hin, desc.Win), device=d.device, dtype=torch.float32)
    need = int(L.fn2_conv_backward_data_workspace_bytes_with_room(C.byref(desc), tr, int(route), Cp))
    ws = _plane_workspace(d.device, need) if need else None
    check(L.fn2_conv_backward_data(C.byref(desc), tr, int(route), _ptr(d), d.shape[1], int(top_c0), _ptr(packed_weight), _ptr(out), Cp, 0, Cp,
                                   _ptr(ws), need, _stream()))
    return out[:, :desc.Cin] if Cp != desc.Cin else out


def conv_backward_weights_supported(desc, transposed=False) -> bool:
    return bool(_lib.lib().fn2_conv_backward_weights_supported(C.byref(desc), int(bool(transposed))))


def conv_backward_weights(bottom, top_diff, desc, transposed=False, out=None, accumulate=False, bottom_c0=0, top_c0=0):
    x, d = _chk(bottom, "bottom"), _chk(top_diff, "top_diff")
    L, tr = _lib.lib(), int(bool(transposed))
    k = desc.kernel
    shape = (desc.Cin, desc.Cout, k, k) if transposed else (desc.Cout, desc.Cin, k, k)
    if out is None:
        out = torch.empty(shape, device=x.device, dtype=torch.float32)
        accumulate = False
    else:
        out = _chk(out, "weight diff")
        if tuple(out.shape) != shape:
            raise ValueError("conv_backward_weights: weight diff has the wrong shape")
    need = int(L.fn2_conv_backward_weights_workspace_bytes(C.byref(desc), tr))
    ws = _plane_workspace(x.device, need) if need else None
    check(L.fn2_conv_backward_weights(C.byref(desc), tr, _ptr(x), x.shape[1], int(bottom_c0), _ptr(d), d.shape[1], int(top_c0), _ptr(out),
                                      int(bool(accumulate)), _ptr(ws), need, _stream()))
    return out


def conv_backward_data_masked_supported(desc, transposed, route) -> bool:
    return bool(_lib.lib().fn2_conv_backward_data_masked_supported(C.byref(desc), int(bool(transposed)), int(route)))


def conv_backward_data_masked(top_diff, packed, desc, transposed, route, bottom_data, negative_slope, top_c0=0, data_c0=0):
    d, y = _chk(top_diff, "top_diff"), _chk(bottom_data, "bottom data")
    out = torch.empty((desc.N, desc.Cin, desc.Hin, desc.Win), device=d.device, dtype=torch.float32)
    check(_lib.lib().fn2_conv_backward_data_masked(C.byref(desc), int(bool(transposed)), int(route), _ptr(d), d.shape[1], int(top_c0), _ptr(packed),
                                                   _ptr(out), desc.Cin, 0, _ptr(y), y.shape[1], int(data_c0), C.c_float(float(negative_slope)), _stream()))
    return out


def conv_backward_weights_bias_fused(desc, transposed=False) -> bool:
    return bool(_lib.lib().fn2_conv_backward_weights_bias_fused(C.byref(desc), int(bool(transposed))))


def conv_backward_weights_bias(bottom, top_diff, desc, transposed=False, out=None):
    x, d = _chk(bottom, "bottom"), _chk(top_diff, "top_diff")
    L, tr = _lib.lib(), int(bool(transposed))
    k = desc.kernel
    dw = out if out is not None else torch.empty((desc.Cout, desc.Cin, k, k), device=x.device, dtype=torch.float32)
    db = torch.empty(desc.Cout, device=x.device, dtype=torch.float32)
    need = int(L.fn2_conv_backward_weights_workspace_bytes(C.byref(desc), tr))
    ws = _plane_workspace(x.device, need) if need else None
    check(L.fn2_conv_backward_weights_bias(C.byref(desc), tr, _ptr(x), _ptr(d), _ptr(dw), _ptr(db), 0, _ptr(ws), need, _stream()))
    return dw, db


def conv_backward_bias(top_diff, C_, top_c0=0, out=None, accumulate=False):
    d = _chk(top_diff, "top_diff")
    N, Ctot, H, W = d.shape
    if out is None:
        out = torch.empty(C_, device=d.device, dtype=torch.float32)
        accumulate = False
    need = int(_lib.lib().fn2_bias_leaky_relu_backward_workspace_bytes(N, C_, H, W))
    ws = _plane_workspace(d.device, need)
    check(_lib.lib().fn2_conv_backward_bias(_ptr(d), Ctot, int(top_c0), _ptr(out), N, int(C_), H, W, int(bool(accumulate)), _ptr(ws), need, _stream()))
    return out


def conv_mfma_supported(Cin, Hin, Win, Cout, kernel, stride, pad) -> bool:
    return bool(_lib.lib().fn2_conv_mfma_supported(int(Cin), int(Hin), int(Win), int(Cout), int(kernel), int(stride), int(pad)))


def conv_mfma_pack_weights(weight):
    w = _chk(weight, "weight")
    Cout, Cin, k, k2 = w.shape
    n = _lib.lib().fn2_conv_mfma_packed_floats(Cout, Cin, k)
    if k != k2 or n == 0:
        raise ValueError(f"conv_mfma: unsupported weight shape {tuple(w.shape)}")
    packed = torch.empty(n, device=w.device, dtype=torch.float32)
    check(_lib.lib().fn2_conv_mfma_pack_weights(_ptr(w), _ptr(packed), Cout, Cin, k, _stream()))
    return packed


def conv_mfma_pack_weights_view(blob, Cout, Cin, kernel, src_cout, src_cin, stride_cout, stride_cin, flip=False):
    w = _chk(blob, "weight", ndim=blob.dim())
    if not w.is_contiguous():
        raise ValueError("conv_mfma_pack_weights_view: the blob itself must be contiguous (the view is described by the strides)")
    n = _lib.lib().fn2_conv_mfma_packed_floats(int(Cout), int(Cin), int(kernel))
    if n == 0:
        raise ValueError(f"conv_mfma: unsupported operand [{Cout},{Cin},{kernel},{kernel}]")
    last = (src_cout - 1) * stride_cout + (src_cin - 1) * stride_cin + kernel * kernel - 1
    if last >= w.numel():
        raise ValueError("conv_mfma_pack_weights_view: the view reaches beyond the blob")
    packed = torch.empty(n, device=w.device, dtype=torch.float32)
    check(_lib.lib().fn2_conv_mfma_pack_weights_view(_ptr(w), _ptr(packed), int(Cout), int(Cin), int(kernel), int(src_cout), int(src_cin),
                                                     int(stride_cout), int(stride_cin), int(bool(flip)), _stream()))
    return packed


def conv_mfma_forward(x, packed_weight, bias, Cout, kernel, stride, pad, relu=True, negative_slope=0.1, out=None, out_c0=0,
                      in_c0=0, Cin=None):
    x = _chk(x, "bottom[0]")
    N, Ctot, H, W = x.shape
    Cin = Ctot - in_c0 if Cin is None else Cin
    Ho, Wo = (H + 2 * pad - kernel) // stride + 1, (W + 2 * pad - kernel) // stride + 1
    if out is None:
        out = torch.empty((N, Cout, Ho, Wo), device=x.device, dtype=torch.float32)
    else:
        _chk(out, "top[0]")
        if out.shape[0] != N or tuple(out.shape[2:]) != (Ho, Wo):
            raise ValueError(f"conv_mfma: top blob {tuple(out.shape)} does not match [{N},*,{Ho},{Wo}]")
    b = _chk(bias, "bias", ndim=1) if bias is not None else None
    pw = _chk(packed_weight, "packed weight", ndim=1)
    check(_lib.lib().fn2_conv_mfma_forward(_ptr(x), _ptr(pw), _ptr(b), _ptr(out), N, Cin, H, W, Ctot, in_c0, Cout, out.shape[1], out_c0,
                                           kernel, stride, pad, int(bool(relu)), C.c_float(float(negative_slope)), _stream()))
    return out


def set_conv_variant(v: int):
    check(_lib.lib().fn2_debug_set_conv_variant(int(v)))


def conv_num_variants() -> int:
    return int(_lib.lib().fn2_conv_mfma_num_variants())


def conv_wino_supported(Cin, Hin, Win, Cout, pad) -> bool:
    return bool(_lib.lib().fn2_conv_wino_supported(int(Cin), int(Hin), int(Win), int(Cout), int(pad)))


def conv_wino_pack_weights(weight):
    w = _chk(weight, "weight")
    Cout, Cin, k, k2 = w.shape
    n = _lib.lib().fn2_conv_wino_packed_floats(Cout, Cin)
    if k != 3 or k2 != 3 or n == 0:
        raise ValueError(f"conv_wino: unsupported weight shape {tuple(w.shape)}")
    packed = torch.empty(n, device=w.device, dtype=torch.float32)
    check(_lib.lib().fn2_conv_wino_pack_weights(_ptr(w), _ptr(packed), Cout, Cin, _stream()))
    return packed


def conv_wino_forward(x, packed_weight, bias, Cout, pad=1, relu=True, negative_slope=0.1, out=None, out_c0=0, in_c0=0, Cin=None):
    x = _chk(x, "bottom[0]")
    N, Ctot, H, W = x.shape
    Cin = Ctot - in_c0 if Cin is None else Cin
    Ho, Wo = H + 2 * pad - 2, W + 2 * pad - 2
    if out is None:
        out = torch.empty((N, Cout, Ho, Wo), device=x.device, dtype=torch.float32)
    else:
        _chk(out, "top[0]")
        if out.shape[0] != N or tuple(out.shape[2:]) != (Ho, Wo):
            raise ValueError(f"conv_wino: top blob {tuple(out.shape)} does not match [{N},*,{Ho},{Wo}]")
    b = _chk(bias, "bias", ndim=1) if bias is not None else None
    pw = _chk(packed_weight, "packed weight", ndim=1)
    check(_lib.lib().fn2_conv_wino_forward(_ptr(x), _ptr(pw), _ptr(b), _ptr(out), N, Cin, H, W, Ctot, in_c0, Cout, out.shape[1], out_c0,
                                           pad, int(bool(relu)), C.c_float(float(negative_slope)), _stream()))
    return out


def conv_plane_supported(N, Cin, Hin, Win, Cout, stride, pad) -> bool:
    return bool(_lib.lib().fn2_conv_plane_supported(int(N), int(Cin), int(Hin), int(Win), int(Cout), int(stride), int(pad)))


def conv_plane_ksplit(N, Cin, Hin, Win, Cout, stride, pad) -> int:
    return int(_lib.lib().fn2_conv_plane_ksplit(int(N), int(Cin), int(Hin), int(Win), int(Cout), int(stride), int(pad)))


_PLANE_WS = {}
_PLANE_WS_RETIRED = []


def _plane_workspace(device, need):
    key = (device, int(torch.cuda.current_stream(device).cuda_stream))
    ws = _PLANE_WS.get(key)
    if ws is None or ws.numel() * 4 < need:
        if ws is not None:
            _PLANE_WS_RETIRED.append(ws)
        ws = _PLANE_WS[key] = torch.empty((need + 3) // 4, device=device, dtype=torch.float32)
    return ws


def conv_plane_k_supported(N, Cin, Hin, Win, Cout, kernel, stride, pad) -> bool:
    return bool(_lib.lib().fn2_conv_plane_k_supported(int(N), int(Cin), int(Hin), int(Win), int(Cout), int(kernel), int(stride), int(pad)))


def conv_plane_k_ksplit(N, Cin, Hin, Win, Cout, kernel, stride, pad) -> int:
    return int(_lib.lib().fn2_conv_plane_k_ksplit(int(N), int(Cin), int(Hin), int(Win), int(Cout), int(kernel), int(stride), int(pad)))


def conv_plane_forward(x, packed_weight, bias, Cout, stride, pad, relu=True, negative_slope=0.1, out=None, out_c0=0, in_c0=0, Cin=None, kernel=3):
    x = _chk(x, "bottom[0]")
    N, Ctot, H, W = x.shape
    Cin = Ctot - in_c0 if Cin is None else Cin
    Ho, Wo = (H + 2 * pad - kernel) // stride + 1, (W + 2 * pad - kernel) // stride + 1
    if out is None:
        out = torch.empty((N, Cout, Ho, Wo), device=x.device, dtype=torch.float32)
    else:
        _chk(out, "top[0]")
        if out.shape[0] != N or tuple(out.shape[2:]) != (Ho, Wo):
            raise ValueError(f"conv_plane: top blob {tuple(out.shape)} does not match [{N},*,{Ho},{Wo}]")
    b = _chk(bias, "bias", ndim=1) if bias is not None else None
    pw = _chk(packed_weight, "packed weight", ndim=1)
    need = int(_lib.lib().fn2_conv_plane_k_workspace_bytes(N, Cin, H, W, Cout, kernel, stride, pad))
    ws = _plane_workspace(x.device, need) if need else None
    check(_lib.lib().fn2_conv_plane_k_forward(_ptr(x), _ptr(pw), _ptr(b), _ptr(out), N, Cin, H, W, Ctot, in_c0, Cout, out.shape[1], out_c0,
                                              kernel, stride, pad, int(bool(relu)), C.c_float(float(negative_slope)),
                                              _ptr(ws if need else None), need, _stream()))
    return out


def tconv_supported(Cin, Hin, Win, Cout, Hout, Wout, kernel, pad) -> bool:
    return bool(_lib.lib().fn2_tconv_supported(int(Cin), int(Hin), int(Win), int(Cout), int(Hout), int(Wout), int(kernel), int(pad)))


def tconv_pack_weights(weight):
    w = weight.detach().contiguous()
    A, B, k, _ = w.shape
    return conv_mfma_pack_weights_view(w, B, A, k, B, A, k * k, B * k * k)


def tconv_forward(x, packed_weight, bias, Cout, kernel, pad, out_hw=None, relu=False, negative_slope=0.1, out=None, out_c0=0, in_c0=0, Cin=None):
    x = _chk(x, "bottom[0]")
    N, Ctot, H, W = x.shape
    Cin = Ctot - in_c0 if Cin is None else Cin
    Ho, Wo = out_hw if out_hw is not None else (2 * (H - 1) + kernel - 2 * pad, 2 * (W - 1) + kernel - 2 * pad)
    if out is None:
        out = torch.empty((N, Cout, Ho, Wo), device=x.device, dtype=torch.float32)
    else:
        _chk(out, "top[0]")
        if out.shape[0] != N or tuple(out.shape[2:]) != (Ho, Wo):
            raise ValueError(f"tconv: top blob {tuple(out.shape)} does not match [{N},*,{Ho},{Wo}]")
    b = _chk(bias, "bias", ndim=1) if bias is not None else None
    pw = _chk(packed_weight, "packed weight", ndim=1)
    check(_lib.lib().fn2_tconv_forward(_ptr(x), _ptr(pw), _ptr(b), _ptr(out), N, Cin, H, W, Ctot, in_c0, Cout, Ho, Wo, out.shape[1], out_c0,
                                       int(kernel), int(pad), int(bool(relu)), C.c_float(float(negative_slope)), _stream()))
    return out


def set_tconv_variant(v: int):
    check(_lib.lib().fn2_debug_set_tconv_variant(int(v)))


def tconv_num_variants() -> int:
    return int(_lib.lib().fn2_tconv_num_variants())


def conv_wgrad_supported(N, Ca, Ha, Wa, Cb, Hb, Wb, kernel, stride, pad) -> bool:
    return bool(_lib.lib().fn2_conv_wgrad_supported(int(N), int(Ca), int(Ha), int(Wa), int(Cb), int(Hb), int(Wb), int(kernel), int(stride), int(pad)))


def conv_wgrad_ksplit(N, Ca, Ha, Wa, Cb, Hb, Wb, kernel, stride, pad) -> int:
    return int(_lib.lib().fn2_conv_wgrad_ksplit(int(N), int(Ca), int(Ha), int(Wa), int(Cb), int(Hb), int(Wb), int(kernel), int(stride), int(pad)))


def conv_wgrad(a, b, kernel, stride, pad, out=None, accumulate=False, a_c0=0, Ca=None, b_c0=0, Cb=None):
    a, b = _chk(a, "a"), _chk(b, "b")
    N, Atot, Ha, Wa = a.shape
    Nb, Btot, Hb, Wb = b.shape
    if N != Nb:
        raise ValueError("conv_wgrad: batch sizes differ")
    Ca = Atot - a_c0 if Ca is None else Ca
    Cb = Btot - b_c0 if Cb is None else Cb
    if out is None:
        out = torch.empty((Ca, Cb, kernel, kernel), device=a.device, dtype=torch.float32)
        accumulate = False
    else:
        out = _chk(out, "weight diff")
        if tuple(out.shape) != (Ca, Cb, kernel, kernel):
            raise ValueError("conv_wgrad: weight diff has the wrong shape")
    need = int(_lib.lib().fn2_conv_wgrad_workspace_bytes(N, Ca, Ha, Wa, Cb, Hb, Wb, kernel, stride, pad))
    ws = _plane_workspace(a.device, need) if need else None
    check(_lib.lib().fn2_conv_wgrad(_ptr(a), _ptr(b), _ptr(out), N, Ca, Ha, Wa, Atot, a_c0, Cb, Hb, Wb, Btot, b_c0, int(kernel), int(stride), int(pad),
                                    int(bool(accumulate)), _ptr(ws), need, _stream()))
    return out


def deconv_plane_supported(N, Cin, Hin, Win, Cout) -> bool:
    return bool(_lib.lib().fn2_deconv_plane_supported(int(N), int(Cin), int(Hin), int(Win), int(Cout)))


def deconv_plane_ksplit(N, Cin, Hin, Win, Cout) -> int:
    return int(_lib.lib().fn2_deconv_plane_ksplit(int(N), int(Cin), int(Hin), int(Win), int(Cout)))


def deconv_plane_pack_weights(weight):
    w = _chk(weight, "weight")
    Cin, Cout, k, k2 = w.shape
    n = _lib.lib().fn2_deconv_plane_packed_floats(Cin, Cout)
    if k not in (3, 4) or k2 != k or n == 0:
        raise ValueError(f"deconv_plane: unsupported weight shape {tuple(w.shape)}")
    packed = torch.empty(n, device=w.device, dtype=torch.float32)
    check(_lib.lib().fn2_deconv_plane_pack_weights_k(_ptr(w), _ptr(packed), Cin, Cout, k, _stream()))
    return packed


def deconv_plane_forward(x, packed_weight, bias, Cout, relu=True, negative_slope=0.1, out=None, out_c0=0, in_c0=0, Cin=None):
    x = _chk(x, "bottom[0]")
    N, Ctot, H, W = x.shape
    Cin = Ctot - in_c0 if Cin is None else Cin
    if out is None:
        out = torch.empty((N, Cout, 2 * H, 2 * W), device=x.device, dtype=torch.float32)
    else:
        _chk(out, "top[0]")
        if out.shape[0] != N or tuple(out.shape[2:]) != (2 * H, 2 * W):
            raise ValueError(f"deconv_plane: top blob {tuple(out.shape)} does not match [{N},*,{2 * H},{2 * W}]")
    b = _chk(bias, "bias", ndim=1) if bias is not None else None
    pw = _chk(packed_weight, "packed weight", ndim=1)
    need = int(_lib.lib().fn2_deconv_plane_workspace_bytes(N, Cin, H, W, Cout))
    ws = _plane_workspace(x.device, need) if need else None
    check(_lib.lib().fn2_deconv_plane_forward(_ptr(x), _ptr(pw), _ptr(b), _ptr(out), N, Cin, H, W, Ctot, in_c0, Cout, out.shape[1], out_c0,
                                              int(bool(relu)), C.c_float(float(negative_slope)), _ptr(ws if need else None), need, _stream()))
    return out


def set_plane_variant(v: int):
    check(_lib.lib().fn2_debug_set_plane_variant(int(v)))


def set_plane_ksplit(k: int):
    check(_lib.lib().fn2_debug_set_plane_ksplit(int(k)))


def set_batch_invariant(on: bool):
    check(_lib.lib().fn2_set_batch_invariant(1 if on else 0))


def get_batch_invariant() -> bool:
    return bool(_lib.lib().fn2_get_batch_invariant())


def plane_num_variants() -> int:
    return int(_lib.lib().fn2_conv_plane_num_variants())


def set_wino_variant(v: int):
    check(_lib.lib().fn2_debug_set_wino_variant(int(v)))


def wino_num_variants() -> int:
    return int(_lib.lib().fn2_conv_wino_num_variants())


def im2col_forward(x, kernel, pad, stride):
    x = _chk(x, "bottom[0]")
    N, Cc, H, W = x.shape
    Hc, Wc = (H + 2 * pad - kernel) // stride + 1, (W + 2 * pad - kernel) // stride + 1
    col = torch.empty((N, Cc * kernel * kernel, Hc * Wc), device=x.device, dtype=torch.float32)
    check(_lib.lib().fn2_im2col_forward(_ptr(x), _ptr(col), N, Cc, H, W, int(kernel), int(pad), int(stride), _stream()))
    return col


def col2im_bias_relu_forward(col, bias, N, Cc, H, W, kernel, pad, stride, relu=True, negative_slope=0.1, out=None, out_c0=0):
    if not (col.is_cuda and col.dtype == torch.float32 and col.is_contiguous()):
        raise ValueError("col2im: expected a contiguous float32 CUDA (HIP) column blob")
    Hc, Wc = (H + 2 * pad - kernel) // stride + 1, (W + 2 * pad - kernel) // stride + 1
    if col.numel() != N * Cc * kernel * kernel * Hc * Wc:
        raise ValueError(f"col2im: column blob has {col.numel()} entries, expected {N * Cc * kernel * kernel * Hc * Wc}")
    b = _chk(bias, "bias", ndim=1) if bias is not None else None
    if out is not None:
        _chk(out, "top[0]")
        if out.shape[0] != N or tuple(out.shape[2:]) != (H, W):
            raise ValueError(f"col2im: top blob {tuple(out.shape)} does not match [{N},*,{H},{W}]")
        check(_lib.lib().fn2_col2im_bias_relu_forward_into(_ptr(col), _ptr(b), _ptr(out), N, Cc, H, W, int(kernel), int(pad), int(stride),
                                                           int(bool(relu)), C.c_float(float(negative_slope)), out.shape[1], int(out_c0), _stream()))
        return out[:, out_c0:out_c0 + Cc]
    out = torch.empty((N, Cc, H, W), device=col.device, dtype=torch.float32)
    check(_lib.lib().fn2_col2im_bias_relu_forward(_ptr(col), _ptr(b), _ptr(out), N, Cc, H, W, int(kernel), int(pad), int(stride),
                                                  int(bool(relu)), C.c_float(float(negative_slope)), _stream()))
    return out


def bias_leaky_relu_backward(top_data, top_diff, negative_slope=0.1, need_bias_diff=True):
    y, yctot, yc0, Cc = _as_slice(top_data, "top.data")
    g, gctot, gc0, gC = _as_slice(top_diff, "top.diff")
    N, _, H, W = y.shape
    if gC != Cc or g.shape[0] != N or tuple(g.shape[2:]) != (H, W):
        raise ValueError("top.data and top.diff must have the same shape")
    d = torch.empty((N, Cc, H, W), device=y.device, dtype=torch.float32)
    db = torch.empty(Cc, device=y.device, dtype=torch.float32) if need_bias_diff else None
    nbytes = _lib.lib().fn2_bias_leaky_relu_backward_workspace_bytes(N, Cc, H, W)
    ws = torch.empty(nbytes, dtype=torch.uint8, device=y.device)
    check(_lib.lib().fn2_bias_leaky_relu_backward_slices2(_ptr(y), yctot, yc0, _ptr(g), gctot, gc0, _ptr(d), _ptr(db), N, Cc, H, W,
                                                          C.c_float(float(negative_slope)), _ptr(ws), nbytes, _stream()))
    return d, db


AUG_NUM_PARAMS = 42


def augmentation_matrix(coeffs, crop_width, crop_height, bottom_width, bottom_height, invert=False):
    import numpy as np
    c = np.ascontiguousarray(coeffs, np.float32)
    if c.shape != (AUG_NUM_PARAMS,):
        raise ValueError(f"coefficient array must have {AUG_NUM_PARAMS} entries")
    out = np.empty(6, np.float32)
    check(_lib.lib().fn2_augmentation_matrix(C.c_void_p(c.ctypes.data), crop_width, crop_height, bottom_width, bottom_height, int(invert),
                                             C.c_void_p(out.ctypes.data)))
    return out


def flow_augmentation_forward(flow, coeffs1, coeffs2, crop_height, crop_width):
    import numpy as np
    fl = _chk(flow, "bottom[0] (flow)")
    N, Cc, H, W = fl.shape
    if Cc != 2:
        raise ValueError("Flow data must have two channels")
    host = []
    for c in (coeffs1, coeffs2):
        a = c.detach().cpu().numpy() if isinstance(c, torch.Tensor) else np.asarray(c)
        a = np.ascontiguousarray(a, np.float32).reshape(N, -1)
        if a.shape[1] != AUG_NUM_PARAMS:
            raise ValueError(f"coefficient blobs must hold {AUG_NUM_PARAMS} values per sample")
        host.append(a)
    top = torch.empty((N, 2, int(crop_height), int(crop_width)), device=fl.device, dtype=torch.float32)
    check(_lib.lib().fn2_flow_augmentation_forward(_ptr(fl), C.c_void_p(host[0].ctypes.data), C.c_void_p(host[1].ctypes.data), _ptr(top),
                                                   N, H, W, int(crop_height), int(crop_width), _stream()))
    return top


MEAN_NONE, MEAN_PER_CHANNEL, MEAN_PER_PIXEL = 0, 1, 2


def data_aug_params(crop_width=0, crop_height=0, max_multiplier=255.0, chromatic_eigvec=None, mean_mode=MEAN_NONE, noise_seed=0, noise_stream=0):
    p = _lib.DataAugParams(int(crop_width), int(crop_height), float(max_multiplier), int(chromatic_eigvec is not None))
    p.noise_seed, p.noise_stream = int(noise_seed), int(noise_stream)
    if chromatic_eigvec is not None:
        if len(chromatic_eigvec) != 9:
            raise ValueError("chromatic_eigvec must have 9 entries")
        p.chromatic_eigvec = (C.c_float * 9)(*[float(v) for v in chromatic_eigvec])
    p.mean_mode = int(mean_mode)
    return p


def data_augmentation_forward(p, bottom, coeffs=None, mean=None):
    import numpy as np
    x = _chk(bottom, "bottom[0]")
    N, Cc, H, W = x.shape
    crop = p.crop_width > 0 and p.crop_height > 0
    ch, cw = (p.crop_height, p.crop_width) if crop else (H, W)
    host = None
    if coeffs is not None:
        host = coeffs.detach().cpu().numpy() if isinstance(coeffs, torch.Tensor) else np.asarray(coeffs)
        host = np.ascontiguousarray(host, np.float32).reshape(N, -1)
        if host.shape[1] != AUG_NUM_PARAMS:
            raise ValueError(f"coefficient blob must hold {AUG_NUM_PARAMS} values per sample")
    m = None
    if p.mean_mode != MEAN_NONE:
        m = _chk(mean, "mean", ndim=None)
        want = Cc if p.mean_mode == MEAN_PER_CHANNEL else Cc * ch * cw
        if m.numel() != want:
            raise ValueError(f"mean: expected {want} values")
    top = torch.empty((N, Cc, max(ch, 0), max(cw, 0)), device=x.device, dtype=torch.float32)
    nws = _lib.lib().fn2_data_augmentation_workspace_bytes(N)
    ws = torch.empty(nws, device=x.device, dtype=torch.uint8)
    check(_lib.lib().fn2_data_augmentation_forward(C.byref(p), _ptr(x), C.c_void_p(host.ctypes.data) if host is not None else None, _ptr(m),
                                                   _ptr(top), N, Cc, H, W, _ptr(ws), nws, _stream()))
    return top
```

Baseline: 3521.

## Fuse input normalization into stem conv and predict_flow with flow upsampling

Adds a RAW variant of the 7x7 stride-2 stem kernel that reads the two raw images directly and applies scale/shift in LDS after staging. This removes the separate scale_shift launches and the intermediate normalized-image buffer. Also adds a fused kernel that gathers the split predict_flow partial sums, writes the flow, and does the 2x flow deconvolution into the concat blob in one pass, replacing two launches per refinement level. Both paths are on by default through FUSED_FORWARD and need extra per-block work and bounds masks.

```diff
diff --git a/flownet2_amd/_lib.py b/flownet2_amd/_lib.py
--- a/flownet2_amd/_lib.py
+++ b/flownet2_amd/_lib.py
@@ -46,6 +46,8 @@
     "fn2_augmentation_matrix", "fn2_flow_augmentation_forward",
     "fn2_data_augmentation_workspace_bytes", "fn2_data_augmentation_forward",
 ]
+
+FUSED_EXPORTS = ["fn2_conv_k7s2_relu_forward_raw", "fn2_predict_flow_upsample_forward_into", "fn2_predict_flow_conv_nsplit"]
 
 
 class Fn2Error(RuntimeError):
@@ -273,7 +275,10 @@
         L.fn2_debug_correlation_units_plan.argtypes = [i, i, i, i, C.POINTER(C.c_uint), i]
     if hasattr(L, "fn2_debug_set_resample_generic"):
         L.fn2_debug_set_resample_generic.argtypes = [i]
-    for name in EXPORTS:
+    L.fn2_conv_k7s2_relu_forward_raw.argtypes = [fp, fp, C.c_float, fp, fp, fp, fp, i, i, i, i, C.c_float, vp]
+    L.fn2_predict_flow_upsample_forward_into.argtypes = [fp, fp, fp, fp, fp, fp, fp, i, i, i, i, i, i, vp, sz, vp]
+    L.fn2_predict_flow_conv_nsplit.argtypes = [i, i, i, i]
+    for name in EXPORTS + FUSED_EXPORTS:
         if not hasattr(L, name):
             raise RuntimeError(f"{SO_PATH} does not export {name}")
         fn = getattr(L, name)
diff --git a/flownet2_amd/build.py b/flownet2_amd/build.py
--- a/flownet2_amd/build.py
+++ b/flownet2_amd/build.py
@@ -27,7 +27,7 @@
     if not os.path.exists(SO):
         return True
     t = os.path.getmtime(SO)
-    deps = sources() + glob.glob(os.path.join(CSRC, "*.hpp")) + [os.path.join(HERE, "..", "include", "flownet2_hip.h")]
+    deps = sources() + glob.glob(os.path.join(CSRC, "*.hpp")) + glob.glob(os.path.join(HERE, "..", "include", "*.h"))
     return any(os.path.getmtime(d) > t for d in deps)
 
 
@@ -46,7 +46,7 @@
     for src in sources():
         obj = os.path.join(objdir, os.path.basename(src) + ".o")
         objs.append(obj)
-        hdrs = glob.glob(os.path.join(CSRC, "*.hpp")) + [os.path.join(HERE, "..", "include", "flownet2_hip.h")]
+        hdrs = glob.glob(os.path.join(CSRC, "*.hpp")) + glob.glob(os.path.join(HERE, "..", "include", "*.h"))
         if not force and os.path.exists(obj) and all(os.path.getmtime(obj) >= os.path.getmtime(d) for d in [src] + hdrs):
             continue
         cmd = [hipcc()] + flags + per_file.get(os.path.basename(src), []) + ["-x", "hip", "-c", src, "-o", obj]
diff --git a/flownet2_amd/csrc/conv_stem.hip b/flownet2_amd/csrc/conv_stem.hip
--- a/flownet2_amd/csrc/conv_stem.hip
+++ b/flownet2_amd/csrc/conv_stem.hip
@@ -1,4 +1,5 @@
 #include "fn2_common.hpp"
+#include "../../include/flownet2_hip_fused.h"
 #include "mfma_tile.hpp"
 
 #include <type_traits>
@@ -15,9 +16,13 @@
   int ntx;
   int nyb;
   float slope;
+  const float* in1;
+  const float* shift;
+  float scale;
+  int n_first;
 };
 
-template <int CIN, int RB, int XT, int PASS>
+template <int CIN, int RB, int XT, int PASS, bool RAW = false>
 __global__ void __launch_bounds__(256, 2)
 conv_k7s2_relu(const float* __restrict__ in, const float* __restrict__ weight, const float* __restrict__ bias,
                float* __restrict__ out, StemArgs a) {
@@ -38,9 +43,11 @@
   const int co0 = cog * 64 + wave * 16;
 
   const size_t plane = (size_t)a.Hin * a.Win;
-  const __amdgpu_buffer_rsrc_t rs = __builtin_amdgcn_make_buffer_rsrc(
-      const_cast<float*>(in + ((size_t)n * a.Ctot + a.c0) * plane), 0, (unsigned)(4u * CIN * plane), kRsrcWord3);
+  const float* bottom = in + ((size_t)n * a.Ctot + a.c0) * plane;
+  if constexpr (RAW) bottom = n < a.n_first ? in + (size_t)n * CIN * plane : a.in1 + (size_t)(n - a.n_first) * CIN * plane;
+  const __amdgpu_buffer_rsrc_t rs = __builtin_amdgcn_make_buffer_rsrc(const_cast<float*>(bottom), 0, (unsigned)(4u * CIN * plane), kRsrcWord3);
   const unsigned lds_base = (unsigned)(uintptr_t)(lds_ptr_t)smem;
+  unsigned inside = 0;
 #pragma unroll
   for (int i = 0; i < (NRUN + 3) / 4; ++i) {
     const int run = i * 4 + wave;
@@ -51,7 +58,10 @@
         const int c = s / (ROWS * (RS / 4)), rem = s % (ROWS * (RS / 4));
         const int row = rem / (RS / 4), gq = rem % (RS / 4);
         const int yi = 2 * y0 - 3 + row, xi = 2 * x0 - 4 + 4 * gq;
-        if (yi >= 0 && yi < a.Hin && xi >= 0 && xi < a.Win) voff = 4u * (unsigned)(c * plane + (size_t)yi * a.Win + xi);
+        if (yi >= 0 && yi < a.Hin && xi >= 0 && xi < a.Win) {
+          voff = 4u * (unsigned)(c * plane + (size_t)yi * a.Win + xi);
+          inside |= 1u << i;
+        }
       }
       __builtin_amdgcn_raw_ptr_buffer_load_lds(rs, (lds_ptr_t)(uintptr_t)(lds_base + run * 1024u), 16, voff, 0, 0, 0);
     }
@@ -70,8 +80,35 @@
       }
   }
   const float bv = bias ? bias[co0 + nn] : 0.f;
+  [[maybe_unused]] float sh[CIN];
+  if constexpr (RAW) {
+#pragma unroll
+    for (int c = 0; c < CIN; ++c) sh[c] = a.shift ? a.shift[c] : 0.f;
+  }
   asm volatile("s_waitcnt vmcnt(0)" ::: "memory");
   __syncthreads();
+  if constexpr (RAW) {
+    static_assert((NRUN + 3) / 4 <= 32, "one mask bit per staging iteration");
+#pragma unroll
+    for (int i = 0; i < (NRUN + 3) / 4; ++i) {
+      if (inside & (1u << i)) {
+        const int s = (i * 4 + wave) * 64 + lane;
+        const int c = s / (ROWS * (RS / 4));
+        float shc = sh[0];
+#pragma unroll
+        for (int k = 1; k < CIN; ++k) shc = c == k ? sh[k] : shc;
+        f32x4 v = *reinterpret_cast<f32x4*>(smem + 4 * s);
+#pragma unroll
+        for (int j = 0; j < 4; ++j) {
+          float prod = v[j] * a.scale;
+          asm volatile("" : "+v"(prod));
+          v[j] = prod + shc;
+        }
+        *reinterpret_cast<f32x4*>(smem + 4 * s) = v;
+      }
+    }
+    __syncthreads();
+  }
 
   const int abase = 2 * nn + kk + 1;
   const int xq = 4 * (lane >> 4);
@@ -121,11 +158,13 @@
   }
 }
 
-template <int CIN, int PASS>
+template <int CIN, int PASS, bool RAW = false>
 static int launch_stem(const float* in, const float* weight, const float* bias, float* out, int N, int Ctot, int c0, int Hin, int Win,
-                       int Cout, float slope, hipStream_t st) {
+                       int Cout, float slope, hipStream_t st, const float* in1 = nullptr, int n_first = 0, float scale = 1.f,
+                       const float* shift = nullptr) {
   constexpr int RB = 2, XT = 7;
   StemArgs a;
+  a.in1 = in1; a.n_first = n_first; a.scale = scale; a.shift = shift;
   a.N = N; a.Hin = Hin; a.Win = Win; a.Cout = Cout; a.slope = slope; a.Ctot = Ctot; a.c0 = c0;
   a.Hout = (Hin + 6 - 7) / 2 + 1; a.Wout = (Win + 6 - 7) / 2 + 1;
   a.ntx = (a.Wout + 16 * XT - 1) / (16 * XT);
@@ -135,10 +174,10 @@
   constexpr size_t lds = sizeof(float) * CIN * (2 * RB + 5) * (32 * XT + 8) + 1024;
   static bool attr_set = false;
   if (!attr_set) {
-    (void)hipFuncSetAttribute(reinterpret_cast<const void*>(&conv_k7s2_relu<CIN, RB, XT, PASS>), hipFuncAttributeMaxDynamicSharedMemorySize, (int)lds);
+    (void)hipFuncSetAttribute(reinterpret_cast<const void*>(&conv_k7s2_relu<CIN, RB, XT, PASS, RAW>), hipFuncAttributeMaxDynamicSharedMemorySize, (int)lds);
     attr_set = true;
   }
-  hipLaunchKernelGGL((conv_k7s2_relu<CIN, RB, XT, PASS>), dim3((unsigned)grid), dim3(256), lds, st, in, weight, bias, out, a);
+  hipLaunchKernelGGL((conv_k7s2_relu<CIN, RB, XT, PASS, RAW>), dim3((unsigned)grid), dim3(256), lds, st, in, weight, bias, out, a);
   return check_launch("conv_k7s2_relu_forward");
 }
 
@@ -167,3 +206,16 @@
   if (rc) return rc;
   return launch_stem<6, 2>(in, weight, bias, out, N, 12, 6, Hin, Win, Cout, negative_slope, st);
 }
+
+FN2_API int fn2_conv_k7s2_relu_forward_raw(const float* img0, const float* img1, float scale, const float* shift, const float* weight,
+                                           const float* bias, float* out, int N, int Hin, int Win, int Cout, float negative_slope, void* stream) {
+  if (N < 0 || Hin <= 0 || Win <= 0 || Cout <= 0) return fail(FN2_ERR_INVALID_ARG, "conv_k7s2_relu_raw: bad shape");
+  if (N == 0) return FN2_OK;
+  if (!img0 || !img1 || !weight || !out) return fail(FN2_ERR_INVALID_ARG, "conv_k7s2_relu_raw: null blob");
+  if (!fn2_conv_k7s2_relu_supported(3, Hin, Win, Cout))
+    return fail(FN2_ERR_UNSUPPORTED, "conv_k7s2_relu_raw: needs Cout %% 64 == 0, width %% 8 == 0 (got Cout %d, W %d)", Cout, Win);
+  if (((reinterpret_cast<uintptr_t>(img0) | reinterpret_cast<uintptr_t>(img1) | reinterpret_cast<uintptr_t>(out)) & 15) != 0)
+    return fail(FN2_ERR_UNSUPPORTED, "conv_k7s2_relu_raw: blobs must be 16-byte aligned");
+  return launch_stem<3, 0, true>(img0, weight, bias, out, 2 * N, 3, 0, Hin, Win, Cout, negative_slope, reinterpret_cast<hipStream_t>(stream),
+                                 img1, N, scale, shift);
+}
diff --git a/flownet2_amd/csrc/flow_head.hip b/flownet2_amd/csrc/flow_head.hip
--- a/flownet2_amd/csrc/flow_head.hip
+++ b/flownet2_amd/csrc/flow_head.hip
@@ -1,4 +1,5 @@
 #include "fn2_common.hpp"
+#include "../../include/flownet2_hip_fused.h"
 
 namespace fn2 {
 
@@ -116,6 +117,77 @@
   }
 }
 
+constexpr int kUpTH = 8, kUpTW = 16;
+
+template <int NSPLIT>
+__global__ void __launch_bounds__(256) conv3x3_c2_gather_up(const float* __restrict__ P, const float* __restrict__ bias, float* __restrict__ flow,
+                                                             const float* __restrict__ wu, const float* __restrict__ bu, float* __restrict__ out,
+                                                             int N, int H, int W, int tiles_x, int tiles_y, int out_ctot, int out_c0) {
+  constexpr int HH = kUpTH + 2, HW = kUpTW + 2;
+  __shared__ float fl[2][HH][HW];
+  int b = blockIdx.x;
+  const int tx = b % tiles_x; b /= tiles_x;
+  const int ty = b % tiles_y;
+  const int n = b / tiles_y;
+  const int y0 = ty * kUpTH, x0 = tx * kUpTW;
+  const unsigned plane = (unsigned)H * W;
+  for (int e = threadIdx.x; e < 2 * HH * HW; e += 256) {
+    const int o = e / (HH * HW), r = e % (HH * HW);
+    const int ly = r / HW, lx = r % HW;
+    const int y = y0 + ly - 1, x = x0 + lx - 1;
+    float sacc = 0.f;
+    if (y >= 0 && y < H && x >= 0 && x < W) {
+      float v[NSPLIT][9];
+#pragma unroll
+      for (int sp = 0; sp < NSPLIT; ++sp) {
+        const float* Pn = P + (((size_t)sp * N + n) * 18 + o * 9) * plane;
+#pragma unroll
+        for (int dy = 0; dy < 3; ++dy)
+#pragma unroll
+          for (int dx = 0; dx < 3; ++dx) {
+            const int yy = y + dy - 1, xx = x + dx - 1;
+            const bool ok = yy >= 0 && yy < H && xx >= 0 && xx < W;
+            v[sp][dy * 3 + dx] = ok ? Pn[(size_t)(dy * 3 + dx) * plane + (unsigned)yy * W + xx] : 0.f;
+          }
+      }
+      sacc = bias ? bias[o] : 0.f;
+#pragma unroll
+      for (int sp = 0; sp < NSPLIT; ++sp)
+#pragma unroll
+        for (int t = 0; t < 9; ++t) sacc += v[sp][t];
+      if (ly >= 1 && ly <= kUpTH && lx >= 1 && lx <= kUpTW) flow[((size_t)n * 2 + o) * plane + (unsigned)y * W + x] = sacc;
+    }
+    fl[o][ly][lx] = sacc;
+  }
+  __syncthreads();
+  const int Ho = 2 * H, Wo = 2 * W;
+  for (int e = threadIdx.x; e < 4 * kUpTH * kUpTW; e += 256) {
+    const int X = 2 * x0 + e % (2 * kUpTW), Y = 2 * y0 + e / (2 * kUpTW);
+    if (Y >= Ho || X >= Wo) continue;
+    float a0 = bu ? bu[0] : 0.f, a1 = bu ? bu[1] : 0.f;
+#pragma unroll
+    for (int t2 = 0; t2 < 2; ++t2) {
+      const int ky = ((Y + 1) & 1) + 2 * t2;
+      const int iy = (Y + 1 - ky) / 2;
+      if (Y + 1 - ky < 0 || iy >= H) continue;
+#pragma unroll
+      for (int t1 = 0; t1 < 2; ++t1) {
+        const int kx = ((X + 1) & 1) + 2 * t1;
+        const int ix = (X + 1 - kx) / 2;
+        if (X + 1 - kx < 0 || ix >= W) continue;
+#pragma unroll
+        for (int c = 0; c < 2; ++c) {
+          const float v = fl[c][iy - y0 + 1][ix - x0 + 1];
+          a0 = fmaf(wu[((c * 2 + 0) * 4 + ky) * 4 + kx], v, a0);
+          a1 = fmaf(wu[((c * 2 + 1) * 4 + ky) * 4 + kx], v, a1);
+        }
+      }
+    }
+    out[(((size_t)n * out_ctot + out_c0 + 0) * Ho + Y) * Wo + X] = a0;
+    out[(((size_t)n * out_ctot + out_c0 + 1) * Ho + Y) * Wo + X] = a1;
+  }
+}
+
 }
 
 using namespace fn2;
@@ -127,6 +199,11 @@
   int nsplit = 1;
   while (nsplit < 8 && blocks * kHeadG * nsplit < 4096 && C >= 8 * kHeadG * nsplit * 2) nsplit *= 2;
   return nsplit;
+}
+
+FN2_API int fn2_predict_flow_conv_nsplit(int N, int C, int H, int W) {
+  if (N < 1 || C < 1 || H < 1 || W < 1) return 0;
+  return head_splits(N, C, H, W);
 }
 
 FN2_API size_t fn2_predict_flow_conv_workspace_bytes(int N, int C, int H, int W) {
@@ -178,3 +255,34 @@
   hipLaunchKernelGGL(deconv4x4s2_c2, dim3(blocks_for(total, 256, 4096)), dim3(256), 0, as_stream(stream), in, weight, bias, top, N, H, W, top_channels, top_c0);
   return check_launch("upsample_flow_deconv_forward_into");
 }
+
+FN2_API int fn2_predict_flow_upsample_forward_into(const float* in, const float* weight, const float* bias, float* flow,
+                                                   const float* up_weight, const float* up_bias, float* top, int N, int C, int H, int W,
+                                                   int top_channels, int top_c0, void* workspace, size_t workspace_bytes, void* stream) {
+  if (N < 0 || C < 1 || H < 1 || W < 1) return fail(FN2_ERR_INVALID_ARG, "predict_flow_upsample: bad shape [%d,%d,%d,%d]", N, C, H, W);
+  if (top_c0 < 0 || top_c0 + 2 > top_channels) return fail(FN2_ERR_INVALID_ARG, "predict_flow_upsample: channel slice outside the blob");
+  if (N == 0) return FN2_OK;
+  if (!in || !weight || !flow || !up_weight || !top) return fail(FN2_ERR_INVALID_ARG, "predict_flow_upsample: NULL blob pointer");
+  const int tiles_x = (W + kUpTW - 1) / kUpTW, tiles_y = (H + kUpTH - 1) / kUpTH;
+  if ((long long)H * W >= (1ll << 29) || 2ll * N > 65535 || (long long)N * tiles_x * tiles_y > 0x7fffffffll)
+    return fail(FN2_ERR_UNSUPPORTED, "predict_flow_upsample: blob too large");
+  const size_t need = fn2_predict_flow_conv_workspace_bytes(N, C, H, W);
+  if (!workspace || workspace_bytes < need) return fail(FN2_ERR_WORKSPACE, "predict_flow_upsample: workspace too small (%zu < %zu)", workspace_bytes, need);
+  const long long total = (long long)N * H * W;
+  const unsigned blocks = (unsigned)((total + kHeadPix - 1) / kHeadPix);
+  const int nsplit = head_splits(N, C, H, W);
+  hipStream_t st = as_stream(stream);
+  float* P = reinterpret_cast<float*>(workspace);
+  hipLaunchKernelGGL(conv3x3_c2_taps<kHeadG>, dim3(blocks, nsplit), dim3(kHeadPix * kHeadG), 0, st, in, weight, P, N, C, H, W, nsplit);
+  const dim3 g2((unsigned)(N * tiles_x * tiles_y));
+#define FN2_GATHER_UP(S) hipLaunchKernelGGL(conv3x3_c2_gather_up<S>, g2, dim3(256), 0, st, P, bias, flow, up_weight, up_bias, top, N, H, W, \
+                                            tiles_x, tiles_y, top_channels, top_c0)
+  switch (nsplit) {
+    case 1: FN2_GATHER_UP(1); break;
+    case 2: FN2_GATHER_UP(2); break;
+    case 4: FN2_GATHER_UP(4); break;
+    default: FN2_GATHER_UP(8); break;
+  }
+#undef FN2_GATHER_UP
+  return check_launch("predict_flow_upsample_forward_into");
+}
diff --git a/flownet2_amd/functional.py b/flownet2_amd/functional.py
--- a/flownet2_amd/functional.py
+++ b/flownet2_amd/functional.py
@@ -49,6 +49,14 @@
 def scale_shift(x, scale, shift=None, out=None, out_c0=0):
     with torch.no_grad():
         return ops.scale_shift_forward(x.detach().contiguous(), scale, shift, out=out, out_c0=out_c0)
+
+
+def conv_k7s2_relu_raw(img0, img1, scale, shift, weight, bias, negative_slope=0.1):
+    if not img0.is_cuda or conv_route_name((2 * img0.shape[0],) + tuple(img0.shape[1:]), weight, 2, 3) != "stem":
+        return None
+    with torch.no_grad():
+        return ops.conv_k7s2_relu_forward_raw(img0.detach().contiguous(), img1.detach().contiguous(), scale, shift, weight.detach().contiguous(),
+                                              bias, negative_slope)
 
 
 class _Correlation(torch.autograd.Function):
@@ -304,6 +312,12 @@
     if _needs_grad(x, weight, bias):
         return _UpsampleFlow.apply(x, weight, bias, None if out is None else (out, out_c0))
     return run(x, weight, bias)
+
+
+def predict_flow_upsample(x, weight, bias, up_weight, up_bias, out, out_c0):
+    with torch.no_grad():
+        return ops.predict_flow_upsample_forward(x.detach().contiguous(), weight.detach().contiguous(), bias, up_weight.detach().contiguous(),
+                                                 up_bias, out, out_c0)
 
 
 class _BiasLeakyReLU(torch.autograd.Function):
diff --git a/flownet2_amd/nets.py b/flownet2_amd/nets.py
--- a/flownet2_amd/nets.py
+++ b/flownet2_amd/nets.py
@@ -152,7 +152,20 @@
     return d
 
 
-def _refine_stage(P, skip, x, dname, flow, uname, backend):
+FUSED_FORWARD = [True]
+
+
+def _predict_flow_stage(P, x, pname, skip, dname, uname, backend):
+    blob = skip[0] if isinstance(skip, tuple) else None
+    if (FUSED_FORWARD[0] and blob is not None and not torch.is_grad_enabled() and x.is_cuda and backend is not None
+            and hasattr(backend, "predict_flow_upsample")):
+        cs, cd = skip[1].shape[1], P[dname + ".w"].shape[1]
+        assert blob.shape[1] == cs + cd + 2
+        return backend.predict_flow_upsample(x, P[pname + ".w"], P[pname + ".b"], P[uname + ".w"], P[uname + ".b"], blob, cs + cd), True
+    return _pf(P, x, pname, backend), False
+
+
+def _refine_stage(P, skip, x, dname, flow, uname, backend, upsampled=False):
     def up(t, name, out=None, out_c0=0):
         if backend is not None and hasattr(backend, "upsample_flow_deconv"):
             if out is not None:
@@ -174,7 +187,9 @@
         part = lambda t, c0, c: t if t.requires_grad else blob[:, c0:c0 + c]
         return _ConcatInPlace.apply(blob, s, part(d, cs, cd), part(u, cs + cd, 2))
     _stage_deconv(P, x, dname, blob, cs, cd, backend)
-    if hasattr(backend, "upsample_flow_deconv"):
+    if upsampled:
+        pass
+    elif hasattr(backend, "upsample_flow_deconv"):
         up(flow, uname, out=blob, out_c0=cs + cd)
     else:
         blob[:, cs + cd:].copy_(up(flow, uname))
@@ -187,18 +202,15 @@
             return backend.predict_flow_conv(x, P[name + ".w"], P[name + ".b"])
         return _conv(x, P, name, 1, 1, act=False, backend=backend)
 
-    def stage(skip, x, dname, flow, uname):
-        return _refine_stage(P, skip, x, dname, flow, uname, backend)
-
-
-    flow6 = pf(conv6_1, "Convolution1")
-    c5 = stage(conv5_1, conv6_1, "deconv5", flow6, "upsample_flow6to5")
-    flow5 = pf(c5, "Convolution2")
-    c4 = stage(conv4_1, c5, "deconv4", flow5, "upsample_flow5to4")
-    flow4 = pf(c4, "Convolution3")
-    c3 = stage(conv3_1, c4, "deconv3", flow4, "upsample_flow4to3")
-    flow3 = pf(c3, "Convolution4")
-    c2 = stage(conv2, c3, "deconv2", flow3, "upsample_flow3to2")
+    def level(x, pname, skip, dname, uname):
+        flow, upsampled = _predict_flow_stage(P, x, pname, skip, dname, uname, backend)
+        return flow, _refine_stage(P, skip, x, dname, flow, uname, backend, upsampled=upsampled)
+
+
+    flow6, c5 = level(conv6_1, "Convolution1", conv5_1, "deconv5", "upsample_flow6to5")
+    flow5, c4 = level(c5, "Convolution2", conv4_1, "deconv4", "upsample_flow5to4")
+    flow4, c3 = level(c4, "Convolution3", conv3_1, "deconv3", "upsample_flow4to3")
+    flow3, c2 = level(c3, "Convolution4", conv2, "deconv2", "upsample_flow3to2")
     flow2 = pf(c2, "Convolution5")
     return {2: flow2, 3: flow3, 4: flow4, 5: flow5, 6: flow6}
 
@@ -275,11 +287,14 @@
         return g_all
 
 
-def flownet_c_core(P, img0, img1, backend, towers=None):
-    x = towers if towers is not None else torch.cat([img0, img1], 0)
-    n = x.shape[0] // 2
-    chain1, chain2 = _stem_chain(P, x, backend)
-    c1 = _conv(x, P, "conv1", 2, 3, backend=backend, relu_chain=chain1)
+def flownet_c_core(P, img0, img1, backend, towers=None, conv1=None):
+    if conv1 is not None:
+        n, c1, chain2 = conv1.shape[0] // 2, conv1, None
+    else:
+        x = towers if towers is not None else torch.cat([img0, img1], 0)
+        n = x.shape[0] // 2
+        chain1, chain2 = _stem_chain(P, x, backend)
+        c1 = _conv(x, P, "conv1", 2, 3, backend=backend, relu_chain=chain1)
     blob2, c2 = _skip_conv(c1, P, "conv2", 2, 2, "deconv2", backend, relu_chain=chain2)
     training = TOWER_SPLIT_OPS[0] and torch.is_grad_enabled() and c2.requires_grad
     c2_first = None
@@ -352,7 +367,12 @@
         mean = _const(img0.device, (0.411, 0.433, 0.45))
     if (ah, aw) == (H, W) and img0.is_cuda and not torch.is_grad_enabled() and hasattr(backend, "scale_shift"):
         neg_mean = _const(img0.device, (-0.411, -0.433, -0.45)) if neg_default else (-mean).contiguous()
-        if kind == "C":
+        c1 = None
+        if kind == "C" and FUSED_FORWARD[0] and hasattr(backend, "conv_k7s2_relu_raw"):
+            c1 = backend.conv_k7s2_relu_raw(img0, img1, 1.0 / 255.0, neg_mean, P["conv1.w"], P["conv1.b"], NEG_SLOPE)
+        if c1 is not None:
+            flows = flownet_c_core(P, None, None, backend, conv1=c1)
+        elif kind == "C":
             x = torch.empty((2 * N, 3, H, W), device=img0.device, dtype=torch.float32)
             backend.scale_shift(img0, 1.0 / 255.0, neg_mean, out=x[:N])
             backend.scale_shift(img1, 1.0 / 255.0, neg_mean, out=x[N:])
@@ -528,14 +548,15 @@
     blob4, c4 = _skip_conv(_conv(c3, P, "conv4", 2, 1, backend=backend), P, "conv4_1", 1, 1, "deconv4", backend)
     blob5, c5 = _skip_conv(_conv(c4, P, "conv5", 2, 1, backend=backend), P, "conv5_1", 1, 1, "deconv5", backend)
     c6 = _conv(_conv(c5, P, "conv6", 2, 1, backend=backend), P, "conv6_1", 1, 1, backend=backend)
-    flow6 = _pf(P, c6, "Convolution1", backend)
-    cat5 = _refine_stage(P, (blob5, c5), c6, "deconv5", flow6, "upsample_flow6to5", backend)
-    flow5 = _pf(P, _conv(cat5, P, "interconv5", 1, 1, act=False, backend=backend), "Convolution2", backend)
-    cat4 = _refine_stage(P, (blob4, c4), cat5, "deconv4", flow5, "upsample_flow5to4", backend)
-    flow4 = _pf(P, _conv(cat4, P, "interconv4", 1, 1, act=False, backend=backend), "Convolution3", backend)
-    cat3 = _refine_stage(P, (blob3, c3), cat4, "deconv3", flow4, "upsample_flow4to3", backend)
-    flow3 = _pf(P, _conv(cat3, P, "interconv3", 1, 1, act=False, backend=backend), "Convolution4", backend)
-    cat2 = _refine_stage(P, (blob2, c2), cat3, "deconv2", flow3, "upsample_flow3to2", backend)
+    def level(head_in, pname, skip, x, dname, uname):
+        flow, upsampled = _predict_flow_stage(P, head_in, pname, skip, dname, uname, backend)
+        return _refine_stage(P, skip, x, dname, flow, uname, backend, upsampled=upsampled)
+
+    inter = lambda cat, name: _conv(cat, P, name, 1, 1, act=False, backend=backend)
+    cat5 = level(c6, "Convolution1", (blob5, c5), c6, "deconv5", "upsample_flow6to5")
+    cat4 = level(inter(cat5, "interconv5"), "Convolution2", (blob4, c4), cat5, "deconv4", "upsample_flow5to4")
+    cat3 = level(inter(cat4, "interconv4"), "Convolution3", (blob3, c3), cat4, "deconv3", "upsample_flow4to3")
+    cat2 = level(inter(cat3, "interconv3"), "Convolution4", (blob2, c2), cat3, "deconv2", "upsample_flow3to2")
     return _pf(P, _conv(cat2, P, "interconv2", 1, 1, act=False, backend=backend), "Convolution5", backend)
 
 
@@ -543,10 +564,11 @@
     blob0, c0 = _conv_into_concat(x, P, "conv0", 1, 1, 16 + 2, backend)
     blob1, c1 = _conv_into_concat(_conv(c0, P, "conv1", 2, 1, backend=backend), P, "conv1_1", 1, 1, 32 + 2, backend)
     c2 = _conv(_conv(c1, P, "conv2", 2, 1, backend=backend), P, "conv2_1", 1, 1, backend=backend)
-    flow2 = _pf(P, c2, "Convolution5", backend)
-    cat1 = _refine_stage(P, (blob1, c1), c2, "deconv1", flow2, "upsample_flow2to1", backend)
-    flow1 = _pf(P, _conv(cat1, P, "interconv1", 1, 1, act=False, backend=backend), "Convolution6", backend)
-    cat0 = _refine_stage(P, (blob0, c0), cat1, "deconv0", flow1, "upsample_flow1to0", backend)
+    flow2, up2 = _predict_flow_stage(P, c2, "Convolution5", (blob1, c1), "deconv1", "upsample_flow2to1", backend)
+    cat1 = _refine_stage(P, (blob1, c1), c2, "deconv1", flow2, "upsample_flow2to1", backend, upsampled=up2)
+    flow1, up1 = _predict_flow_stage(P, _conv(cat1, P, "interconv1", 1, 1, act=False, backend=backend), "Convolution6", (blob0, c0), "deconv0",
+                                     "upsample_flow1to0", backend)
+    cat0 = _refine_stage(P, (blob0, c0), cat1, "deconv0", flow1, "upsample_flow1to0", backend, upsampled=up1)
     return _pf(P, _conv(cat0, P, "interconv0", 1, 1, act=False, backend=backend), "Convolution7", backend)
 
 
diff --git a/flownet2_amd/ops.py b/flownet2_amd/ops.py
--- a/flownet2_amd/ops.py
+++ b/flownet2_amd/ops.py
@@ -356,6 +356,30 @@
     return out
 
 
+def predict_flow_conv_nsplit(N, C, H, W) -> int:
+    return int(_lib.lib().fn2_predict_flow_conv_nsplit(int(N), int(C), int(H), int(W)))
+
+
+def predict_flow_upsample_forward(x, weight, bias, up_weight, up_bias, out, out_c0):
+    x, w, wu = _chk(x, "bottom[0]"), _chk(weight, "weight"), _chk(up_weight, "upsample weight")
+    _chk(out, "top[1]")
+    if not out.is_contiguous():
+        raise ValueError("upsample_flow: the top blob must be contiguous (it is written in place)")
+    N, Cc, H, W = x.shape
+    if tuple(w.shape) != (2, Cc, 3, 3) or tuple(wu.shape) != (2, 2, 4, 4):
+        raise ValueError(f"predict_flow weight must be [2,{Cc},3,3] and the upsample_flow weight [2,2,4,4]")
+    if out.shape[0] != N or tuple(out.shape[2:]) != (2 * H, 2 * W):
+        raise ValueError(f"upsample_flow: top blob {tuple(out.shape)} does not match [{N},*,{2 * H},{2 * W}]")
+    b = _chk(bias, "bias", ndim=1) if bias is not None else None
+    bu = _chk(up_bias, "upsample bias", ndim=1) if up_bias is not None else None
+    flow = torch.empty((N, 2, H, W), device=x.device, dtype=torch.float32)
+    nbytes = _lib.lib().fn2_predict_flow_conv_workspace_bytes(N, Cc, H, W)
+    ws = torch.empty(nbytes, dtype=torch.uint8, device=x.device) if nbytes else None
+    check(_lib.lib().fn2_predict_flow_upsample_forward_into(_ptr(x), _ptr(w), _ptr(b), _ptr(flow), _ptr(wu), _ptr(bu), _ptr(out), N, Cc, H, W,
+                                                            out.shape[1], int(out_c0), _ptr(ws), nbytes, _stream()))
+    return flow
+
+
 def bias_leaky_relu_(x, bias=None, negative_slope=0.1):
     if not (isinstance(x, torch.Tensor) and x.is_cuda and x.dtype == torch.float32 and x.dim() == 4 and x.is_contiguous()):
         raise ValueError("bias_leaky_relu_: expected a contiguous float32 CUDA (HIP) NCHW tensor")
@@ -450,6 +474,22 @@
     out = torch.empty((N, Cout, (H - 1) // 2 + 1, (W - 1) // 2 + 1), device=x.device, dtype=torch.float32)
     check(_lib.lib().fn2_conv_k7s2_relu_forward(_ptr(x), _ptr(w), _ptr(b), _ptr(out), N, Cin, H, W, Cout,
                                                 C.c_float(float(negative_slope)), _stream()))
+    return out
+
+
+def conv_k7s2_relu_forward_raw(img0, img1, scale, shift, weight, bias=None, negative_slope=0.1):
+    a, b2, w = _chk(img0, "bottom[0]"), _chk(img1, "bottom[1]"), _chk(weight, "weight")
+    N, Cin, H, W = a.shape
+    Cout = w.shape[0]
+    if Cin != 3 or tuple(b2.shape) != tuple(a.shape) or tuple(w.shape) != (Cout, 3, 7, 7):
+        raise ValueError(f"raw stem: two [N,3,H,W] images and a [Cout,3,7,7] weight, got {tuple(a.shape)}, {tuple(b2.shape)}, {tuple(w.shape)}")
+    s = _chk(shift, "shift", ndim=1) if shift is not None else None
+    if s is not None and s.numel() != 3:
+        raise ValueError("raw stem: shift must have 3 entries")
+    b = _chk(bias, "bias", ndim=1) if bias is not None else None
+    out = torch.empty((2 * N, Cout, (H - 1) // 2 + 1, (W - 1) // 2 + 1), device=a.device, dtype=torch.float32)
+    check(_lib.lib().fn2_conv_k7s2_relu_forward_raw(_ptr(a), _ptr(b2), C.c_float(float(scale)), _ptr(s), _ptr(w), _ptr(b), _ptr(out), N, H, W, Cout,
+                                                    C.c_float(float(negative_slope)), _stream()))
     return out
 
 
diff --git a/include/flownet2_hip_fused.h b/include/flownet2_hip_fused.h
--- /dev/null
+++ b/include/flownet2_hip_fused.h
@@ -0,0 +1,21 @@
+#ifndef FLOWNET2_HIP_FUSED_H_
+#define FLOWNET2_HIP_FUSED_H_
+
+#include <stddef.h>
+
+#ifdef __cplusplus
+extern "C" {
+#endif
+
+int fn2_conv_k7s2_relu_forward_raw(const float* img0, const float* img1, float scale, const float* shift, const float* weight,
+                                   const float* bias, float* top, int N, int Hin, int Win, int Cout, float negative_slope, void* stream);
+
+int fn2_predict_flow_upsample_forward_into(const float* in, const float* weight, const float* bias, float* flow,
+                                           const float* up_weight, const float* up_bias, float* top, int N, int C, int H, int W,
+                                           int top_channels, int top_c0, void* workspace, size_t workspace_bytes, void* stream);
+int fn2_predict_flow_conv_nsplit(int N, int C, int H, int W);
+
+#ifdef __cplusplus
+}
+#endif
+#endif
```

Measured after the change: 3542 (median of 6 runs). Within noise of the previous version (+0.6%).
